# Gadersd/stable-diffusion-burn

Measured on AMD Instinct MI355X. Metric: images/sec @512x512, 20-step DDIM CFG=7.5, SD v1.4, higher is better.
Workload: dtype f32

## Files before the change

include/sdmi.h:

```cpp
#ifndef SDMI_H
#define SDMI_H

#include <stddef.h>
#include <stdint.h>

#ifdef __cplusplus
extern "C" {
#endif

typedef struct sdmi_ctx sdmi_ctx;

typedef enum sdmi_status {
    SDMI_OK = 0,
    SDMI_ERR_INVALID = -1,
    SDMI_ERR_HIP = -2,
    SDMI_ERR_WEIGHTS = -3,
    SDMI_ERR_IO = -4,
    SDMI_ERR_UNSUPPORTED = -5,
    SDMI_ERR_STATE = -6
} sdmi_status;

typedef struct sdmi_config {
    int32_t device;
    int32_t model_channels;
// ... 87 lines not shown
} sdmi_hires;
int sdmi_hires_latent(sdmi_ctx* ctx, const float* context, int32_t n, int32_t T, const float* uncond, int32_t Tu, double scale, size_t n_steps,
                      const float* init_latent, uint64_t seed, const sdmi_hires* hires, const float* hires_noise, float* latent_out);
int sdmi_hires_image(sdmi_ctx* ctx, const float* context, int32_t n, int32_t T, const float* uncond, int32_t Tu, double scale, size_t n_steps,
                     const float* init_latent, uint64_t seed, const sdmi_hires* hires, const float* hires_noise, uint8_t* rgb_out);

typedef struct sdmi_lora sdmi_lora;
int sdmi_lora_create(sdmi_ctx* ctx, sdmi_lora** out);
int sdmi_lora_add(sdmi_lora* a, const char* target, const float* down, const float* up, int32_t rank, float alpha);
int sdmi_lora_set_scale(sdmi_lora* a, double scale);
int sdmi_lora_get_scale(sdmi_lora* a, double* scale, int32_t* n_targets);
int sdmi_lora_destroy(sdmi_lora* a);
int sdmi_lora_effective_weight(sdmi_ctx* ctx, const char* name, float* out, size_t n);

int sdmi_qkv_attention(sdmi_ctx* ctx, const float* q, const float* k, const float* v,
                       const float* mask, int32_t mask_ld, int32_t n, int32_t nq, int32_t nk,
                       int32_t n_state, int32_t n_head, float* out);

typedef struct sdmi_tokenizer sdmi_tokenizer;

int sdmi_tokenizer_create(sdmi_tokenizer** out, const char* merges_path);
void sdmi_tokenizer_destroy(sdmi_tokenizer* tok);
int sdmi_tokenizer_vocab_size(const sdmi_tokenizer* tok);
int sdmi_tokenizer_encode(const sdmi_tokenizer* tok, const char* text, int32_t* ids, int32_t capacity, int32_t* n_ids);
int sdmi_tokenizer_decode(const sdmi_tokenizer* tok, const int32_t* ids, int32_t n, char* out, int32_t capacity, int32_t* n_bytes);

int sdmi_clip_forward(sdmi_ctx* ctx, const int32_t* tokens, int32_t n, int32_t seq_len, float* out);

int sdmi_context(sdmi_ctx* ctx, const sdmi_tokenizer* tok, const char* text, float* out, int32_t capacity_tokens, int32_t* T);

int sdmi_write_png(const char* path, const uint8_t* rgb, int32_t width, int32_t height);

int sdmi_sample_latent_dev(sdmi_ctx* ctx, const float* context, int32_t n, int32_t T,
                           const float* uncond, int32_t Tu, double scale, size_t n_steps,
                           const float* init_latent, float* latent_out);
int sdmi_latent_to_image_dev(sdmi_ctx* ctx, const float* latent, int32_t n, uint8_t* rgb_out);
int sdmi_sample_image_dev(sdmi_ctx* ctx, const float* context, int32_t n, int32_t T,
                          const float* uncond, int32_t Tu, double scale, size_t n_steps,
                          const float* init_latent, uint8_t* rgb_out);
int sdmi_img2img_latent_dev(sdmi_ctx* ctx, const float* context, int32_t n, int32_t T, const float* uncond, int32_t Tu,
                            double scale, size_t n_steps, double strength, const float* z0, const float* mask,
                            const float* noise, uint64_t seed, float* latent_out);
int sdmi_img2img_image_dev(sdmi_ctx* ctx, const float* context, int32_t n, int32_t T, const float* uncond, int32_t Tu,
                           double scale, size_t n_steps, double strength, const uint8_t* init_rgb, const float* mask,
                           const float* noise, uint64_t seed, uint8_t* rgb_out);
int sdmi_hires_latent_dev(sdmi_ctx* ctx, const float* context, int32_t n, int32_t T, const float* uncond, int32_t Tu, double scale, size_t n_steps,
                          const float* init_latent, const sdmi_hires* hires, const float* hires_noise, float* latent_out);
int sdmi_hires_image_dev(sdmi_ctx* ctx, const float* context, int32_t n, int32_t T, const float* uncond, int32_t Tu, double scale, size_t n_steps,
                         const float* init_latent, const sdmi_hires* hires, const float* hires_noise, uint8_t* rgb_out);

typedef struct sdmi_multi sdmi_multi;
int sdmi_create_multi(sdmi_multi** out, const sdmi_config* cfg , const int32_t* devices, int32_t n_devices);
void sdmi_destroy_multi(sdmi_multi* m);
int32_t sdmi_multi_size(sdmi_multi* m);
sdmi_ctx* sdmi_multi_ctx(sdmi_multi* m, int32_t index);
int sdmi_multi_load_weights(sdmi_multi* m, const char* kind, const char* path);
int sdmi_sample_image_sharded(sdmi_multi* m, const float* context, int32_t T, const float* uncond, int32_t Tu,
                              double scale, size_t n_steps, int32_t n_images, const float* init_latents, uint64_t seed,
                              uint8_t* rgb_out);
int sdmi_multi_set_sampler(sdmi_multi* m, const sdmi_sampler* sampler);
int sdmi_shard_range(int32_t n_images, int32_t rank, int32_t n_ranks, int32_t* begin, int32_t* end);
int64_t sdmi_multi_broadcast_count(sdmi_multi* m);
int sdmi_selftest_rank_errors(int32_t n_ranks, int32_t failing_rank);


int sdmi_op_group_norm(sdmi_ctx* ctx, const float* x, const float* gamma, const float* beta,
                       int32_t n, int32_t c, int32_t h, int32_t w, int32_t n_group, float eps,
                       int32_t fuse_silu, float* out);
int sdmi_op_group_norm_fp8(sdmi_ctx* ctx, const float* x, const float* gamma, const float* beta,
                           int32_t n, int32_t c, int32_t h, int32_t w, int32_t n_group, float eps,
                           int32_t fuse_silu, float* out);
int sdmi_op_layer_norm(sdmi_ctx* ctx, const float* x, const float* gamma, const float* beta,
                       int32_t rows, int32_t c, float eps, float* out);
int sdmi_op_conv2d(sdmi_ctx* ctx, const float* x, const float* weight, const float* bias,
                   int32_t n, int32_t cin, int32_t h, int32_t w, int32_t cout, int32_t k,
                   int32_t stride, int32_t pad, int32_t upsample2x, float* out);
int sdmi_op_linear(sdmi_ctx* ctx, const float* x, const float* weight, const float* bias,
                   int32_t rows, int32_t cin, int32_t cout, float* out);
int sdmi_op_conv2d_epilogue(sdmi_ctx* ctx, const float* x, const float* weight, const float* bias, const float* temb,
                            int32_t temb_stride, const float* resid, int32_t resid_ld, int32_t n, int32_t cin, int32_t h,
                            int32_t w, int32_t cout, int32_t k, int32_t stride, int32_t pad, int32_t upsample2x, float* out);
int sdmi_op_linear_epilogue(sdmi_ctx* ctx, const float* x, const float* weight, const float* bias, const float* resid,
                            int32_t resid_ld, int32_t rows, int32_t cin, int32_t cout, float* out);
typedef struct sdmi_op_view {
    int32_t in_ld, in_off;
    int32_t out_ld, out_off;
    float in_fill;
    int32_t in_planes, out_planes;
} sdmi_op_view;
int sdmi_op_conv2d_view(sdmi_ctx* ctx, const float* x, const float* weight, const float* bias, const float* temb, int32_t temb_stride,
                        const float* resid, int32_t resid_ld, int32_t n, int32_t cin, int32_t h, int32_t w, int32_t cout, int32_t k,
                        int32_t stride, int32_t pad, int32_t upsample2x, const sdmi_op_view* view, float* parent, float* parent_planes);
int sdmi_op_linear_view(sdmi_ctx* ctx, const float* x, const float* weight, const float* bias, const float* resid, int32_t resid_ld,
                        int32_t rows, int32_t cin, int32_t cout, const sdmi_op_view* view, float* parent);
int sdmi_op_group_norm_view(sdmi_ctx* ctx, const float* x, const float* gamma, const float* beta, int32_t n, int32_t c, int32_t h, int32_t w,
                            int32_t n_group, float eps, int32_t fuse_silu, const sdmi_op_view* view, int32_t form, float* out);
int sdmi_op_cat_chain(sdmi_ctx* ctx, const float* x, const float* w_x, const float* b_x, const float* w_skip, const float* b_skip,
                      const float* gamma, const float* beta, int32_t n, int32_t cin, int32_t h, int32_t w, int32_t cx, int32_t cskip,
                      float eps, int32_t fuse_silu, int32_t dense, float* out);
int sdmi_op_geglu(sdmi_ctx* ctx, const float* proj, int32_t rows, int32_t hidden, float* out);
int sdmi_op_qkv_attention_ragged(sdmi_ctx* ctx, const float* q, const float* k, const float* v, const int32_t* kv_len,
                                 int32_t n, int32_t nq, int32_t nk, int32_t n_state, int32_t n_head, float* out);
int sdmi_op_resize(sdmi_ctx* ctx, const float* x, int32_t n, int32_t h, int32_t w, int32_t out_h, int32_t out_w, int32_t mode, int32_t antialias,
                   float* out);
int sdmi_op_geglu_forward(sdmi_ctx* ctx, const float* x, const float* weight, const float* bias, int32_t rows, int32_t cin,
                          int32_t hidden, float* out);
int sdmi_op_timestep_embedding(sdmi_ctx* ctx, int32_t t, int32_t dim, float* out);

int sdmi_set_option(sdmi_ctx* ctx, const char* key, const char* value);
int sdmi_last_call_stats(sdmi_ctx* ctx, double* gpu_ms, int64_t* n_kernels, double* flops);
int sdmi_profile_stats(sdmi_ctx* ctx, int32_t cls, double* ms, int64_t* launches, double* flops, double* bytes);
int sdmi_profile_overhead(sdmi_ctx* ctx, double* ms);
int sdmi_bench_conv(sdmi_ctx* ctx, int32_t n, int32_t cin, int32_t h, int32_t w, int32_t cout,
                    int32_t k, int32_t stride, int32_t upsample2x, int32_t tile_cfg, int32_t splitk,
                    int32_t iters, double* ms_out);

int sdmi_bench_attention(sdmi_ctx* ctx, int32_t n, int32_t nq, int32_t nk, int32_t n_state, int32_t n_head,
                         int32_t iters, double* ms_out);

#ifdef __cplusplus
}
#endif
#endif
```

stable_diffusion_burn_amd/_capi.py:

```python
from __future__ import annotations

import ctypes as C
import os
import sys
from pathlib import Path

_PKG = Path(__file__).resolve().parent
LIB_PATH = _PKG / "lib" / "libsdmi.so"


class SdmiError(RuntimeError):
    def __init__(self, status: int, message: str):
        super().__init__(f"sdmi status {status}: {message}")
        self.status = status


class SdmiConfig(C.Structure):
    _fields_ = [
        ("device", C.c_int32), ("model_channels", C.c_int32), ("n_head", C.c_int32), ("ctx_dim", C.c_int32),
        ("latent_h", C.c_int32), ("latent_w", C.c_int32), ("vae_ch", C.c_int32), ("max_batch", C.c_int32),
        ("precision", C.c_int32), ("clip_layers", C.c_int32), ("clip_heads", C.c_int32), ("clip_vocab", C.c_int32),
        ("clip_ctx", C.c_int32), ("reserved", C.c_int32 * 3),
    ]

# ... 16 lines not shown
_F = C.POINTER(C.c_float)
_HIRES = C.POINTER(SdmiHires)
_SAMPLER = C.POINTER(SdmiSampler)
_VIEW = C.POINTER(SdmiOpView)
_U8 = C.POINTER(C.c_uint8)
_CTX = C.c_void_p
_TOK = C.c_void_p
_I32 = C.POINTER(C.c_int32)

SIGNATURES = {
    "sdmi_default_config": (C.c_int, [C.POINTER(SdmiConfig)]),
    "sdmi_create": (C.c_int, [C.POINTER(_CTX), C.POINTER(SdmiConfig)]),
    "sdmi_destroy": (None, [_CTX]),
    "sdmi_last_error": (C.c_char_p, []),
    "sdmi_synchronize": (C.c_int, [_CTX]),
    "sdmi_version": (C.c_char_p, []),
    "sdmi_set_stream": (C.c_int, [_CTX, C.c_void_p, C.c_int32]),
    "sdmi_set_weight": (C.c_int, [_CTX, C.c_char_p, _F, C.c_int32, C.POINTER(C.c_int64)]),
    "sdmi_weight_count": (C.c_int, [_CTX]),
    "sdmi_weight_info": (C.c_int, [_CTX, C.c_int32, C.POINTER(C.c_char_p), C.POINTER(C.c_int32), C.POINTER(C.c_int64)]),
    "sdmi_load_weights_dir": (C.c_int, [_CTX, C.c_char_p]),
    "sdmi_load_weights_mpk": (C.c_int, [_CTX, C.c_char_p]),
    "sdmi_mpk_list": (C.c_int, [C.c_char_p, C.c_char_p, C.c_size_t, C.POINTER(C.c_size_t)]),
    "sdmi_load_weights_packed": (C.c_int, [_CTX, _F, C.c_size_t, C.c_int32]),
    "sdmi_packed_size": (C.c_int64, [_CTX, C.c_int32]),
    "sdmi_finalize_weights": (C.c_int, [_CTX]),
    "sdmi_unet_forward": (C.c_int, [_CTX, _F, C.c_int32, _F, C.c_int32, C.c_int32, _F]),
    "sdmi_sample_latent": (C.c_int, [_CTX, _F, C.c_int32, C.c_int32, _F, C.c_int32, C.c_double, C.c_size_t, _F, C.c_uint64, _F]),
    "sdmi_decode_latent": (C.c_int, [_CTX, _F, C.c_int32, _F]),
    "sdmi_latent_to_image": (C.c_int, [_CTX, _F, C.c_int32, _U8]),
    "sdmi_sample_image": (C.c_int, [_CTX, _F, C.c_int32, C.c_int32, _F, C.c_int32, C.c_double, C.c_size_t, _F, C.c_uint64, _U8]),
    "sdmi_img2img_timesteps": (C.c_int, [C.c_int32, C.c_size_t, C.c_double, _I32, C.c_int32, _I32]),
    "sdmi_img2img_latent": (C.c_int, [_CTX, _F, C.c_int32, C.c_int32, _F, C.c_int32, C.c_double, C.c_size_t, C.c_double, _F, _F, _F, C.c_uint64, _F]),
    "sdmi_img2img_image": (C.c_int, [_CTX, _F, C.c_int32, C.c_int32, _F, C.c_int32, C.c_double, C.c_size_t, C.c_double, _U8, _F, _F, C.c_uint64, _U8]),
    "sdmi_set_sampler": (C.c_int, [_CTX, _SAMPLER]),
    "sdmi_get_sampler": (C.c_int, [_CTX, _SAMPLER]),
    "sdmi_sampler_coefs": (C.c_int, [_SAMPLER, _F, C.c_int32, _I32, C.c_int32, C.c_int64, C.POINTER(C.c_double)]),
    "sdmi_set_latent_size": (C.c_int, [_CTX, C.c_int32, C.c_int32]),
    "sdmi_get_latent_size": (C.c_int, [_CTX, _I32, _I32]),
    "sdmi_resize_weights": (C.c_int, [C.c_int32, C.c_int32, C.c_int32, C.c_int32, _I32, _I32, C.POINTER(C.c_double), C.c_int32, _I32, _I32]),
    "sdmi_hires_latent": (C.c_int, [_CTX, _F, C.c_int32, C.c_int32, _F, C.c_int32, C.c_double, C.c_size_t, _F, C.c_uint64, _HIRES, _F, _F]),
    "sdmi_hires_image": (C.c_int, [_CTX, _F, C.c_int32, C.c_int32, _F, C.c_int32, C.c_double, C.c_size_t, _F, C.c_uint64, _HIRES, _F, _U8]),
    "sdmi_hires_latent_dev": (C.c_int, [_CTX, C.c_void_p, C.c_int32, C.c_int32, C.c_void_p, C.c_int32, C.c_double, C.c_size_t, C.c_void_p, _HIRES, C.c_void_p, C.c_void_p]),
    "sdmi_hires_image_dev": (C.c_int, [_CTX, C.c_void_p, C.c_int32, C.c_int32, C.c_void_p, C.c_int32, C.c_double, C.c_size_t, C.c_void_p, _HIRES, C.c_void_p, C.c_void_p]),
    "sdmi_op_resize": (C.c_int, [_CTX, _F, C.c_int32, C.c_int32, C.c_int32, C.c_int32, C.c_int32, C.c_int32, C.c_int32, _F]),
    "sdmi_multi_set_sampler": (C.c_int, [C.c_void_p, _SAMPLER]),
    "sdmi_lora_create": (C.c_int, [_CTX, C.POINTER(C.c_void_p)]),
    "sdmi_lora_add": (C.c_int, [C.c_void_p, C.c_char_p, _F, _F, C.c_int32, C.c_float]),
    "sdmi_lora_set_scale": (C.c_int, [C.c_void_p, C.c_double]),
    "sdmi_lora_get_scale": (C.c_int, [C.c_void_p, C.POINTER(C.c_double), _I32]),
    "sdmi_lora_destroy": (C.c_int, [C.c_void_p]),
    "sdmi_lora_effective_weight": (C.c_int, [_CTX, C.c_char_p, _F, C.c_size_t]),
    "sdmi_qkv_attention": (C.c_int, [_CTX, _F, _F, _F, _F, C.c_int32, C.c_int32, C.c_int32, C.c_int32, C.c_int32, C.c_int32, _F]),
    "sdmi_tokenizer_create": (C.c_int, [C.POINTER(_TOK), C.c_char_p]),
    "sdmi_tokenizer_destroy": (None, [_TOK]),
    "sdmi_tokenizer_vocab_size": (C.c_int, [_TOK]),
    "sdmi_tokenizer_encode": (C.c_int, [_TOK, C.c_char_p, _I32, C.c_int32, _I32]),
    "sdmi_tokenizer_decode": (C.c_int, [_TOK, _I32, C.c_int32, C.c_char_p, C.c_int32, _I32]),
    "sdmi_clip_forward": (C.c_int, [_CTX, _I32, C.c_int32, C.c_int32, _F]),
    "sdmi_context": (C.c_int, [_CTX, _TOK, C.c_char_p, _F, C.c_int32, _I32]),
    "sdmi_encode_image": (C.c_int, [_CTX, _F, C.c_int32, _F]),
    "sdmi_write_png": (C.c_int, [C.c_char_p, _U8, C.c_int32, C.c_int32]),
    "sdmi_sample_latent_dev": (C.c_int, [_CTX, C.c_void_p, C.c_int32, C.c_int32, C.c_void_p, C.c_int32, C.c_double, C.c_size_t, C.c_void_p, C.c_void_p]),
    "sdmi_latent_to_image_dev": (C.c_int, [_CTX, C.c_void_p, C.c_int32, C.c_void_p]),
    "sdmi_sample_image_dev": (C.c_int, [_CTX, C.c_void_p, C.c_int32, C.c_int32, C.c_void_p, C.c_int32, C.c_double, C.c_size_t, C.c_void_p, C.c_void_p]),
    "sdmi_img2img_latent_dev": (C.c_int, [_CTX, C.c_void_p, C.c_int32, C.c_int32, C.c_void_p, C.c_int32, C.c_double, C.c_size_t, C.c_double, C.c_void_p, C.c_void_p, C.c_void_p, C.c_uint64, C.c_void_p]),
    "sdmi_img2img_image_dev": (C.c_int, [_CTX, C.c_void_p, C.c_int32, C.c_int32, C.c_void_p, C.c_int32, C.c_double, C.c_size_t, C.c_double, C.c_void_p, C.c_void_p, C.c_void_p, C.c_uint64, C.c_void_p]),
    "sdmi_create_multi": (C.c_int, [C.POINTER(C.c_void_p), C.POINTER(SdmiConfig), _I32, C.c_int32]),
    "sdmi_destroy_multi": (None, [C.c_void_p]),
    "sdmi_multi_size": (C.c_int32, [C.c_void_p]),
    "sdmi_multi_ctx": (C.c_void_p, [C.c_void_p, C.c_int32]),
    "sdmi_multi_load_weights": (C.c_int, [C.c_void_p, C.c_char_p, C.c_char_p]),
    "sdmi_sample_image_sharded": (C.c_int, [C.c_void_p, _F, C.c_int32, _F, C.c_int32, C.c_double, C.c_size_t, C.c_int32, _F, C.c_uint64, _U8]),
    "sdmi_shard_range": (C.c_int, [C.c_int32, C.c_int32, C.c_int32, _I32, _I32]),
    "sdmi_multi_broadcast_count": (C.c_int64, [C.c_void_p]),
    "sdmi_selftest_rank_errors": (C.c_int, [C.c_int32, C.c_int32]),
    "sdmi_op_group_norm": (C.c_int, [_CTX, _F, _F, _F, C.c_int32, C.c_int32, C.c_int32, C.c_int32, C.c_int32, C.c_float, C.c_int32, _F]),
    "sdmi_op_group_norm_fp8": (C.c_int, [_CTX, _F, _F, _F, C.c_int32, C.c_int32, C.c_int32, C.c_int32, C.c_int32, C.c_float, C.c_int32, _F]),
    "sdmi_op_layer_norm": (C.c_int, [_CTX, _F, _F, _F, C.c_int32, C.c_int32, C.c_float, _F]),
    "sdmi_op_conv2d": (C.c_int, [_CTX, _F, _F, _F, C.c_int32, C.c_int32, C.c_int32, C.c_int32, C.c_int32, C.c_int32, C.c_int32, C.c_int32, C.c_int32, _F]),
    "sdmi_op_linear": (C.c_int, [_CTX, _F, _F, _F, C.c_int32, C.c_int32, C.c_int32, _F]),
    "sdmi_op_conv2d_epilogue": (C.c_int, [_CTX, _F, _F, _F, _F, C.c_int32, _F, C.c_int32, C.c_int32, C.c_int32, C.c_int32, C.c_int32, C.c_int32, C.c_int32, C.c_int32,
                                          C.c_int32, C.c_int32, _F]),
    "sdmi_op_linear_epilogue": (C.c_int, [_CTX, _F, _F, _F, _F, C.c_int32, C.c_int32, C.c_int32, C.c_int32, _F]),
    "sdmi_op_conv2d_view": (C.c_int, [_CTX, _F, _F, _F, _F, C.c_int32, _F, C.c_int32, C.c_int32, C.c_int32, C.c_int32, C.c_int32, C.c_int32, C.c_int32, C.c_int32,
                                      C.c_int32, C.c_int32, _VIEW, _F, _F]),
    "sdmi_op_linear_view": (C.c_int, [_CTX, _F, _F, _F, _F, C.c_int32, C.c_int32, C.c_int32, C.c_int32, _VIEW, _F]),
    "sdmi_op_group_norm_view": (C.c_int, [_CTX, _F, _F, _F, C.c_int32, C.c_int32, C.c_int32, C.c_int32, C.c_int32, C.c_float, C.c_int32, _VIEW, C.c_int32, _F]),
    "sdmi_op_cat_chain": (C.c_int, [_CTX, _F, _F, _F, _F, _F, _F, _F, C.c_int32, C.c_int32, C.c_int32, C.c_int32, C.c_int32, C.c_int32, C.c_float, C.c_int32,
                                    C.c_int32, _F]),
    "sdmi_op_geglu_forward": (C.c_int, [_CTX, _F, _F, _F, C.c_int32, C.c_int32, C.c_int32, _F]),
    "sdmi_op_geglu": (C.c_int, [_CTX, _F, C.c_int32, C.c_int32, _F]),
    "sdmi_op_qkv_attention_ragged": (C.c_int, [_CTX, _F, _F, _F, _I32, C.c_int32, C.c_int32, C.c_int32, C.c_int32, C.c_int32, _F]),
    "sdmi_op_timestep_embedding": (C.c_int, [_CTX, C.c_int32, C.c_int32, _F]),
    "sdmi_set_option": (C.c_int, [_CTX, C.c_char_p, C.c_char_p]),
    "sdmi_last_call_stats": (C.c_int, [_CTX, C.POINTER(C.c_double), C.POINTER(C.c_int64), C.POINTER(C.c_double)]),
    "sdmi_profile_stats": (C.c_int, [_CTX, C.c_int32, C.POINTER(C.c_double), C.POINTER(C.c_int64), C.POINTER(C.c_double), C.POINTER(C.c_double)]),
    "sdmi_profile_overhead": (C.c_int, [_CTX, C.POINTER(C.c_double)]),
    "sdmi_bench_conv": (C.c_int, [_CTX, C.c_int32, C.c_int32, C.c_int32, C.c_int32, C.c_int32, C.c_int32, C.c_int32, C.c_int32, C.c_int32, C.c_int32, C.c_int32, C.POINTER(C.c_double)]),
    "sdmi_bench_attention": (C.c_int, [_CTX, C.c_int32, C.c_int32, C.c_int32, C.c_int32, C.c_int32, C.c_int32, C.POINTER(C.c_double)]),
}

_lib = None


def load_library() -> C.CDLL:
    global _lib
    if _lib is not None:
        return _lib
    if not LIB_PATH.exists():
        raise ImportError(
            f"{LIB_PATH} is missing: build it with `python -m stable_diffusion_burn_amd.build` "
            "(libsdmi has no CPU or PyTorch fallback)")
    lib = C.CDLL(str(LIB_PATH), mode=C.RTLD_GLOBAL if "torch" in sys.modules else C.RTLD_LOCAL)
    for name, (res, args) in SIGNATURES.items():
        fn = getattr(lib, name)
        fn.restype = res
        fn.argtypes = args
    _lib = lib
    return lib


def check(status: int) -> None:
    if status != 0:
        msg = load_library().sdmi_last_error()
        raise SdmiError(status, msg.decode("utf-8", "replace") if msg else "")
```

stable_diffusion_burn_amd/csrc/engine.cpp:

```cpp
#include "engine.hpp"
#include "mpk_reader.hpp"

#include <dlfcn.h>

#include <algorithm>
#include <cmath>
#include <cstdarg>
#include <cstdio>
#include <cstring>
#include <fstream>
#include <sstream>

namespace sdmi {

static constexpr size_t kAlign = 256;
static constexpr size_t kSlabMin = (size_t)1 << 30;

DevPool::~DevPool() {
    for (auto& s : slabs_) (void)hipFree(s.base);
}

void* DevPool::alloc(size_t bytes) {
    if (bytes == 0) bytes = kAlign;
    bytes = (bytes + kAlign - 1) / kAlign * kAlign;
// ... 532 lines not shown
            SDMI_HIP(hipEventCreateWithFlags(&stager_->done[i], hipEventDisableTiming));
        }
    }
    Stager& st = *stager_;
    const size_t need = (bytes + 255) / 256 * 256;
    if (st.used + need > kStageBytes) {
        SDMI_HIP(hipEventRecord(st.done[st.cur], stream_));
        st.busy[st.cur] = true;
        st.cur ^= 1;
        st.used = 0;
        if (st.busy[st.cur]) { SDMI_HIP(hipEventSynchronize(st.done[st.cur])); st.busy[st.cur] = false; }
    }
    *offset = st.used;
    *half = st.cur;
    st.used += need;
    return st.pinned[st.cur] + *offset;
}

void* Engine::persistent_alloc(size_t bytes, bool weight_buffer) {
    void* p = nullptr;
    SDMI_HIP(hipMalloc(&p, bytes));
    if (pool_.fill() >= 0) {
        hipError_t e = hipMemsetAsync(p, pool_.fill(), bytes, stream_);
        if (e == hipSuccess && !weight_buffer) e = hipStreamSynchronize(stream_);
        if (e != hipSuccess) { (void)hipFree(p); SDMI_HIP(e); }
        pool_.note_fill(bytes);
    }
    if (weight_buffer) persistent_blocks_.push_back({p, bytes});
    return p;
}

void Engine::ensure_arena(int group) {
    if (arena_done_[group]) return;
    size_t total = 0;
    for (auto& e : entries_) {
        if (e.group != group || e.kind == 3 || *e.dst) continue;
        size_t count = 1;
        for (int i = 0; i < e.ndim; ++i) count *= (size_t)e.dims[i];
        if (e.kind == 0 && e.dims[1] == 3) count = count / 3 * 4;
        total += (count * (e.wdt ? 2 : 4) + 255) / 256 * 256;
    }
    if (total) {
        char* base = static_cast<char*>(persistent_alloc(total));
        weight_allocs_.push_back(base);
        arena_base_[group] = base;
        arena_bytes_[group] = total;
        if (!bf16_) {
            split_base_[group] = static_cast<char*>(persistent_alloc(total / 2 * 3));
            weight_allocs_.push_back(split_base_[group]);
        }
        size_t off = 0;
        for (auto& e : entries_) {
            if (e.group != group || e.kind == 3 || *e.dst) continue;
            size_t count = 1;
            for (int i = 0; i < e.ndim; ++i) count *= (size_t)e.dims[i];
            if (e.kind == 0 && e.dims[1] == 3) count = count / 3 * 4;
            *e.dst = reinterpret_cast<float*>(base + off);
            off += (count * (e.wdt ? 2 : 4) + 255) / 256 * 256;
        }
    }
    if (opt_keep_masters_) {
        size_t mtotal = 0;
        for (auto& e : entries_)
            if (e.group == group && e.kind <= 1) mtotal += (stage_elems(e) * sizeof(float) + 255) / 256 * 256;
        if (mtotal) {
            char* mbase = static_cast<char*>(persistent_alloc(mtotal));
            weight_allocs_.push_back(mbase);
            size_t off = 0;
            for (auto& e : entries_) {
                if (e.group != group || e.kind > 1) continue;
                e.master = reinterpret_cast<float*>(mbase + off);
                off += (stage_elems(e) * sizeof(float) + 255) / 256 * 256;
            }
        }
    }
    arena_done_[group] = true;
}

Engine::TempSplit::TempSplit(Engine* e_, const float* bt_, long long rows, long long K) : e(e_), bt(bt_) {
    if (e->bf16_ || K % 32 || rows <= 0) return;
    planes = e->pool_.alloc((size_t)rows * K * 6);
    hipError_t err = launch_pack_split3(bt, planes, rows, (int)K, e->stream_, e->b3_grouped(rows));
    if (err != hipSuccess) { e->pool_.free(planes); planes = nullptr; SDMI_HIP(err); }
    e->temp_split_bt_ = bt;
    e->temp_split_planes_ = planes;
}
Engine::TempSplit::~TempSplit() {
    if (!planes) return;
    e->temp_split_bt_ = nullptr;
    e->temp_split_planes_ = nullptr;
    e->pool_.free(planes);
}

const void* Engine::split_planes(const float* bt) const {
    if (bt && bt == temp_split_bt_) return temp_split_planes_;
    const char* b = reinterpret_cast<const char*>(bt);
    for (int g = 0; g < 3; ++g)
        if (split_base_[g] && b >= arena_base_[g] && b < arena_base_[g] + arena_bytes_[g]) return split_base_[g] + (size_t)(b - arena_base_[g]) / 2 * 3;
    for (const SplitRegion& r : split_regions_)
        if (b >= r.base && b < r.base + r.bytes) return r.planes + (size_t)(b - r.base) / 2 * 3;
    return nullptr;
}

static size_t entry_count(const WeightEntry& e) {
    size_t count = 1;
    for (int i = 0; i < e.ndim; ++i) count *= (size_t)e.dims[i];
    return count;
}

size_t Engine::stage_elems(const WeightEntry& e) {
    const size_t count = entry_count(e);
    return (e.kind == 0 && e.dims[1] == 3) ? count / 3 * 4 : count;
}

void Engine::pack_entry(WeightEntry& e, float* stage) {
    const size_t n_stage = stage_elems(e);
    if (e.pre_scale != 1.f) SDMI_HIP(launch_scale_f32(stage, (long long)n_stage, e.pre_scale, stream_));
    hipError_t err;
    if (e.kind == 0) {
        const int cout = (int)e.dims[0], cin = e.dims[1] == 3 ? 4 : (int)e.dims[1], k = (int)e.dims[2];
        if (!(cin % 32 == 0 || (cin < 32 && cin % 4 == 0))) throw Error(SDMI_ERR_UNSUPPORTED, "conv Cin must be a multiple of 32, or < 32 and a multiple of 4");
        err = e.wdt ? launch_pack_conv_weight_bf16(stage, *e.dst, cout, cin, k, k, stream_)
                    : launch_pack_conv_weight(stage, *e.dst, cout, cin, k, k, stream_);
        if (err == hipSuccess && e.dst8) {
            const size_t kp = (size_t)((cin + 127) / 128 * 128) * k * k;
            if (!*e.dst8) {
                void* q = persistent_alloc((size_t)cout * kp);
                weight_allocs_.push_back(q);
                void* sc = persistent_alloc((size_t)cout * kp / 32);
                weight_allocs_.push_back(sc);
                *e.dst8 = reinterpret_cast<float*>(q);
                *e.dsts = reinterpret_cast<float*>(sc);
            }
            err = launch_pack_conv_weight_fp8(stage, *e.dst8, *e.dsts, cout, cin, k, k, stream_);
        }
    } else {
        err = e.wdt ? launch_pack_linear_weight_bf16(stage, *e.dst, (int)e.dims[0], (int)e.dims[1], stream_)
                    : launch_pack_linear_weight(stage, *e.dst, (int)e.dims[0], (int)e.dims[1], stream_);
        if (err == hipSuccess && e.dst8) {
            const int cin = (int)e.dims[0], cout = (int)e.dims[1];
            const size_t kp = (size_t)(cin + 127) / 128 * 128;
            if (!*e.dst8) {
                void* q = persistent_alloc((size_t)cout * kp);
                weight_allocs_.push_back(q);
                void* sc = persistent_alloc((size_t)cout * kp / 32);
                weight_allocs_.push_back(sc);
                *e.dst8 = reinterpret_cast<float*>(q);
                *e.dsts = reinterpret_cast<float*>(sc);
            }
            err = launch_pack_linear_weight_fp8(stage, *e.dst8, *e.dsts, cin, cout, stream_);
        }
    }
    SDMI_HIP(err);
    if (!e.wdt) {
        const long long rows = e.kind == 0 ? e.dims[0] : e.dims[1];
        const long long K = e.kind == 0 ? (e.dims[1] == 3 ? 4 : e.dims[1]) * e.dims[2] * e.dims[3] : e.dims[0];
        void* planes = const_cast<void*>(split_planes(*e.dst));
        if (planes && K % 32 == 0) SDMI_HIP(launch_pack_split3(*e.dst, planes, rows, (int)K, stream_, b3_grouped(rows)));
    }
}

void Engine::stage_commit(WeightEntry& e, size_t offset, int half) {
    Stager& st = *stager_;
    const size_t count = entry_count(e);
    const float* host = reinterpret_cast<const float*>(st.pinned[half] + offset);
    if (e.kind == 3) {
        alphas_.assign(host, host + count);
        e.set = true;
        return;
    }
    ensure_arena(e.group);
    if (e.kind == 2) {
        SDMI_HIP(hipMemcpyAsync(*e.dst, host, count * sizeof(float), hipMemcpyHostToDevice, stream_));
    } else {
        float* stage = reinterpret_cast<float*>(st.dev[half] + offset);
        const size_t n_stage = stage_elems(e);
        SDMI_HIP(hipMemcpyAsync(stage, host, n_stage * sizeof(float), hipMemcpyHostToDevice, stream_));
        if (e.master) SDMI_HIP(hipMemcpyAsync(e.master, stage, n_stage * sizeof(float), hipMemcpyDeviceToDevice, stream_));
// ... 409 lines not shown
        }
    }
    SDMI_HIP(hipEventRecord(ev0_, stream_));
}
void Engine::end_call() {
    SDMI_HIP(hipEventRecord(ev1_, stream_));
    if (call_dev_ && has_user_stream_) SDMI_HIP(hipStreamWaitEvent(user_stream_, ev1_, 0));
    SDMI_HIP(hipEventSynchronize(ev1_));
    float ms = 0;
    SDMI_HIP(hipEventElapsedTime(&ms, ev0_, ev1_));
    last_ms = ms; last_kernels = n_kernels_; last_flops = flops_;
}
void Engine::abort_call() noexcept {
    (void)hipStreamSynchronize(stream_);
    try {
        us_ = UNetState{};
        pool_.free_since(call_mark_);
    } catch (...) {}
}

void Engine::set_option(const std::string& key, const std::string& value) {
    if (key == "gemm_tile") gopt_.force_tile = (value == "auto") ? -1 : std::stoi(value);
    else if (key == "splitk") gopt_.force_splits = std::stoi(value);
    else if (key == "roctx") roctx_enable(std::stoi(value) != 0);
    else if (key == "fp8_convs") opt_fp8_convs_ = std::stoi(value);
    else if (key == "fp8_min_rows") opt_fp8_min_rows_ = std::stoi(value);
    else if (key == "fp8_linear") opt_fp8_linear_ = std::stoi(value);
    else if (key == "fp8_ops") opt_fp8_ops_ = std::stoi(value);
    else if (key == "op_resid") opt_op_resid_ = std::stoi(value);
    else if (key == "op_misalign") opt_op_misalign_ = std::stoi(value);
    else if (key == "pool_fill") {
        const int b = std::stoi(value);
        if (b < -1 || b > 255) throw Error(SDMI_ERR_INVALID, "pool_fill: -1 (off) or a byte 0 .. 255");
        pool_.set_fill(b);
        if (b >= 0 && std::none_of(entries_.begin(), entries_.end(), [](const WeightEntry& w) { return w.set; })) {
            SDMI_HIP(hipSetDevice(cfg_.device));
            for (const PersistentBlock& pb : persistent_blocks_) {
                SDMI_HIP(hipMemsetAsync(pb.p, b, pb.bytes, stream_));
                pool_.note_fill(pb.bytes);
            }
        }
    }
    else if (key == "dump_pool_fills") {
        std::ofstream f(value);
        if (!f) throw Error(SDMI_ERR_IO, "dump_pool_fills: cannot write " + value);
        unsigned long long blocks = 0, bytes = 0;
        pool_.take_fill_counts(&blocks, &bytes);
        f << blocks << " " << bytes << "\n";
    }
    else if (key == "cfg_share") opt_cfg_share_ = std::stoi(value);
    else if (key == "attn_kv_splits") opt_attn_kv_splits_ = std::stoi(value);
    else if (key == "attn_kv_prefer8") opt_attn_kv_prefer8_ = std::stoi(value);
    else if (key == "b3_grouped") {
        if (!entries_.empty() && std::any_of(entries_.begin(), entries_.end(), [](const WeightEntry& w) { return w.set; }))
            throw Error(SDMI_ERR_STATE, "b3_grouped selects the layout the weight planes are packed in: set it before the first weight is loaded");
        opt_b3_grouped_ = std::stoi(value);
    }
    else if (key == "keep_masters") {
        if (std::any_of(entries_.begin(), entries_.end(), [](const WeightEntry& w) { return w.set; }) || arena_done_[0] || arena_done_[1] || arena_done_[2])
            throw Error(SDMI_ERR_STATE, "keep_masters decides what the weight arenas hold: set it before the first weight is loaded");
        opt_keep_masters_ = std::stoi(value) != 0;
    }
    else if (key == "attn_pack_tail") opt_attn_pack_tail_ = (value == "default") ? 3 : std::stoi(value);
    else if (key == "gn32_min_wgs") opt_gn32_min_wgs_ = (opt_gn32_min_wgs_ & ~0xFFFF) | (std::stoi(value) & 0xFFFF);
    else if (key == "gn32_stats_min_wgs") opt_gn32_min_wgs_ = (opt_gn32_min_wgs_ & 0xFFFF) | ((std::stoi(value) + 1) << 16);
    else if (key == "gn_target_wgs") gn_tune_.target_wgs = std::stoi(value);
    else if (key == "gn_max_threads") gn_tune_.max_threads = std::stoi(value);
    else if (key == "gn_unroll") gn_tune_.unroll = std::stoi(value);
    else if (key == "fp8_tile") opt_fp8_tile_ = (value == "auto") ? -1 : std::stoi(value);
    else if (key == "resid_acc") opt_resid_acc_ = std::stoi(value);
    else if (key == "attn_bf16") opt_attn_bf16_ = std::stoi(value);
    else if (key == "attn_bf16_variant") opt_attn_bf16_variant_ = (value == "default") ? kAttnBf16VariantDefault : std::stoi(value, nullptr, 0);
    else if (key == "attn_split") opt_attn_split_ = std::stoi(value);
    else if (key == "gemm_bf16x") gopt_.gemm_bf16x = std::stoi(value);
    else if (key == "gemm_x32") gopt_.gemm_x32 = std::stoi(value);
    else if (key == "gemm_f32s") gopt_.gemm_f32s = std::stoi(value);
    else if (key == "bench_cold") opt_bench_cold_ = std::stoi(value);
    else if (key == "gemm_probe") opt_gemm_probe_ = std::stoi(value);
    else if (key == "conv3_reuse") gopt_.conv3_reuse = std::stoi(value);
    else if (key == "gemm_planes") gopt_.gemm_planes = (value == "default") ? GemmPlanOpts().gemm_planes : std::stoi(value);
    else if (key == "gemm3x_variant") opt_gemm3x_variant_ = (value == "default") ? kGemm3xVariantDefault : std::stoi(value);
    else if (key == "gemm_bf16x_variant") opt_gemm_bf16x_variant_ = (value == "default") ? kGemmBf16xVariantDefault : std::stoi(value);
    else if (key == "geglu_fuse") opt_geglu_fuse_ = std::stoi(value);
    else if (key == "record_shapes") { record_shapes_ = std::stoi(value) != 0; if (record_shapes_) { shape_counts_.clear(); choice_counts_.clear(); } }
    else if (key == "dump_shapes") {
        std::ofstream f(value);
        if (!f) throw Error(SDMI_ERR_IO, "dump_shapes: cannot write " + value);
        for (auto& kv : shape_counts_) f << kv.first << " " << kv.second << "\n";
    }
    else if (key == "dump_choices") {
        std::ofstream f(value);
        if (!f) throw Error(SDMI_ERR_IO, "dump_choices: cannot write " + value);
        for (auto& kv : choice_counts_) f << kv.first << " x" << kv.second << "\n";
    }
    else if (key == "profile") { prof_flush(); profiling_ = std::stoi(value) != 0; prof_tagging_ = std::stoi(value) >= 2; if (profiling_) prof_calibrate(); }
    else if (key == "dump_profile_tags") {
        prof_flush();
        std::ofstream f(value);
        if (!f) throw Error(SDMI_ERR_IO, "dump_profile_tags: cannot write " + value);
        for (auto& kv : prof_tags_) f << kv.second.ms << " " << kv.second.launches << " " << kv.second.flops << " " << kv.second.bytes << "\t" << kv.first << "\n";
    }
    else if (key == "profile_reset") prof_reset();
    else if (key == "tune" || key == "tune_bf16") tuning_.set(value, key == "tune_bf16");
    else if (key == "tune_clear") tuning_.clear();
    else throw Error(SDMI_ERR_INVALID, "unknown option '" + key + "'");
}

void Engine::set_resid_acc(ConvGemm& p, bool eligible, bool resid_ok) const {
    p.resid_acc = 0;
    if (!eligible || (p.N % 8) || (p.ldc % 8)) return;
    if ((opt_resid_acc_ & 1) && p.resid && resid_ok && (p.ldr % 4) == 0 && ((uintptr_t)p.resid & 7) == 0) p.resid_acc |= 1;
    if ((opt_resid_acc_ & 2) && (p.bias || p.rowvec) && (p.rowvec_stride % 4) == 0 && (((uintptr_t)p.bias | (uintptr_t)p.rowvec) & 15) == 0) p.resid_acc |= 2;
}

void Engine::record_choice(const ConvGemm& p, const char* kind, int cfg, const char* note) {
    if (!record_shapes_) return;
    char ck[128];
    std::snprintf(ck, sizeof ck, "%d,%d,%d k%d s%d u%d W%d%s cfg=%d splits=%d%s acc=%d", p.M, p.N, p.K, p.KH, p.stride, p.ups, p.Ws, kind, cfg, p.splits, note, p.resid_acc);
    ++choice_counts_[ck];
}

void Engine::run_gemm(ConvGemm& p, const GemmRun& r) {
    if (p.splits == 1) {
        p.slabs = nullptr; p.slab_stride = 0;
        ProfScope ps(this, r.pc, r.flops, r.bytes);
        ps.set_tag("%s %d,%d,%d k%d%s%s%s cfg=%d splits=1", r.what, p.M, p.N, p.K, p.KH, p.geglu ? " geglu" : "", p.resid ? " resid" : "", p.rowvec ? " rowvec" : "", r.cfg);
        SDMI_HIP(r.launch(p, r.index, stream_));
        count_kernel(r.flops);
        return;
    }
    p.slab_stride = (long long)p.M * p.N;
    Buf slab(this, (size_t)p.splits * p.slab_stride * sizeof(float));
    p.slabs = slab.f();
    {
        ProfScope ps(this, r.pc, r.flops, r.bytes);
        ps.set_tag("%s %d,%d,%d k%d%s cfg=%d splits=%d", r.what, p.M, p.N, p.K, p.KH, p.geglu ? " geglu" : "", r.cfg, p.splits);
        SDMI_HIP(r.launch(p, r.index, stream_));
    }
    count_kernel(r.flops);
    ProfScope ps(this, PC_SPLITK_REDUCE, 0, (double)(p.splits + 1) * p.slab_stride * 4.0);
    if (r.reduce_tag) ps.set_tag("reduce %d,%d,%d k%d cfg=%d splits=%d", p.M, p.N, p.K, p.KH, r.cfg, p.splits);
    SDMI_HIP(r.bf16_reduce ? launch_splitk_reduce_bf16(p, stream_) : launch_splitk_reduce(p, stream_));
    count_kernel();
}

void Engine::launch_gemm(ConvGemm& p, int in_dt, int force_cfg, int force_splits) {
    const int kt_elems = in_dt ? 64 : 32;
    p.kt_total = (p.K + kt_elems - 1) / kt_elems;
    if (in_dt && (p.Cin % 64)) throw Error(SDMI_ERR_UNSUPPORTED, "bf16 GEMM: K slices must be multiples of 64");
    if (record_shapes_) {
        char sk[96];
        std::snprintf(sk, sizeof sk, "%d,%d,%d,%d,%d,%d,%d,%d", p.NB, p.Cin, p.Hs, p.Ws, p.N, p.KH, p.stride, p.ups);
        ++shape_counts_[sk];
    }
    p.Bt3 = in_dt ? nullptr : split_planes(p.Bt);
    p.b3_grouped = b3_grouped((long long)p.N * (p.geglu ? 2 : 1)) ? 1 : 0;
    p.variant = in_dt ? opt_gemm_bf16x_variant_ : opt_gemm3x_variant_;
    p.zero_page = zero_page_;
    p.probe = probe_buf_;
    GemmPlanIn in{};
    in.M = p.M; in.N = p.N; in.K = p.K; in.kt_total = p.kt_total; in.bf16 = in_dt; in.geglu = p.geglu; in.out_mode = p.out_mode; in.force_cfg = force_cfg; in.force_splits = force_splits;
    in.KH = p.KH; in.KW = p.KW; in.stride = p.stride; in.pad = p.pad; in.ups = p.ups; in.Cin = p.Cin; in.Hs = p.Hs; in.Ws = p.Ws; in.Ho = p.Ho; in.Wo = p.Wo;
    in.zero_page = zero_page_ != nullptr;
    in.x32_ok = !in_dt && p.CS == 32 && p.Cin % 32 == 0 && p.out_mode == 0;
    in.s_ok = in.x32_ok && p.Bt3 && (unsigned long long)p.N * (p.geglu ? 2 : 1) * (unsigned long long)p.kt_total * 192ull < 0xFFFFFF00ull;
    in.p_ok = in.s_ok && (unsigned long long)p.NB * p.Hs * p.Ws * (unsigned long long)(p.A3 ? p.a3_ld : p.Cin * 6) < 0xFFFFFF00ull;
    in.from_planes = !in_dt && p.A3 != nullptr;
    if (!in.from_planes && !p.A) throw Error(SDMI_ERR_STATE, "gemm: no activations");
    const GemmPlan g = plan_gemm(in, gopt_, tuning_);
    p.kt_per_split = g.kt_per_split; p.splits = g.splits;
    const bool w_planes = g.tile.family >= kFamS, a_planes = g.tile.family == kFamP;
    const double flops = 2.0 * p.M * (double)p.N * p.K * (p.geglu ? 2.0 : 1.0);
    const unsigned long long es = in_dt ? 2ull : 4ull;
    const unsigned long long a_ext = ((unsigned long long)p.NB * p.Hs * p.Ws - 1) * (unsigned long long)p.a_ld * es + (unsigned long long)p.Cin * es;
    const unsigned long long b_ext = ((unsigned long long)p.N * (p.geglu ? 2 : 1) - 1) * (unsigned long long)p.b_ld * es + (unsigned long long)p.K * es;
    if (a_ext >= 0xFFFFFFE0ull || b_ext >= 0xFFFFFFE0ull) throw Error(SDMI_ERR_UNSUPPORTED, "GEMM: operand larger than 4 GiB (the buffer-load range check needs 32-bit extents)");
    p.a_bytes = (unsigned)a_ext;
    p.b_bytes = (unsigned)b_ext;
    void* const c3_want = in_dt ? nullptr : p.C3;
    const int ldc3_want = p.ldc3;
    const bool vec_out = (p.N % 4 == 0) && (!p.C || p.ldc % 4 == 0) && (!p.resid || p.ldr % 4 == 0);
    const bool c3_native = c3_want && w_planes && vec_out && (!p.geglu || (p.geglu == 2 && a_planes));
    std::unique_ptr<Buf> c_tmp;
    if (!c3_native) {
        p.C3 = nullptr;
        if (c3_want && !p.C) {
            c_tmp.reset(new Buf(this, (size_t)p.M * p.N * sizeof(float)));
            p.C = c_tmp->f(); p.ldc = p.N;
        }
    }
    if (!p.C) p.ldc = p.N;
    std::unique_ptr<Buf> a3_tmp;
    if (a_planes && !p.A3) {
        const long long rows = (long long)p.NB * p.Hs * p.Ws;
        p.a3_ld = (p.Cin / 32) * 192;
        a3_tmp.reset(new Buf(this, (size_t)rows * p.a3_ld));
        ProfScope ps(this, PC_SPLIT_ROWS, 0, (double)rows * p.Cin * 10.0);
        SDMI_HIP(launch_split3_rows(p.A, a3_tmp->p, rows, p.Cin, p.a_ld, p.a3_ld, stream_));
        count_kernel();
        p.A3 = a3_tmp->p;
    }
    set_resid_acc(p, in_dt && g.tile.family == kFamX && g.splits == 1, !p.geglu);
    record_choice(p, "", g.cfg, p.Bt3 || in_dt ? "" : " (no planes)");
    const double a_es = in_dt ? 2.0 : (a_planes ? 6.0 : 4.0), w_es = in_dt ? 2.0 : (w_planes ? 6.0 : 4.0);
    const double c_es = in_dt ? (p.out_mode == 1 ? 4.0 : 2.0) : (p.out_mode == 2 ? 2.0 : ((p.C ? 4.0 : 0.0) + (c3_native ? 6.0 : 0.0)));
    const double gemm_bytes = (double)p.NB * p.Hs * p.Ws * p.Cin * a_es + (double)p.N * (p.geglu ? 2.0 : 1.0) * p.K * w_es + (double)p.M * p.N * c_es;
    static const GemmLauncher kLaunchers[2][kNumGemmFamilies] = {{launch_conv_gemm2, launch_conv_gemm2x, launch_conv_gemm3x, launch_conv_gemm3p},
                                                                 {launch_conv_gemm_bf16, launch_conv_gemm_bf16_large, nullptr, nullptr}};
    run_gemm(p, GemmRun{kLaunchers[in_dt ? 1 : 0][g.tile.family], g.tile.index, "gemm", g.cfg, w_planes ? PC_CONV_SPLIT : PC_CONV_GEMM, in_dt != 0, true, flops, gemm_bytes});
    if (c3_want && !c3_native) {
        ProfScope ps(this, PC_SPLIT_ROWS, 0, (double)p.M * p.N * 10.0);
        SDMI_HIP(launch_split3_rows(p.C, c3_want, p.M, p.N, p.ldc, ldc3_want, stream_));
        count_kernel();
    }
}

void Engine::conv(const ConvW& w, const Act& x, Act& y, int stride, int ups, const float* rowvec, int rowvec_stride,
                  const Act* resid, bool pad_br) {
    if (x.c != w.cin) throw Error(SDMI_ERR_INVALID, "conv: input channels mismatch");
    const int pad = pad_br ? 0 : (w.k == 3 ? 1 : 0);
    const int hin = x.h << ups, win = x.w << ups;
    const int extra = pad_br ? 1 : 0;
    const int ho = (hin + 2 * pad + extra - w.k) / stride + 1, wo = (win + 2 * pad + extra - w.k) / stride + 1;
    if (y.n != x.n || y.h != ho || y.w != wo || y.c != w.cout) throw Error(SDMI_ERR_INVALID, "conv: output shape mismatch");
    ConvGemm p{};
    if (resid && (resid->rows() != y.rows() || resid->c != y.c || resid->dt != y.dt)) throw Error(SDMI_ERR_STATE, "conv: residual shape / type mismatch");
    p.A = x.p; p.Bt = w.bt; p.C = y.p; p.bias = w.bias; p.rowvec = rowvec; p.resid = resid ? resid->p : nullptr;
    if (resid && !resid->p) throw Error(SDMI_ERR_STATE, "conv: the residual must exist as fp32");
    if (!x.dt && plane_gemm(w.cin, w.cout) && split_planes(w.bt)) { p.A3 = x.p3; p.a3_ld = x.ld3; }
    if (!x.p && !p.A3) throw Error(SDMI_ERR_STATE, "conv: the input exists only as planes, which this layer cannot read");
    p.C3 = y.p3; p.ldc3 = y.ld3;
    p.M = x.n * ho * wo; p.N = w.cout; p.K = w.cin * w.k * w.k;
    p.NB = x.n; p.Hs = x.h; p.Ws = x.w; p.Cin = w.cin; p.Ho = ho; p.Wo = wo;
    p.KH = w.k; p.KW = w.k; p.stride = stride; p.pad = pad; p.ups = ups;
    p.ldc = y.stride(); p.ldr = resid ? resid->stride() : y.stride(); p.a_ld = x.stride(); p.b_ld = p.K; p.rowvec_stride = rowvec_stride;
    p.CS = std::min(32, w.cin);
    if (!y.p && !y.p3) throw Error(SDMI_ERR_STATE, "conv: no output buffer");
    if (x.dt != w.dt) throw Error(SDMI_ERR_STATE, "conv: activation / weight storage types disagree");
    p.out_mode = x.dt ? (y.dt ? 0 : 1) : (y.dt ? 2 : 0);
    if (resid && !x.dt && y.dt) throw Error(SDMI_ERR_STATE, "conv: residual not supported on the fp32->bf16 layers");
    launch_gemm(p, x.dt);
}

static ConvGemm linear_gemm(const float* A, int rows, const float* bt, const float* bias, int cin, int cout, float* C, int ldc, const float* resid, int ldr) {
    ConvGemm p{};
    p.A = A; p.Bt = bt; p.C = C; p.bias = bias; p.resid = resid;
    p.M = rows; p.N = cout; p.K = cin;
    p.NB = 1; p.Hs = 1; p.Ws = rows; p.Cin = cin; p.Ho = 1; p.Wo = rows;
    p.KH = 1; p.KW = 1; p.stride = 1; p.pad = 0; p.ups = 0;
    p.ldc = ldc; p.ldr = ldr; p.a_ld = cin; p.b_ld = cin; p.rowvec_stride = 0; p.CS = 32;
    return p;
}

void Engine::gemm(const float* A, int a_rows, const float* bt, const float* bias, int cin, int cout, float* C, int ldc,
                  const float* resid, int ldr, int dt, int out_mode, const void* A3, void* C3) {
    if (dt < 0) dt = edt();
    if (cin % 32) throw Error(SDMI_ERR_UNSUPPORTED, "linear: in_features must be a multiple of 32");
    ConvGemm p = linear_gemm(A, a_rows, bt, bias, cin, cout, C, ldc, resid, ldr);
    p.A3 = A3; p.a3_ld = (cin / 32) * 192;
    p.C3 = C3; p.ldc3 = (cout / 32) * 192;
    if (C3 && (cout % 32)) throw Error(SDMI_ERR_STATE, "linear: plane output needs out_features % 32 == 0");
    p.out_mode = out_mode;
    launch_gemm(p, dt);
}

void Engine::gemm_geglu(const float* x, long long rows, const float* bt, const float* bias, int cin, int hidden, float* out, int dt,
                        const void* x3, void* out3) {
    if (dt < 0) dt = edt();
    if (x3 && (out3 || out) && !dt && opt_geglu_fuse_ && hidden % 32 == 0 && cin % 32 == 0 && split_planes(bt)) {
        const int cfg = plan_geglu_plane_tile(rows, hidden, cin, gopt_, tuning_);
        if (cfg >= 0) {
            ConvGemm p = linear_gemm(x, (int)rows, bt, bias, cin, hidden, out, hidden, nullptr, hidden);
            p.A3 = x3; p.a3_ld = (cin / 32) * 192;
            p.C3 = out3; p.ldc3 = (hidden / 32) * 192;
            p.geglu = 2;
            launch_gemm(p, 0, cfg, 1);
            return;
        }
    }
    if (x3 || out3) {
        Buf proj(this, (size_t)rows * 2 * hidden * 4);
        gemm(x, (int)rows, bt, bias, cin, 2 * hidden, proj.f(), 2 * hidden, nullptr, 0, dt, 0, x3, nullptr);
        {
            ProfScope ps(this, PC_GEGLU, 0, (double)rows * hidden * (8.0 + (out3 ? 6.0 : 4.0)));
            if (out3) SDMI_HIP(launch_geglu_planes(proj.f(), out3, rows, hidden, stream_));
            else SDMI_HIP(launch_geglu(proj.f(), out, rows, hidden, stream_));
        }
        count_kernel();
        return;
    }
    const bool eligible = opt_geglu_fuse_ && hidden % 8 == 0 && cin % (dt ? 64 : 32) == 0 && (dt ? gopt_.gemm_bf16x : gopt_.gemm_x32);
    const int cfg = eligible ? plan_geglu_paired_tile(rows, hidden, opt_geglu_fuse_, !dt && gopt_.gemm_f32s && split_planes(bt)) : -1;
    if (cfg >= 0) {
        ConvGemm p = linear_gemm(x, (int)rows, bt, bias, cin, hidden, out, hidden, nullptr, hidden);
        p.geglu = 1;
        launch_gemm(p, dt, cfg, 1);
        return;
// ... 63 lines not shown
        int kv_splits = 1;
        if (!dt && !mask && opt_attn_kv_splits_ != 1) {
            const long long wgs = (long long)((nq + (on_split ? 127 : 63)) / (on_split ? 128 : 64)) * n * n_head;
            const int tiles = (nk + attn_f32_kv_tile(p) - 1) / attn_f32_kv_tile(p);
            long long s_auto = wgs > 0 && wgs <= 128 ? 256 / wgs : 1;
            s_auto = std::min<long long>(std::min<long long>(s_auto, tiles / 2), 8);
            if (on_split && opt_attn_kv_prefer8_) {
                const long long wgs8 = (long long)((nq + 255) / 256) * n * n_head;
                const long long s8 = std::min<long long>(std::min<long long>(wgs8 < 256 ? (256 + wgs8 - 1) / wgs8 : 1, tiles / 2), 8);
                if (s8 >= 2 && wgs8 * s8 >= 256) s_auto = s8;
            }
            kv_splits = opt_attn_kv_splits_ > 1 ? std::min(opt_attn_kv_splits_, std::max(1, tiles)) : (int)std::max<long long>(1, s_auto);
        }
        std::unique_ptr<Buf> part_o, part_ml;
        if (kv_splits > 1) {
            part_o.reset(new Buf(this, (size_t)kv_splits * n * nq * n_head * d_head * sizeof(float)));
            part_ml.reset(new Buf(this, (size_t)kv_splits * n * n_head * nq * 2 * sizeof(float)));
            p.kv_splits = kv_splits; p.part_o = part_o->f(); p.part_ml = part_ml->f();
        }
        ProfScope ps(this, PC_ATTENTION, fl, 0, kv_splits > 1 ? 2 : 1);
        ps.set_tag("attention n%d nq%d nk%d h%d d%d slices=%d", n, nq, nk, n_head, d_head, kv_splits);
        if (dt && opt_attn_bf16_ && (d_head == 40 || d_head == 80 || d_head == 160)) SDMI_HIP(launch_attention_bf16(p, stream_));
        else if (on_split) SDMI_HIP(launch_attention_split(p, stream_));
        else SDMI_HIP(launch_attention(p, stream_));
        count_kernel(fl);
        if (kv_splits > 1) {
            SDMI_HIP(launch_attention_combine(p, stream_));
            count_kernel();
        }
        return;
    }
    if (mask) throw Error(SDMI_ERR_UNSUPPORTED, "attention: additive mask is only supported for head dims 40/80/160");
    if (d_head % 32) throw Error(SDMI_ERR_UNSUPPORTED, "attention: head dim must be 40/80/160 or a multiple of 32");
    if (dt && (d_head % 64)) throw Error(SDMI_ERR_UNSUPPORTED, "bf16 attention (unfused path): head dim must be a multiple of 64");
    for (int b = 0; b < n; ++b)
        if ((kv_len_host ? kv_len_host[b] : nk) % (dt ? 64 : 32)) throw Error(SDMI_ERR_UNSUPPORTED, "attention (unfused path): key count must be a multiple of 32 (64 for bf16)");
    for (int b = 0; b < n; ++b) {
        const int nkb = kv_len_host ? kv_len_host[b] : nk;
        Buf s(this, (size_t)nq * nkb * sizeof(float));
        Buf pb(this, dt ? (size_t)nq * nkb * 2 : 256);
        Buf vt(this, (size_t)d_head * nkb * (dt ? 2 : 4));
        for (int h = 0; h < n_head; ++h) {
            const float* qb = adv(q, b * q_bs + h * d_head, dt);
            const float* kb = adv(k, b * k_bs + h * d_head, dt);
            const float* vb = adv(v, b * v_bs + h * d_head, dt);
            float* ob = adv(o, b * o_bs + h * d_head, dt);
            ConvGemm g{};
            g.A = qb; g.Bt = kb; g.C = s.f();
            g.M = nq; g.N = nkb; g.K = d_head; g.NB = 1; g.Hs = 1; g.Ws = nq; g.Cin = d_head; g.Ho = 1; g.Wo = nq;
            g.KH = g.KW = 1; g.stride = 1; g.ldc = nkb; g.ldr = nkb; g.a_ld = ldq; g.b_ld = ldk; g.CS = 32;
            g.out_mode = dt ? 1 : 0;
            launch_gemm(g, dt);
            if (dt) { ProfScope ps_o(this, PC_OTHER); SDMI_HIP(launch_softmax_rows_f32_to_bf16(s.f(), pb.p, nq, nkb, scale * scale, stream_)); }
            else { ProfScope ps_o(this, PC_OTHER); SDMI_HIP(launch_softmax_rows(s.f(), nq, nkb, scale * scale, stream_)); }
            count_kernel();
            if (dt) { ProfScope ps_o(this, PC_OTHER); SDMI_HIP(launch_transpose2d_bf16(vb, vt.p, nkb, d_head, ldv, stream_)); }
            else { ProfScope ps_o(this, PC_OTHER); SDMI_HIP(launch_transpose2d(vb, vt.f(), nkb, d_head, ldv, stream_)); }
            count_kernel();
            ConvGemm g2{};
            g2.A = dt ? pb.f() : s.f(); g2.Bt = vt.f(); g2.C = ob;
            g2.M = nq; g2.N = d_head; g2.K = nkb; g2.NB = 1; g2.Hs = 1; g2.Ws = nq; g2.Cin = nkb; g2.Ho = 1; g2.Wo = nq;
            g2.KH = g2.KW = 1; g2.stride = 1; g2.ldc = ldo; g2.ldr = ldo; g2.a_ld = nkb; g2.b_ld = nkb; g2.CS = 32;
            launch_gemm(g2, dt);
        }
    }
}

void Engine::res_block(const ResW& w, const Act& x, Act& y, int step) {
    Range rng(this, "ResBlock");
    Act h2 = new_act(x.n, x.h, x.w, w.cout);
    const float* rowvec = nullptr;
    if (w.has_embed) rowvec = us_.temb.at(w.temb_index) + (size_t)step * w.cout;
    if (use_fp8(w.conv_in, x)) {
        ActQ q1 = new_actq(x.n, x.h, x.w, x.c);
        group_norm_fp8(w.norm_in, x, q1, true);
        conv_fp8(w.conv_in, q1, h2, rowvec, nullptr);
        release(q1);
    } else {
        Act h1 = plane_gemm(x.c, w.cout) ? new_act3(x.n, x.h, x.w, x.c, 2) : new_act(x.n, x.h, x.w, x.c);
        group_norm(w.norm_in, x, h1, true);
        conv(w.conv_in, h1, h2, 1, 0, rowvec, 0, nullptr);
        release(h1);
    }
    Act sk{};
    if (w.has_skip) {
        if (y.p) { sk = y; sk.p3 = nullptr; sk.view = true; }
        else sk = new_act(y.n, y.h, y.w, y.c);
        if (use_fp8_wide(w.skip.bt8, x.rows()) && x.dt == 1 && x.c % 32 == 0) {
            ActQ xq = new_actq(x.n, x.h, x.w, x.c);
            quantize(x, xq);
            conv_fp8(w.skip, xq, sk, nullptr, nullptr);
            release(xq);
        } else {
            conv(w.skip, x, sk, 1, 0, nullptr, 0, nullptr);
        }
    }
    const Act* resid = w.has_skip ? &sk : &x;
    if (use_fp8(w.conv_out, h2)) {
        ActQ q3 = new_actq(x.n, x.h, x.w, w.cout);
        group_norm_fp8(w.norm_out, h2, q3, true);
        release(h2);
        conv_fp8(w.conv_out, q3, y, nullptr, resid);
        release(q3);
    } else {
        Act h3 = plane_gemm(w.cout, w.cout) ? new_act3(x.n, x.h, x.w, w.cout, 2) : new_act(x.n, x.h, x.w, w.cout);
        group_norm(w.norm_out, h2, h3, true);
        release(h2);
        conv(w.conv_out, h3, y, 1, 0, nullptr, 0, resid);
        release(h3);
    }
    if (w.has_skip) release(sk);
}

bool Engine::use_fp8(const ConvW& w, const Act& x) const {
    return fp8_ && opt_fp8_convs_ && w.bt8 && x.dt == 1 && x.rows() >= opt_fp8_min_rows_;
}

ActQ Engine::new_actq(int n, int h, int w, int c) {
    ActQ a; a.n = n; a.h = h; a.w = w; a.c = c; a.cp = (c + 127) / 128 * 128;
    a.q = pool_.alloc((size_t)a.rows() * a.cp);
    a.s = pool_.alloc((size_t)a.rows() * (a.cp / 32));
    return a;
}
void Engine::release(ActQ& a) {
    if (a.q) pool_.free(a.q);
    if (a.s) pool_.free(a.s);
    a.q = a.s = nullptr;
}

void Engine::group_norm_fp8(const NormW& w, const Act& x, ActQ& y, bool silu) {
    const int hw = x.h * x.w;
    if (x.dt != 1 || y.c != x.c) throw Error(SDMI_ERR_STATE, "group_norm_fp8: bf16 input of matching width expected");
    Buf part(this, gn_partials_bytes_bf16(x.n, hw, x.c, gn_tune_));
    ProfScope ps(this, PC_GROUP_NORM, 0, (double)x.bytes() + (double)x.rows() * (y.cp + y.cp / 32), 2);
    SDMI_HIP(launch_group_norm_fp8(x.p, y.q, y.s, w.gamma, w.beta, x.n, hw, x.c, x.stride(), 32, w.eps, silu, part.p, stream_, &gn_tune_));
    count_kernel(); count_kernel();
}

void Engine::conv_fp8(const ConvW& w, const ActQ& x, Act& y, const float* rowvec, const Act* resid, int stride, int ups, int rowvec_stride) {
    if (x.c != w.cin || (w.k != 3 && w.k != 1) || !w.bt8) throw Error(SDMI_ERR_STATE, "conv_fp8: not an MXFP8-packed convolution");
    const int pad = w.k == 3 ? 1 : 0;
    const int hin = x.h << ups, win = x.w << ups;
    const int ho = (hin + 2 * pad - w.k) / stride + 1, wo = (win + 2 * pad - w.k) / stride + 1;
    if (y.n != x.n || y.h != ho || y.w != wo || y.c != w.cout || y.dt != 1) throw Error(SDMI_ERR_INVALID, "conv_fp8: output shape / type mismatch");
    if (resid && (resid->rows() != y.rows() || resid->c != y.c || resid->dt != 1)) throw Error(SDMI_ERR_STATE, "conv_fp8: residual shape / type mismatch");
    ConvGemm p{};
    p.A = reinterpret_cast<const float*>(x.q); p.Bt = w.bt8; p.C = y.p; p.bias = w.bias; p.rowvec = rowvec; p.resid = resid ? resid->p : nullptr;
    p.a_scale = x.s; p.b_scale = w.bs8;
    p.M = x.n * ho * wo; p.N = w.cout; p.K = x.cp * w.k * w.k;
    p.NB = x.n; p.Hs = x.h; p.Ws = x.w; p.Cin = x.cp; p.Ho = ho; p.Wo = wo;
    p.KH = w.k; p.KW = w.k; p.stride = stride; p.pad = pad; p.ups = ups;
    p.ldc = y.stride(); p.ldr = resid ? resid->stride() : y.stride(); p.a_ld = x.cp; p.b_ld = p.K; p.rowvec_stride = rowvec_stride; p.CS = 128;
    launch_fp8(p, 2.0 * p.M * (double)p.N * w.cin * w.k * w.k);
}

void Engine::gemm_fp8(const ActQ& x, const LinW& w, int n_rows_w, void* C, int ldc, const float* resid, int ldr) {
    if (x.c != w.cin || !w.bt8) throw Error(SDMI_ERR_STATE, "gemm_fp8: not an MXFP8-packed Linear layer");
    ConvGemm p = linear_gemm(reinterpret_cast<const float*>(x.q), (int)x.rows(), w.bt8, w.bias, x.cp, n_rows_w, reinterpret_cast<float*>(C), ldc, resid, ldr);
    p.a_scale = x.s; p.b_scale = w.bs8; p.CS = 128;
    launch_fp8(p, 2.0 * p.M * (double)p.N * w.cin);
}

void Engine::launch_fp8(ConvGemm& p, double flops) {
    p.out_mode = 0;
    p.variant = opt_gemm_bf16x_variant_;
    p.zero_page = zero_page_;
    p.kt_total = p.K / 128;
    if ((unsigned long long)p.NB * p.Hs * p.Ws * (unsigned long long)p.a_ld >= 0xFFFFFFE0ull || (unsigned long long)p.N * p.K >= 0xFFFFFFE0ull) throw Error(SDMI_ERR_UNSUPPORTED, "fp8 GEMM: operand larger than 4 GiB");
    const TileChoice tc = plan_gemm_fp8(p.M, p.N, p.kt_total, opt_fp8_tile_, gopt_.force_splits, &p.kt_per_split);
    p.splits = tc.splits;
    set_resid_acc(p, tc.splits == 1, true);
    record_choice(p, " fp8", tc.cfg, "");
    const double fp8_bytes = ((double)p.NB * p.Hs * p.Ws * p.a_ld + (double)p.N * p.K) * (1.0 + 1.0 / 32.0) + (double)p.M * p.N * 2.0;
    run_gemm(p, GemmRun{launch_conv_gemm_fp8x, tc.cfg, "gemm_fp8", tc.cfg, PC_CONV_FP8, true, false, flops, fp8_bytes});
}

void Engine::conv_raw(const ConvW& w, const Act& x, Act& y, int stride, int ups) {
    if (use_fp8_wide(w.bt8, y.rows()) && x.dt == 1 && y.dt == 1 && x.p && x.c % 32 == 0) {
        ActQ xq = new_actq(x.n, x.h, x.w, x.c);
        quantize(x, xq);
        conv_fp8(w, xq, y, nullptr, nullptr, stride, ups);
        release(xq);
        return;
    }
    conv(w, x, y, stride, ups, nullptr, 0, nullptr);
}

void Engine::quantize(const Act& x, ActQ& y) {
    if (x.dt != 1 || !x.p || y.c != x.c || y.rows() != x.rows()) throw Error(SDMI_ERR_STATE, "quantize: bf16 input of matching shape expected");
    ProfScope ps(this, PC_OTHER, 0, (double)x.rows() * (x.c * 2.0 + y.cp * 1.03));
    SDMI_HIP(launch_quantize_bf16_fp8(x.p, y.q, y.s, x.rows(), x.c, x.stride(), stream_));
    count_kernel();
}

// ... 796 lines not shown
    }
    SDMI_HIP(launch_layer_norm(x, out, gamma, beta, rows, c, eps, stream_));
}

const float* Engine::stage_epi(std::unique_ptr<Buf>& b, const float* host, long long rows, int c, int ld, int dt, long long nchw_hw) {
    if (ld < c) throw Error(SDMI_ERR_INVALID, "epilogue operand: row stride below the channel count");
    const size_t es = dt ? 2 : 4, bytes = (size_t)rows * ld * es;
    std::vector<unsigned char> img(bytes);
    for (long long r = 0; r < rows; ++r)
        for (int j = 0; j < ld; ++j) {
            const float v = j >= c ? std::nanf("") : nchw_hw ? host[((r / nchw_hw) * c + j) * nchw_hw + r % nchw_hw] : host[r * c + j];
            unsigned char* d = img.data() + ((size_t)r * ld + j) * es;
            if (dt) {
                uint32_t u;
                std::memcpy(&u, &v, 4);
                const uint16_t hb = std::isnan(v) ? (uint16_t)0x7FC0 : (uint16_t)((u + 0x7FFFu + ((u >> 16) & 1u)) >> 16);
                std::memcpy(d, &hb, 2);
            } else std::memcpy(d, &v, 4);
        }
    b.reset(new Buf(this, bytes + 16));
    unsigned char* dst = static_cast<unsigned char*>(b->p) + (opt_op_misalign_ ? es : 0);
    SDMI_HIP(hipMemcpyAsync(dst, img.data(), bytes, hipMemcpyHostToDevice, stream_));
    SDMI_HIP(hipStreamSynchronize(stream_));
    return reinterpret_cast<const float*>(dst);
}

void Engine::op_conv2d(const float* x, const float* wt, const float* bias, int n, int cin, int h, int wd, int cout,
                       int k, int stride, int pad, int ups, float* out, const EpiOps* epi) {
    if (!(k == 1 || k == 3) || pad != (k == 3 ? 1 : 0) || !(stride == 1 || stride == 2))
        throw Error(SDMI_ERR_UNSUPPORTED, "conv2d: only 3x3 pad 1 / 1x1 pad 0, stride 1|2 are on the hot path");
    if (!(cin % 32 == 0 || (cin < 32 && cin % 4 == 0))) throw Error(SDMI_ERR_UNSUPPORTED, "conv2d: Cin must be a multiple of 32, or < 32 and a multiple of 4");
    if (epi && epi->temb_stride && epi->temb_stride < cout) throw Error(SDMI_ERR_INVALID, "conv2d: temb_stride below cout");
    std::unique_ptr<Buf> tb, rb;
    const float* temb = (epi && epi->temb) ? stage_epi(tb, epi->temb, epi->temb_stride ? n : 1, cout, epi->temb_stride ? epi->temb_stride : cout, 0) : nullptr;
    auto epi_resid = [&](const Act& y) {
        Act r = y;
        r.view = true; r.p3 = nullptr;
        r.ld = epi->resid_ld ? epi->resid_ld : y.c;
        r.p = const_cast<float*>(stage_epi(rb, epi->resid, y.rows(), y.c, r.ld, y.dt, (long long)y.h * y.w));
        return r;
    };
    if (fp8_ && opt_fp8_convs_ && k == 3 && stride == 1 && !ups && cin % 32 == 0 && cout % 8 == 0) {
        const int cp = (cin + 127) / 128 * 128;
        ConvW w; w.cin = cin; w.cout = cout; w.k = 3; w.dt = 1; w.bias = const_cast<float*>(bias);
        Buf bt8(this, (size_t)cout * cp * 9), bs8(this, (size_t)cout * cp * 9 / 32);
        SDMI_HIP(launch_pack_conv_weight_fp8(wt, bt8.p, bs8.p, cout, cin, 3, 3, stream_));
        w.bt8 = bt8.f(); w.bs8 = bs8.f();
        Act a32 = new_act(n, h, wd, cin, 0);
        SDMI_HIP(launch_nchw_to_nhwc(x, a32.p, n, cin, h, wd, 1.0f, stream_));
        ActQ q = new_actq(n, h, wd, cin);
        SDMI_HIP(launch_quantize_fp8(a32.p, q.q, q.s, a32.rows(), cin, stream_));
        release(a32);
        Act y = new_act(n, h, wd, cout, 1);
        Act r;
        if (epi && epi->resid) r = epi_resid(y);
        conv_fp8(w, q, y, temb, r.p ? &r : nullptr, 1, 0, epi ? epi->temb_stride : 0);
        SDMI_HIP(launch_nhwc_bf16_to_nchw_f32(y.p, out, n, cout, h, wd, stream_));
        release(q); release(y);
        return;
    }
    ConvW w; w.cin = cin; w.cout = cout; w.k = k;
    w.dt = (bf16_ && cin % 64 == 0) ? 1 : 0;
    if (bf16_ && !w.dt && cin >= 32) throw Error(SDMI_ERR_UNSUPPORTED, "bf16 conv2d: Cin must be a multiple of 64 (or < 32)");
    Buf bt(this, (size_t)cout * cin * k * k * 4);
    if (w.dt) SDMI_HIP(launch_pack_conv_weight_bf16(wt, bt.p, cout, cin, k, k, stream_));
    else SDMI_HIP(launch_pack_conv_weight(wt, bt.f(), cout, cin, k, k, stream_));
    TempSplit planes(this, bt.f(), w.dt ? 0 : cout, (long long)cin * k * k);
    w.bt = bt.f(); w.bias = const_cast<float*>(bias);
    Act a = new_act(n, h, wd, cin, w.dt);
    if (w.dt) SDMI_HIP(launch_nchw_f32_to_nhwc_bf16(x, a.p, n, cin, h, wd, 1.0f, stream_));
    else SDMI_HIP(launch_nchw_to_nhwc(x, a.p, n, cin, h, wd, 1.0f, stream_));
    const int hin = h << ups, win = wd << ups;
    const int ho = (hin + 2 * pad - k) / stride + 1, wo = (win + 2 * pad - k) / stride + 1;
    Act y = new_act(n, ho, wo, cout, (bf16_ && cout > 4) ? 1 : 0);
    const bool with_resid = opt_op_resid_ && cin == cout && stride == 1 && !ups && a.dt == y.dt;
    Act r;
    if (epi && epi->resid) r = epi_resid(y);
    conv(w, a, y, stride, ups, temb, epi ? epi->temb_stride : 0, r.p ? &r : with_resid ? &a : nullptr);
    if (y.dt) SDMI_HIP(launch_nhwc_bf16_to_nchw_f32(y.p, out, n, cout, ho, wo, stream_));
    else SDMI_HIP(launch_nhwc_to_nchw(y.p, out, n, cout, ho, wo, stream_));
    release(a); release(y);
}

void Engine::op_linear(const float* x, const float* wt, const float* bias, int rows, int cin, int cout, float* out, const EpiOps* epi) {
    const int rld = (epi && epi->resid) ? (epi->resid_ld ? epi->resid_ld : cout) : 0;
    std::unique_ptr<Buf> rb;
    auto epi_resid = [&](int dt) { return rld ? stage_epi(rb, epi->resid, rows, cout, rld, dt) : nullptr; };
    if (fp8_ && opt_fp8_ops_ && cin % 32 == 0 && cout % 8 == 0) {
        const size_t kp = (size_t)(cin + 127) / 128 * 128;
        Buf xh(this, (size_t)rows * cin * 2), yh(this, (size_t)rows * cout * 2), w8(this, (size_t)cout * kp), s8(this, (size_t)cout * kp / 32);
        SDMI_HIP(launch_f32_to_bf16(x, xh.p, (long long)rows * cin, stream_));
        SDMI_HIP(launch_pack_linear_weight_fp8(wt, w8.p, s8.p, cin, cout, stream_));
        Act xa; xa.p = xh.f(); xa.n = 1; xa.h = 1; xa.w = rows; xa.c = cin; xa.dt = 1;
        ActQ q = new_rowsq(rows, cin);
        quantize(xa, q);
        LinW lw; lw.cin = cin; lw.cout = cout; lw.dt = 1; lw.bias = const_cast<float*>(bias); lw.bt8 = w8.f(); lw.bs8 = s8.f();
        gemm_fp8(q, lw, cout, yh.p, cout, epi_resid(1), rld);
        SDMI_HIP(launch_nhwc_bf16_to_nchw_f32(yh.p, out, rows, cout, 1, 1, stream_));
        release(q);
        return;
    }
    Buf bt(this, (size_t)cin * cout * 4);
    if (bf16_ && cin % 64 == 0) {
        Buf xh(this, (size_t)rows * cin * 2), yh(this, (size_t)rows * cout * 2);
        SDMI_HIP(launch_pack_linear_weight_bf16(wt, bt.p, cin, cout, stream_));
        SDMI_HIP(launch_f32_to_bf16(x, xh.p, (long long)rows * cin, stream_));
        const bool with_resid = opt_op_resid_ && cin == cout;
        if (rld) gemm(xh.f(), rows, bt.f(), bias, cin, cout, yh.f(), cout, epi_resid(1), rld, 1);
        else gemm(xh.f(), rows, bt.f(), bias, cin, cout, yh.f(), cout, with_resid ? xh.f() : nullptr, with_resid ? cin : 0, 1);
        SDMI_HIP(launch_nhwc_bf16_to_nchw_f32(yh.p, out, rows, cout, 1, 1, stream_));
        return;
    }
    SDMI_HIP(launch_pack_linear_weight(wt, bt.f(), cin, cout, stream_));
    TempSplit planes(this, bt.f(), cout, cin);
    const bool with_resid = opt_op_resid_ && cin == cout;
    if (rld) gemm(x, rows, bt.f(), bias, cin, cout, out, cout, epi_resid(0), rld, 0);
    else gemm(x, rows, bt.f(), bias, cin, cout, out, cout, with_resid ? x : nullptr, with_resid ? cin : 0, 0);
}

void Engine::check_view(const sdmi_op_view& v, int cin, int cout) {
    if (v.in_ld < cin || v.in_off < 0 || v.in_off + cin > v.in_ld || v.out_ld < cout || v.out_off < 0 || v.out_off + cout > v.out_ld ||
        v.in_planes < 0 || v.in_planes > 3 || v.out_planes < 0 || v.out_planes > 3)
        throw Error(SDMI_ERR_INVALID, "view: need 0 <= off, off + c <= ld and planes in 0 .. 3");
}

void Engine::op_conv2d_view(const float* xp, const float* wt, const float* bias, int n, int cin, int h, int wd, int cout, int k, int stride, int pad, int ups,
                            const sdmi_op_view& v, const EpiOps* epi, float* yp, float* yp3) {
    check_view(v, cin, cout);
    if (!(k == 1 || k == 3) || pad != (k == 3 ? 1 : 0) || !(stride == 1 || stride == 2))
        throw Error(SDMI_ERR_UNSUPPORTED, "conv2d: only 3x3 pad 1 / 1x1 pad 0, stride 1|2 are on the hot path");
    if (!(cin % 32 == 0 || (cin < 32 && cin % 4 == 0))) throw Error(SDMI_ERR_UNSUPPORTED, "conv2d: Cin must be a multiple of 32, or < 32 and a multiple of 4");
    if (epi && epi->temb_stride && epi->temb_stride < cout) throw Error(SDMI_ERR_INVALID, "conv2d: temb_stride below cout");
    const bool q8 = fp8_ && opt_fp8_convs_ && k == 3 && stride == 1 && !ups && cin % 32 == 0 && cout % 8 == 0;
    const int wdt = (bf16_ && cin % 64 == 0) ? 1 : 0;
    if (!q8 && bf16_ && !wdt && cin >= 32) throw Error(SDMI_ERR_UNSUPPORTED, "bf16 conv2d: Cin must be a multiple of 64 (or < 32)");
    const int xdt = q8 ? 1 : wdt, ydt = q8 ? 1 : ((bf16_ && cout > 4) ? 1 : 0);
    const int hin = h << ups, win = wd << ups;
    const int ho = (hin + 2 * pad - k) / stride + 1, wo = (win + 2 * pad - k) / stride + 1;
    if ((xdt && v.in_planes > 1) || (ydt && v.out_planes > 1)) throw Error(SDMI_ERR_INVALID, "view: planes are an fp32 format");
    Act a = (!xdt && v.in_planes > 1) ? new_act3(n, h, wd, v.in_ld, v.in_planes) : new_act(n, h, wd, v.in_ld, xdt);
    if (xdt) SDMI_HIP(launch_f32_to_bf16(xp, a.p, a.rows() * v.in_ld, stream_));
    else {
        if (a.p) SDMI_HIP(hipMemcpyAsync(a.p, xp, a.bytes(), hipMemcpyDeviceToDevice, stream_));
        if (a.p3) SDMI_HIP(launch_split3_rows(xp, a.p3, a.rows(), v.in_ld, v.in_ld, a.ld3, stream_));
    }
    Act y = (!ydt && v.out_planes > 1) ? new_act3(n, ho, wo, v.out_ld, v.out_planes) : new_act(n, ho, wo, v.out_ld, ydt);
    if (ydt) SDMI_HIP(launch_f32_to_bf16(yp, y.p, y.rows() * v.out_ld, stream_));
    else {
        if (y.p) SDMI_HIP(hipMemcpyAsync(y.p, yp, y.bytes(), hipMemcpyDeviceToDevice, stream_));
        if (y.p3) SDMI_HIP(launch_split3_rows(yp, y.p3, y.rows(), v.out_ld, v.out_ld, y.ld3, stream_));
    }
    auto give_back = [&] {
        if (ydt) SDMI_HIP(launch_nhwc_bf16_to_nchw_f32(y.p, yp, (int)y.rows(), v.out_ld, 1, 1, stream_));
        else {
            if (y.p) SDMI_HIP(hipMemcpyAsync(yp, y.p, y.bytes(), hipMemcpyDeviceToDevice, stream_));
            if (y.p3) SDMI_HIP(launch_join3_rows(y.p3, y.p ? yp3 : yp, y.rows(), v.out_ld, y.ld3, v.out_ld, stream_));
        }
    };
    try {
        Act xs = slice(a, v.in_off, cin), ys = slice(y, v.out_off, cout);
        std::unique_ptr<Buf> tb, rb;
        const float* temb = (epi && epi->temb) ? stage_epi(tb, epi->temb, epi->temb_stride ? n : 1, cout, epi->temb_stride ? epi->temb_stride : cout, 0) : nullptr;
        Act r;
        if (epi && epi->resid) {
            if (!ys.p) throw Error(SDMI_ERR_INVALID, "view: a residual needs the output as fp32");
            r = ys;
// ... 383 lines not shown
```

stable_diffusion_burn_amd/csrc/engine.hpp:

```cpp
#pragma once
#include <hip/hip_runtime.h>

#include <functional>
#include <map>
#include <memory>
#include <stdexcept>
#include <string>
#include <vector>

#include "../../include/sdmi.h"
#include "error.hpp"
#include "gemm_plan.hpp"
#include "kernels.hpp"

namespace sdmi {

#define SDMI_HIP(expr)                                                                                   \
    do {                                                                                                 \
        hipError_t _e = (expr);                                                                          \
        if (_e != hipSuccess)                                                                            \
            throw ::sdmi::Error(SDMI_ERR_HIP, std::string(#expr) + ": " + hipGetErrorString(_e) + " (" + \
                                                  __FILE__ + ":" + std::to_string(__LINE__) + ")");      \
    } while (0)

// ... 55 lines not shown
};
struct MhaW { LinW q, k, v, out; };
struct SpatialW {
    NormW norm; ConvW proj_in, proj_out; NormW ln1, ln2, ln3; MhaW attn1, attn2; LinW geglu_proj, mlp_lin;
    int c = 0, ctx_index = -1;
};
enum BlockKind { BK_CONV, BK_DOWN, BK_RES, BK_RES_ST, BK_RES_UP, BK_RES_ST_UP };
struct UBlock { BlockKind kind; int cin, cout; ConvW conv; ResW res; SpatialW st; ConvW up; };
struct VaeAttnW { NormW norm; ConvW q, k, v, proj_out; int c = 0; };
struct DecBlockW { ResW res[3]; ConvW upsampler; bool has_up = false; int cin = 0, cout = 0; };

struct ClipBlockW { NormW attn_ln, mlp_ln; LinW q, k, v, out, fc1, fc2; };

struct WeightEntry {
    std::string name;
    int kind;
    int ndim;
    int64_t dims[4];
    float** dst;
    int wdt = 0;
    int group = 0;
    float** dst8 = nullptr;
    float** dsts = nullptr;
    float pre_scale = 1.f;
    bool set = false;
    float* master = nullptr;
};

struct LoraTarget { int entry; int rank; double alpha; float* down; float* up; };

struct MetaEntry { std::string name; int n; float expect[2]; float* store; };

class Engine {
public:
    explicit Engine(const sdmi_config& cfg);
    ~Engine();
    Engine(const Engine&) = delete;
    Engine& operator=(const Engine&) = delete;

    void set_weight(const char* name, const float* data, int ndim, const int64_t* dims);
    void load_weights_dir(const char* dir);
    void load_weights_mpk(const char* path);
    void load_weights_packed(const float* data, size_t n_floats, int groups);
    size_t packed_size(int groups) const;
    void finalize_weights();
    const std::vector<WeightEntry>& entries() const { return entries_; }
    sdmi_lora* lora_create();
    void lora_add(sdmi_lora* a, const char* target, const float* down, const float* up, int rank, float alpha);
    void lora_set_scale(sdmi_lora* a, double scale);
    void lora_destroy(sdmi_lora* a);
    void effective_weight(const char* name, float* out, size_t n);

    void unet_forward_dev(const float* x_nchw, int t, const float* context, int n, int T, float* out_nchw);
    void clip_forward_dev(const int32_t* tokens, int n, int T, float* out);
    bool clip_ready() const { return clip_ready_; }
    void encode_image_dev(const float* img_nchw, int n, float* latent_nchw);
    void sample_latent_dev(const float* context, int n, int T, const float* uncond, int Tu, double scale,
                           size_t n_steps, const float* init_latent, float* latent_out, bool out_nhwc = false);
    void img2img_latent_dev(const float* context, int n, int T, const float* uncond, int Tu, double scale, size_t n_steps,
                            double strength, const float* z0, const float* mask, const float* noise, uint64_t seed, float* latent_out);
    void img2img_image_dev(const float* context, int n, int T, const float* uncond, int Tu, double scale, size_t n_steps,
                           double strength, const uint8_t* init_rgb, const float* mask, const float* noise, uint64_t seed, float* latent_out);
    void hires_latent_dev(const float* context, int n, int T, const float* uncond, int Tu, double scale, size_t n_steps, const float* init_latent,
                          const sdmi_hires& hr, const float* hires_noise, float* latent_out);
    static void check_hires(const sdmi_hires* hr);
    void resize_nhwc4(const float* x, int n, int h, int w, int oh, int ow, int mode, int antialias, float* y);
    void op_resize(const float* x_nchw, int n, int h, int w, int oh, int ow, int mode, int antialias, float* out_nchw);
    static void check_sampler(const sdmi_sampler& s);
    void set_sampler(const sdmi_sampler* s);
    const sdmi_sampler& sampler() const { return sampler_; }
    void decode_latent_dev(const float* latent_nchw, int n, float in_scale, float* img_nchw, uint8_t* rgb_u8);
    void qkv_attention_dev(const float* q, const float* k, const float* v, const float* mask, int mask_ld, int n,
                           int nq, int nk, int n_state, int n_head, float* out, const int* kv_len_host = nullptr);

    void op_group_norm(const float* x, const float* gamma, const float* beta, int n, int c, int h, int w, int groups,
                       float eps, bool silu, float* out);
    void op_group_norm_fp8(const float* x, const float* gamma, const float* beta, int n, int c, int h, int w, int groups, float eps,
                           bool silu, float* out);
    void op_layer_norm(const float* x, const float* gamma, const float* beta, int rows, int c, float eps, float* out);
    struct EpiOps { const float* temb = nullptr; int temb_stride = 0; const float* resid = nullptr; int resid_ld = 0; };
    void op_conv2d(const float* x, const float* w, const float* bias, int n, int cin, int h, int wd, int cout, int k,
                   int stride, int pad, int ups, float* out, const EpiOps* epi = nullptr);
    void op_linear(const float* x, const float* w, const float* bias, int rows, int cin, int cout, float* out, const EpiOps* epi = nullptr);
    void op_geglu(const float* proj, int rows, int hidden, float* out);
    static void check_view(const sdmi_op_view& v, int cin, int cout);
    void op_conv2d_view(const float* xp, const float* w, const float* bias, int n, int cin, int h, int wd, int cout, int k, int stride, int pad, int ups,
                        const sdmi_op_view& v, const EpiOps* epi, float* yp, float* yp3);
    void op_linear_view(const float* x, const float* w, const float* bias, int rows, int cin, int cout, const sdmi_op_view& v, const EpiOps* epi, float* yp);
    void op_group_norm_view(const float* xp, const float* gamma, const float* beta, int n, int c, int h, int w, int groups, float eps, bool silu,
                            const sdmi_op_view& v, int form, float* out);
    void op_cat_chain(const float* x, const float* w_x, const float* b_x, const float* w_skip, const float* b_skip, const float* gamma, const float* beta,
                      int n, int cin, int h, int wd, int cx, int cskip, float eps, bool silu, bool dense, float* out);
    void op_geglu_forward(const float* x, const float* wt, const float* bias, int rows, int cin, int hidden, float* out);
    void op_timestep_embedding(int t, int dim, float* out);
    double bench_conv(int n, int cin, int h, int w, int cout, int k, int stride, int ups, int tile_cfg, int splitk,
                      int iters);

    double bench_attention(int n, int nq, int nk, int n_state, int n_head, int iters);
    void set_option(const std::string& key, const std::string& value);
    void sync();
    void begin_call(bool dev_inputs = false);
    void end_call();
    void abort_call() noexcept;
    struct Call {
        Engine& e; bool done = false;
        Call(Engine& e_, bool dev_inputs = false) : e(e_) { e.begin_call(dev_inputs); }
        void finish() { e.end_call(); done = true; }
        ~Call() { if (!done) e.abort_call(); }
        Call(const Call&) = delete;
        Call& operator=(const Call&) = delete;
    };
    void set_user_stream(hipStream_t s, bool enable) { user_stream_ = s; has_user_stream_ = enable; }
    double last_ms = 0;
    long long last_kernels = 0;
    double last_flops = 0;

    hipStream_t stream() const { return stream_; }
    DevPool& pool() { return pool_; }
    const sdmi_config& config() const { return cfg_; }
    int latent_h() const { return lat_h_; }
    int latent_w() const { return lat_w_; }
    static void check_latent_size(int h, int w);
    void set_latent_size(int h, int w) { check_latent_size(h, w); lat_h_ = h; lat_w_ = w; }

    struct Buf {
        Engine* e; void* p;
        Buf(Engine* e_, size_t bytes) : e(e_), p(e_->pool_.alloc(bytes)) {}
        ~Buf() { if (p) e->pool_.free(p); }
        Buf(const Buf&) = delete;
        Buf& operator=(const Buf&) = delete;
        float* f() const { return reinterpret_cast<float*>(p); }
    };
    const float* stage_epi(std::unique_ptr<Buf>& b, const float* host, long long rows, int c, int ld, int dt, long long nchw_hw = 0);

private:
    void destroy() noexcept;
    struct Stager;
    std::unique_ptr<Stager> stager_;
    bool arena_done_[3] = {false, false, false};
    char* arena_base_[3] = {nullptr, nullptr, nullptr};
    size_t arena_bytes_[3] = {0, 0, 0};
    char* split_base_[3] = {nullptr, nullptr, nullptr};
    struct SplitRegion { char* base; size_t bytes; char* planes; };
    std::vector<SplitRegion> split_regions_;
    const void* split_planes(const float* bt) const;
    bool b3_grouped(long long rows) const { return opt_b3_grouped_ != 0 && rows % 16 == 0; }
    struct TempSplit {
        Engine* e; const float* bt; void* planes = nullptr;
        TempSplit(Engine* e_, const float* bt_, long long rows, long long K);
        ~TempSplit();
        TempSplit(const TempSplit&) = delete;
        TempSplit& operator=(const TempSplit&) = delete;
    };
    const float* temp_split_bt_ = nullptr;
    const void* temp_split_planes_ = nullptr;
    char* stage_reserve(size_t bytes, size_t* offset, int* half);
    void stage_commit(WeightEntry& e, size_t offset, int half);
    void pack_entry(WeightEntry& e, float* stage);
    static size_t stage_elems(const WeightEntry& e);
    int opt_keep_masters_ = 0;
    std::vector<sdmi_lora*> loras_;
    bool lora_owned(const sdmi_lora* a) const;
    void lora_refuse_bulk_load(const char* what) const;
    bool lora_active_on(int entry) const;
    void lora_compose(int entry, float* dst);
    void lora_repack(int entry);
    void upload_weight(WeightEntry& e, const float* data);
    void stager_release();
    void ensure_arena(int group);
    bool set_meta(const std::string& name, const float* values, size_t n);
    void add_meta(const std::string& name, int n, float e0, float e1, float* store);
    std::vector<MetaEntry> meta_;
    std::map<std::string, int> meta_index_;
    void add_entry(const std::string& name, int kind, std::initializer_list<int64_t> dims, float** dst, int wdt = 0);
    int cur_group_ = 0;
    void build_model();

    Act new_act(int n, int h, int w, int c, int dt = -1);
    Act new_act3(int n, int h, int w, int c, int what);
    void release(Act& a);
    void probe_report(void* pb_dev, size_t max_blocks, int n, int cin, int h, int w, int cout, int k, int tile_cfg, int splitk);
    void conv(const ConvW& w, const Act& x, Act& y, int stride, int ups, const float* rowvec, int rowvec_stride,
              const Act* resid, bool pad_br = false);
    static Act slice(const Act& parent, int c_off, int c);
    void gemm(const float* A, int a_rows, const float* bt, const float* bias, int cin, int cout, float* C, int ldc,
              const float* resid, int ldr, int dt = -1, int out_mode = 0, const void* A3 = nullptr, void* C3 = nullptr);
    bool plane_gemm(int cin, int cout) const { return !bf16_ && gopt_.gemm_planes != 0 && gopt_.gemm_f32s != 0 && cin % 32 == 0 && cout >= 32; }
    void launch_gemm(ConvGemm& p, int in_dt, int force_cfg = -1, int force_splits = 0);
    using GemmLauncher = hipError_t (*)(const ConvGemm&, int, hipStream_t);
    struct GemmRun { GemmLauncher launch; int index; const char* what; int cfg; int pc; bool bf16_reduce, reduce_tag; double flops, bytes; };
    void record_choice(const ConvGemm& p, const char* kind, int cfg, const char* note);
    void run_gemm(ConvGemm& p, const GemmRun& r);
    int edt() const { return bf16_ ? 1 : 0; }
    size_t esz() const { return bf16_ ? 2 : 4; }
    static float* adv(const float* p, long long elems, int dt) { return (float*)((char*)const_cast<float*>(p) + elems * (dt ? 2 : 4)); }
    void group_norm(const NormW& w, const Act& x, Act& y, bool silu);
    ActQ new_actq(int n, int h, int w, int c);
    void release(ActQ& a);
    void group_norm_fp8(const NormW& w, const Act& x, ActQ& y, bool silu);
    void conv_fp8(const ConvW& w, const ActQ& x, Act& y, const float* rowvec, const Act* resid, int stride = 1, int ups = 0, int rowvec_stride = 0);
    bool use_fp8(const ConvW& w, const Act& x) const;
    bool use_fp8_wide(const float* bt8, long long rows) const { return fp8_ && opt_fp8_convs_ && opt_fp8_linear_ && bt8 && rows >= opt_fp8_min_rows_; }
    void set_resid_acc(ConvGemm& p, bool eligible, bool resid_ok) const;
    void launch_fp8(ConvGemm& p, double flops);
    void gemm_fp8(const ActQ& x, const LinW& w, int n_rows_w, void* C, int ldc, const float* resid, int ldr);
    void conv_raw(const ConvW& w, const Act& x, Act& y, int stride, int ups);
    void quantize(const Act& x, ActQ& y);
    void layer_norm_fp8(const NormW& w, const float* x, long long rows, ActQ& y);
    ActQ new_rowsq(long long rows, int c) { return new_actq(1, 1, (int)rows, c); }
    void layer_norm(const NormW& w, const float* x, long long rows, float* y, int dt = -1, void* y3 = nullptr);
    void gemm_geglu(const float* x, long long rows, const float* bt, const float* bias, int cin, int hidden, float* out, int dt,
                    const void* x3 = nullptr, void* out3 = nullptr);
    void attention(const float* q, int ldq, long long q_bs, const float* k, int ldk, long long k_bs, const float* v,
                   int ldv, long long v_bs, float* o, int ldo, long long o_bs, int n, int nq, int nk, int n_head,
                   int d_head, const int* kv_len_dev, const int* kv_len_host, const float* mask, int mask_ld, int dt = -1, void* o3 = nullptr, bool q_log2 = false);
    static bool q_prescaled(int dt, int d_head) { return dt != 0 && attn_bf16_q_is_log2(d_head); }

    void res_block(const ResW& w, const Act& x, Act& y, int step);
    void spatial_transformer(const SpatialW& w, const Act& x, Act& y);
    void vae_attn(const VaeAttnW& w, const Act& x, Act& y);

    void unet_prepare(const float* ctx_packed, int nb, int t_max, const int* kv_len_host, const std::vector<int>& ts);
    void unet_release();
    void unet_run(const float* x_nhwc, int nb, int step, float* out_nhwc, bool cfg_pair = false);
    void decode_one(const float* z_nhwc, int n, Act& img);
    Act encode_one(Act& rgb);
    struct Blend { const float* mask; const float* z0; const float* eps; };
    void sample_loop(const float* context, int n, int T, const float* uncond, int Tu, double scale, const std::vector<int>& ts,
                     size_t step_size, const std::function<void(float* latent, float* unet_in, long long per_half)>& start,
                     const Blend* blend, float* latent_out, bool out_nhwc = false);
    std::vector<int> img2img_schedule(int n, int T, int Tu, size_t n_steps, double strength, size_t* step_size);

    void count_kernel(double flops = 0) { ++n_kernels_; flops_ += flops; }
    struct Range {
        Engine* e;
        Range(Engine* e_, const char* name) : e(e_->roctx_on_ ? e_ : nullptr) { if (e) e->roctx_push(name); }
        Range(Engine* e_, const std::string& name) : Range(e_, name.c_str()) {}
        ~Range() { if (e) e->roctx_pop(); }
        Range(const Range&) = delete;
        Range& operator=(const Range&) = delete;
    };
    bool roctx_on_ = false;
    void roctx_enable(bool on);
    void roctx_push(const char* name);
    void roctx_pop();
    void check_batch(int n) const {
        if (cfg_.max_batch > 0 && n > cfg_.max_batch)
            throw Error(SDMI_ERR_INVALID, "batch of " + std::to_string(n) + " exceeds sdmi_config.max_batch = " + std::to_string(cfg_.max_batch));
    }

public:
    enum ProfClass { PC_CONV_GEMM, PC_SPLITK_REDUCE, PC_ATTENTION, PC_GROUP_NORM, PC_LAYER_NORM, PC_CONV_FP8, PC_CONV_SPLIT, PC_SPLIT_ROWS, PC_OTHER, PC_GEGLU, PC_COUNT };
    struct ProfStat { double ms = 0; long long launches = 0; double flops = 0; double bytes = 0; };
    ProfStat prof_[PC_COUNT];
    void prof_flush();
    void prof_calibrate();
    double prof_overhead_ms_ = 0;
    void prof_reset() { prof_flush(); for (auto& p : prof_) p = ProfStat{}; prof_tags_.clear(); }
    std::map<std::string, ProfStat> prof_tags_;

private:
    struct ProfScope {
        Engine* e; int cls; double flops, bytes; int n_launch; hipEvent_t a = nullptr, b = nullptr; int tag = -1;
        ProfScope(Engine* e_, int cls_, double flops_ = 0, double bytes_ = 0, int n_launch_ = 1);
        ~ProfScope();
        void set_tag(const char* fmt, ...) __attribute__((format(printf, 2, 3)));
    };
    struct ProfPending { int cls; hipEvent_t a, b; double flops, bytes; int n_launch; int tag; };
    bool prof_tagging_ = false;
    std::vector<std::string> prof_tag_names_;
    std::map<std::string, int> prof_tag_ids_;
    hipEvent_t prof_event();
    bool profiling_ = false;
    std::vector<hipEvent_t> prof_free_;
    std::vector<ProfPending> prof_pending_;

    sdmi_config cfg_;
    int lat_h_ = 0, lat_w_ = 0;
    bool bf16_ = false;
    bool fp8_ = false;
    int opt_fp8_convs_ = 1;
    int opt_fp8_min_rows_ = 1024;
    int opt_fp8_tile_ = -1;
    int opt_gn32_min_wgs_ = 256 | ((64 + 1) << 16);
    GnTune gn_tune_;
    int opt_b3_grouped_ = 1;
    int opt_attn_pack_tail_ = 3;
    int opt_attn_kv_prefer8_ = 1;
    int opt_attn_kv_splits_ = 0;
    int opt_cfg_share_ = 1;
    int opt_op_resid_ = 0;
    int opt_op_misalign_ = 0;
    int opt_fp8_ops_ = 0;
    int opt_fp8_linear_ = 0;
    sdmi_sampler sampler_{};
    hipStream_t stream_ = nullptr;
    hipEvent_t ev0_ = nullptr, ev1_ = nullptr, ev_user_ = nullptr;
    hipStream_t user_stream_ = nullptr;
    bool has_user_stream_ = false;
    bool call_dev_ = false;
    unsigned long long call_mark_ = 0;
    DevPool pool_;
    std::vector<WeightEntry> entries_;
    std::map<std::string, int> entry_index_;
    std::vector<void*> weight_allocs_;
    void* persistent_alloc(size_t bytes, bool weight_buffer = true);
    struct PersistentBlock { void* p; size_t bytes; };
    std::vector<PersistentBlock> persistent_blocks_;
    bool finalized_ = false;
    std::vector<float> alphas_;

    LinW lin1_time_, lin2_time_;
    std::vector<UBlock> in_blocks_, out_blocks_;
    ResW mid_res1_, mid_res2_;
    SpatialW mid_st_;
    NormW unet_norm_out_;
    ConvW unet_conv_out_;
    std::vector<ResW*> res_list_;
    std::vector<SpatialW*> st_list_;
    ConvW post_quant_, dec_conv_in_, dec_conv_out_;
    ResW dec_mid1_, dec_mid2_;
    VaeAttnW dec_attn_;
    DecBlockW dec_blocks_[4];
    NormW dec_norm_out_;
    float* clip_tok_ = nullptr;
    float* clip_pos_ = nullptr;
    std::vector<ClipBlockW> clip_blocks_;
    NormW clip_ln_;
    bool clip_ready_ = false;
    struct EncBlockW { ResW res[2]; ConvW down; bool has_down = false; int cin = 0, cout = 0; };
    ConvW enc_conv_in_, enc_conv_out_, quant_conv_;
    EncBlockW enc_blocks_[4];
    ResW enc_mid1_, enc_mid2_;
    VaeAttnW enc_attn_;
    NormW enc_norm_out_;
    bool enc_ready_ = false;

    struct UNetState {
        int nb = 0, t_max = 0, steps = 0;
        std::vector<float*> temb;
        std::vector<float*> kc, vc;
        int* kv_len_dev = nullptr;
        std::vector<int> kv_len_host;
        std::vector<void*> owned;
    } us_;

    int opt_resid_acc_ = 3;
    int opt_attn_bf16_ = 1;
    static constexpr int kAttnBf16VariantDefault = 7;
    int opt_attn_bf16_variant_ = kAttnBf16VariantDefault;
    int opt_geglu_fuse_ = 1;
    int opt_attn_split_ = 1;
    static constexpr int kGemm3xVariantDefault = 2;
    int opt_gemm3x_variant_ = kGemm3xVariantDefault;
    int opt_gemm_probe_ = 0;
    unsigned long long* probe_buf_ = nullptr;
    int opt_bench_cold_ = 0;
    static constexpr int kGemmBf16xVariantDefault = 5;
    int opt_gemm_bf16x_variant_ = kGemmBf16xVariantDefault;
    void* zero_page_ = nullptr;
    GemmPlanOpts gopt_;
    GemmTuning tuning_;
    bool record_shapes_ = false;
    std::map<std::string, long long> shape_counts_;
    std::map<std::string, long long> choice_counts_;

    long long n_kernels_ = 0;
    double flops_ = 0;
};

struct ResizeRow { int first = 0; std::vector<double> w; };
std::vector<ResizeRow> resize_rows(int in_size, int out_size, int mode, bool antialias);

void set_last_error(const std::string& msg);

}

struct sdmi_ctx {
    sdmi::Engine* engine;
};
struct sdmi_lora {
    sdmi::Engine* engine;
    double scale = 0;
    std::vector<sdmi::LoraTarget> targets;
    std::vector<void*> allocs;
};
```

stable_diffusion_burn_amd/csrc/k_gemm3p.hip:

```cpp
#include "kernels.hpp"
#include "k_common.hpp"
#include "k_gemm_epi.hpp"
#include "k_split3.hpp"

namespace sdmi {

typedef float f32x4 __attribute__((ext_vector_type(4)));
typedef unsigned int u32x4 __attribute__((ext_vector_type(4)));
typedef unsigned int u32x2 __attribute__((ext_vector_type(2)));
typedef __bf16 bf16x8 __attribute__((ext_vector_type(8)));
typedef __attribute__((address_space(3))) void lds_void;
typedef __attribute__((address_space(1))) const void global_cvoid;

template <int MI, int NI, int NAG, int NBW, int A_BYTES, int NWV>
struct P3Wave {
    static constexpr int NA = 3 * NAG;
    static constexpr int NP = NA + NBW;
    static constexpr int NMF = 6 * NI;
    static constexpr int NAF = MI > 2 ? 3 : MI;
    static_assert(MI == 2 || MI == 4, "fragment rows per wave");
    static_assert(NI >= 2, "plane reads of a fragment take three instruction slots (behind())");

    f32x4 acc[MI][NI];
    u32x4 wf[3][NI];
    u32x4 af[NAF][3];
    int a_iy0[NAG], a_ix0[NAG];
    unsigned a_off[NAG];
    unsigned w_off[NBW];
    unsigned w_kstep;
    const char *Abase, *Wbase, *zero, *a_src;
    unsigned pix_bytes;
    int Hin, Win, ups, Ws, KH, KW, wave;
    int cs, ky, kx, kt_next, kt_end;
    const unsigned char* a_tile;
    const unsigned char* w_tile;
    unsigned char* next_stage;

    template <int J>
    __device__ __forceinline__ void piece() {
        if constexpr (J < NA) {
            constexpr int jg = J / 3, pl = J - 3 * jg;
            if constexpr (pl == 0) {
                const int iy = a_iy0[jg] + ky;
                const int ix = a_ix0[jg] + kx;
                const bool ok = ((unsigned)iy < (unsigned)Hin) & ((unsigned)ix < (unsigned)Win);
                const unsigned off = a_off[jg] + (unsigned)((iy >> ups) * Ws + (ix >> ups)) * pix_bytes + (unsigned)cs * 192u;
                a_src = (ok ? Abase : zero) + (ok ? off : 0u);
            }
            __builtin_amdgcn_global_load_lds((global_cvoid*)(a_src + pl * 64), (lds_void*)(next_stage + ((wave + NWV * jg) * 3 + pl) * 1024), 16, 0, 0);
        } else {
            constexpr int j = J - NA;
            const char* src = Wbase + (w_off[j] + (unsigned)kt_next * w_kstep);
            __builtin_amdgcn_global_load_lds((global_cvoid*)src, (lds_void*)(next_stage + A_BYTES + (wave + NWV * j) * 1024), 16, 0, 0);
        }
        if constexpr (J == NP - 1) {
            const bool adv = kt_next + 1 < kt_end;
            const bool wrap_x = (kx + 1 == KW);
            const bool wrap_y = wrap_x && (ky + 1 == KH);
            const int kx1 = wrap_x ? 0 : kx + 1;
            const int ky1 = wrap_x ? (wrap_y ? 0 : ky + 1) : ky;
            const int cs1 = wrap_y ? cs + 1 : cs;
            kx = adv ? kx1 : kx;
            ky = adv ? ky1 : ky;
            cs = adv ? cs1 : cs;
            kt_next = adv ? kt_next + 1 : kt_next;
        }
    }
    template <int J0, int J1>
    __device__ __forceinline__ void pieces() {
        if constexpr (J0 < J1) { piece<J0>(); pieces<J0 + 1, J1>(); }
    }

    template <int F, int PL>
    __device__ __forceinline__ void read_a() { af[F % NAF][PL] = *reinterpret_cast<const u32x4*>(a_tile + (F * 3 + PL) * 1024); }
    template <int PL, int N>
    __device__ __forceinline__ void read_w() { wf[PL][N] = *reinterpret_cast<const u32x4*>(w_tile + (N * 3 + PL) * 1024); }

    static constexpr int DMA_SLOTS = 3 * NI + NMF;
    template <int MIDX, int K>
    __device__ __forceinline__ void behind() {
        constexpr int pr = K / NI, ni = K % NI;
        if constexpr (MIDX == 0) {
            if constexpr (pr == 0) { read_w<0, ni>(); if constexpr (ni == NI - 1) read_a<0, 2>(); }
            if constexpr (pr == 1) { read_w<1, ni>(); if constexpr (ni == NI - 1) read_a<0, 1>(); }
            if constexpr (K >= 2 * NI && K < 2 * NI + 3) read_a<1, K - 2 * NI>();
            if constexpr (MI > 2 && K >= 2 * NI + 3 && K < 2 * NI + 6) read_a<2, K - 2 * NI - 3>();
        } else if constexpr (MIDX + 2 < MI) {
            if constexpr (K < 3) read_a<MIDX + 2, K>();
        }
        if constexpr (MIDX == 0 && pr >= 3) {
            constexpr int slot = K - 3 * NI;
            pieces<slot * NP / DMA_SLOTS, (slot + 1) * NP / DMA_SLOTS>();
        } else if constexpr (MIDX == 1) {
            constexpr int slot = 3 * NI + K;
            pieces<slot * NP / DMA_SLOTS, (slot + 1) * NP / DMA_SLOTS>();
        }
    }
    template <int MIDX, int K>
    __device__ __forceinline__ void mfmas() {
        if constexpr (K < NMF) {
            constexpr int WP[6] = {2, 0, 1, 1, 0, 0};
            constexpr int AP[6] = {0, 2, 1, 0, 1, 0};
            constexpr int pr = K / NI, ni = K % NI;
            acc[MIDX][ni] = __builtin_amdgcn_mfma_f32_16x16x32_bf16(__builtin_bit_cast(bf16x8, wf[WP[pr]][ni]), __builtin_bit_cast(bf16x8, af[MIDX % NAF][AP[pr]]),
                                                                    acc[MIDX][ni], 0, 0, 0);
            behind<MIDX, K>();
            __builtin_amdgcn_sched_barrier(0);
            mfmas<MIDX, K + 1>();
        }
    }
    template <int MIDX>
    __device__ __forceinline__ void rows() {
        if constexpr (MIDX < MI) { mfmas<MIDX, 0>(); rows<MIDX + 1>(); }
    }
    template <int N>
    __device__ __forceinline__ void head_w() {
        if constexpr (N < NI) { read_w<2, N>(); head_w<N + 1>(); }
    }
    __device__ __forceinline__ void tile() {
        read_a<0, 0>();
        head_w<0>();
        __builtin_amdgcn_sched_barrier(0);
        rows<0>();
    }
};

template <int MI, int NI, int WM, int WN, int NSTG, bool PROBE = false>
__global__ __launch_bounds__(WM * WN * 64, 2) void conv_gemm3p_kernel(const ConvGemm p) {
    static_assert(NSTG == 2 || NSTG == 3, "LDS stages");
    constexpr int BM = 16 * MI * WM;
    constexpr int BN = 16 * NI * WN;
    constexpr int NWV = WM * WN;
    static_assert(NWV == 8 || NWV == 4, "8 or 4 waves per workgroup");
    static_assert(BM % (16 * NWV) == 0, "every wave owns whole 16-row fragment groups of the activation tile");
    constexpr int NAG = BM / (16 * NWV);
    constexpr int PW = (BN / 16) * 3;
    constexpr int NBW = (PW + NWV - 1) / NWV;
    constexpr int A_BYTES = (BM / 16) * 3 * 1024;
    constexpr int STAGE = A_BYTES + NBW * NWV * 1024;

    extern __shared__ __attribute__((aligned(16))) unsigned char smem_p3[];

    const int tid = threadIdx.x;
    const int lane = tid & 63;
    const int wave = __builtin_amdgcn_readfirstlane(tid >> 6);
    const int wm = wave / WN;
    const int wn = wave - wm * WN;

    constexpr int WNC = 16 * NI;
    const bool geglu = p.geglu != 0;
    const int BNO = geglu ? BN / 2 : BN;
    const int MT = (p.M + BM - 1) / BM;
    const int NT = (p.N + BNO - 1) / BNO;
    const GemmWork gw = gemm_work_of_block(p, MT, NT);
    if (!gw.live) return;
    const int lid = gw.lid;
    const int m0 = gw.tm * BM;
    const int n0 = gw.tn * BNO;
    const int z = gw.z;
    const int kt_begin = z * p.kt_per_split;
    const int kt_end = min(kt_begin + p.kt_per_split, p.kt_total);
    const int n_t = kt_end - kt_begin;
    const int T = p.KH * p.KW;
    const int HoWo = p.Ho * p.Wo;

    P3Wave<MI, NI, NAG, NBW, A_BYTES, NWV> w;
    w.Hin = p.Hs << p.ups;
    w.Win = p.Ws << p.ups;
    w.ups = p.ups;
    w.Ws = p.Ws;
    w.KH = p.KH;
    w.KW = p.KW;
    w.wave = wave;
    w.pix_bytes = (unsigned)p.a3_ld;
    w.Abase = reinterpret_cast<const char*>(p.A3);
    w.Wbase = reinterpret_cast<const char*>(p.Bt3);
    w.zero = reinterpret_cast<const char*>(p.zero_page);
    w.a_src = w.zero;

    const int r16 = lane >> 2;
    const int ch = (lane & 3) ^ ((-(r16 >> 2)) & 3);
#pragma unroll
    for (int j = 0; j < NAG; ++j) {
        const int m = m0 + (wave + NWV * j) * 16 + r16;
        const bool ok = m < p.M;
        const int mm = ok ? m : 0;
        const int nb = mm / HoWo;
        const int rem = mm - nb * HoWo;
        const int oy = rem / p.Wo;
        const int ox = rem - oy * p.Wo;
        w.a_off[j] = (unsigned)nb * (unsigned)(p.Hs * p.Ws) * w.pix_bytes + ch * 16;
        w.a_iy0[j] = ok ? oy * p.stride - p.pad : -(1 << 28);
        w.a_ix0[j] = ox * p.stride - p.pad;
    }
    const unsigned w_row_bytes = (unsigned)p.kt_total * 192u;
#pragma unroll
    for (int j = 0; j < NBW; ++j) {
        const int q = wave + NWV * j;
        const int f = q / 3, pl = q - 3 * f;
        int n = n0 + f * 16 + r16;
        long long wrow = n;
        if (p.geglu == 2) {
            const int fw = f / NI, ni = f - fw * NI;
            const int vg = fw / (WN / 2 > 0 ? WN / 2 : 1), col = fw - vg * (WN / 2);
            n = n0 + col * WNC + ni * 16 + r16;
            wrow = (long long)n + (vg ? p.N : 0);
        } else if (geglu) {
            const int fw = f / NI, ni = f - fw * NI;
            n = n0 + fw * (WNC / 2) + (ni >> 1) * 16 + r16;
            wrow = (long long)n + ((ni & 1) ? p.N : 0);
        }
        if (n >= p.N) wrow -= (n - (p.N - 1));
        w.w_off[j] = p.b3_grouped ? (unsigned)(wrow >> 4) * (w_row_bytes * 16u) + pl * 1024 + (unsigned)(wrow & 15) * 64 + ch * 16
                                  : (unsigned)wrow * w_row_bytes + pl * 64 + ch * 16;
    }
    w.w_kstep = p.b3_grouped ? 3072u : 192u;

    w.cs = kt_begin / T;
    const int tap0 = kt_begin - w.cs * T;
    w.ky = tap0 / p.KW;
    w.kx = tap0 - w.ky * p.KW;
    w.kt_next = kt_begin;
    w.kt_end = kt_end;

    const int c15 = lane & 15, g4 = lane >> 4;
    const int fr = c15 * 64 + ((g4 ^ ((-(c15 >> 2)) & 3)) << 4);
    const int a_fr = wm * MI * 3 * 1024 + fr;
    const int w_fr = A_BYTES + wn * NI * 3 * 1024 + fr;

#pragma unroll
    for (int mi = 0; mi < MI; ++mi)
#pragma unroll
        for (int ni = 0; ni < NI; ++ni) w.acc[mi][ni] = f32x4{0.f, 0.f, 0.f, 0.f};

    unsigned long long pt0 = 0, pt1 = 0, pc0 = 0, pwait = 0;
    if constexpr (PROBE) pt0 = __builtin_amdgcn_s_memrealtime();
    w.next_stage = smem_p3;
    w.template pieces<0, NAG * 3 + NBW>();
    if constexpr (PROBE) {
        __syncthreads();
        pt1 = __builtin_amdgcn_s_memrealtime();
        pc0 = __builtin_amdgcn_s_memtime();
    }
    if constexpr (NSTG == 2) {
        for (int t = 0; t < n_t; ++t) {
            const int cur = t & 1;
            unsigned long long pa = 0;
            if constexpr (PROBE) pa = __builtin_amdgcn_s_memtime();
            sdmi_dma_landed();
            __syncthreads();
            if constexpr (PROBE) pwait += __builtin_amdgcn_s_memtime() - pa;
            w.next_stage = smem_p3 + (cur ^ 1) * STAGE;
            w.a_tile = smem_p3 + cur * STAGE + a_fr;
            w.w_tile = smem_p3 + cur * STAGE + w_fr;
            w.tile();
        }
    } else {
        w.next_stage = smem_p3 + STAGE;
        w.template pieces<0, NAG * 3 + NBW>();
        int cur = 0;
        for (int t = 0; t < n_t; ++t) {
            unsigned long long pa = 0;
            if constexpr (PROBE) pa = __builtin_amdgcn_s_memtime();
            asm volatile("s_waitcnt vmcnt(%0)" ::"n"(NAG * 3 + NBW) : "memory");
            __builtin_amdgcn_s_barrier();
            asm volatile("" ::: "memory");
            if constexpr (PROBE) pwait += __builtin_amdgcn_s_memtime() - pa;
            const int nxt = cur == 0 ? 2 : cur - 1;
            w.next_stage = smem_p3 + nxt * STAGE;
            w.a_tile = smem_p3 + cur * STAGE + a_fr;
            w.w_tile = smem_p3 + cur * STAGE + w_fr;
            w.tile();
            cur = cur == 2 ? 0 : cur + 1;
        }
    }
    asm volatile("s_waitcnt vmcnt(0)" ::: "memory");
    unsigned long long pt2 = 0, pc2 = 0;
    if constexpr (PROBE) { pt2 = __builtin_amdgcn_s_memrealtime(); pc2 = __builtin_amdgcn_s_memtime(); }

    gemm_epilogue_f32<MI, NI, WM, WN>(p, w.acc, smem_p3, m0, n0, z, lid, wave, lane, HoWo);
    if constexpr (PROBE) {
        asm volatile("s_waitcnt vmcnt(0)" ::: "memory");
        __syncthreads();
        unsigned long long* d = p.probe + 24ull * (blockIdx.x + (unsigned long long)gridDim.x * blockIdx.z);
        if (lane == 0) { d[4 + 2 * wave] = pc2 - pc0; d[5 + 2 * wave] = pwait; }
        if (tid == 0) { d[0] = pt0; d[1] = pt1; d[2] = pt2; d[3] = __builtin_amdgcn_s_memrealtime(); }
    }
}

template <int MI, int NI, int WM, int WN, int NSTG, bool PROBE = false>
static hipError_t launch_cfg_3p(const ConvGemm& p, dim3 grid, hipStream_t stream) {
    auto k = conv_gemm3p_kernel<MI, NI, WM, WN, NSTG, PROBE>;
    constexpr int NWV = WM * WN;
    constexpr size_t stage = (size_t)(MI * WM) * 3 * 1024 + (size_t)((NI * WN * 3 + NWV - 1) / NWV) * NWV * 1024;
    constexpr size_t lds = NSTG * stage > (size_t)NWV * 16 * (16 * NI + 4) * 4 ? NSTG * stage : (size_t)NWV * 16 * (16 * NI + 4) * 4;
    static_assert(lds <= 160 * 1024, "the stages must fit the CU's LDS");
    hipError_t e = set_max_dynamic_lds(reinterpret_cast<const void*>(k), (int)lds);
    if (e != hipSuccess) return e;
    hipLaunchKernelGGL(k, grid, dim3(NWV * 64), lds, stream, p);
    return hipGetLastError();
}

hipError_t launch_conv_gemm3p(const ConvGemm& p, int cfg, hipStream_t stream) {
    if (cfg < 0 || cfg >= kNumGemmTilesP) return hipErrorInvalidValue;
    if ((p.Cin % 32) || p.CS != 32 || !p.zero_page || !p.Bt3 || !p.A3 || p.a3_ld <= 0 || (p.a3_ld % 192) || p.out_mode != 0) return hipErrorInvalidValue;
    const bool odd_ni = (cfg == 0 || cfg == 3 || cfg == 7);
    if (p.geglu == 1 && (odd_ni || p.splits != 1 || (p.N & 7) || (p.ldc & 7) || p.rowvec || p.resid)) return hipErrorInvalidValue;
    if (p.geglu == 2 && (cfg == 8 || p.splits != 1 || (p.N & 3) || (p.C && (p.ldc & 3)) || (p.C3 && (p.N & 31)) || p.rowvec || p.resid || (!p.C && !p.C3))) return hipErrorInvalidValue;
    if (p.geglu != 0 && p.geglu != 1 && p.geglu != 2) return hipErrorInvalidValue;
    if ((unsigned long long)p.N * (p.geglu ? 2 : 1) * (unsigned long long)p.kt_total * 192ull >= 0xFFFFFF00ull) return hipErrorInvalidValue;
    if ((unsigned long long)p.NB * p.Hs * p.Ws * (unsigned long long)p.a3_ld >= 0xFFFFFF00ull) return hipErrorInvalidValue;
    const int bm = kTilesP[cfg].bm, bn = kTilesP[cfg].bn;
    const int bno = p.geglu ? bn / 2 : bn;
    const int MT = (p.M + bm - 1) / bm, NT = (p.N + bno - 1) / bno;
    const dim3 grid = gemm_grid(p, MT * NT);
    if (p.probe) {
        if ((unsigned long long)grid.x * grid.z > (unsigned long long)kGemmProbeBlocks) return hipErrorInvalidValue;
        switch (cfg) {
            case 0: return launch_cfg_3p<4, 5, 4, 2, 2, true>(p, grid, stream);
            case 3: return launch_cfg_3p<2, 5, 4, 2, 2, true>(p, grid, stream);
            case 4: return launch_cfg_3p<2, 4, 4, 2, 3, true>(p, grid, stream);
        }
        return hipErrorInvalidValue;
    }
    switch (cfg) {
        case 0: return launch_cfg_3p<4, 5, 4, 2, 2>(p, grid, stream);
        case 1: return launch_cfg_3p<4, 4, 4, 2, 2>(p, grid, stream);
        case 2: return launch_cfg_3p<4, 4, 2, 4, 2>(p, grid, stream);
        case 3: return launch_cfg_3p<2, 5, 4, 2, 2>(p, grid, stream);
        case 4: return launch_cfg_3p<2, 4, 4, 2, 3>(p, grid, stream);
        case 5: return launch_cfg_3p<2, 2, 2, 2, 3>(p, grid, stream);
        case 6: return launch_cfg_3p<2, 4, 2, 2, 2>(p, grid, stream);
        case 7: return launch_cfg_3p<4, 5, 1, 4, 2>(p, grid, stream);
        case 8: return launch_cfg_3p<2, 4, 4, 1, 2>(p, grid, stream);
    }
    return hipErrorInvalidValue;
}

__global__ void split3_rows_kernel(const float* __restrict__ x, unsigned short* __restrict__ y3, long long rows, int kt, long long ld, long long ld3_elems) {
    const long long total = rows * kt * 4;
    for (long long i = (long long)blockIdx.x * blockDim.x + threadIdx.x; i < total; i += (long long)gridDim.x * blockDim.x) {
        const int g = (int)(i & 3);
        const long long rk = i >> 2;
        const long long row = rk / kt;
        const int k = (int)(rk - row * kt);
        const float* src = x + row * ld + k * 32;
        const f32x4 lo = *reinterpret_cast<const f32x4*>(src + 4 * g);
        const f32x4 hi = *reinterpret_cast<const f32x4*>(src + 16 + 4 * g);
        u32x4 ph, pm, plo;
        s3_split8(lo, hi, ph, pm, plo);
        unsigned short* dst = y3 + row * ld3_elems + k * 96 + g * 8;
        *reinterpret_cast<u32x4*>(dst) = ph;
        *reinterpret_cast<u32x4*>(dst + 32) = pm;
        *reinterpret_cast<u32x4*>(dst + 64) = plo;
    }
}

hipError_t launch_split3_rows(const float* x, void* y3, long long rows, int c, long long ld, long long ld3_bytes, hipStream_t s) {
    if ((c % 32) || (ld % 4) || (ld3_bytes % 192) || ld3_bytes < (long long)(c / 32) * 192) return hipErrorInvalidValue;
    const long long total = rows * (c / 32) * 4;
    long long blocks = (total + 255) / 256;
    if (blocks > 8192) blocks = 8192;
    if (blocks < 1) blocks = 1;
    hipLaunchKernelGGL(split3_rows_kernel, dim3((unsigned)blocks), dim3(256), 0, s, x, reinterpret_cast<unsigned short*>(y3), rows, c / 32, ld, ld3_bytes / 2);
    return hipGetLastError();
}

__global__ void join3_rows_kernel(const unsigned short* __restrict__ x3, float* __restrict__ y, long long rows, int kt, long long ld3_elems, long long ld) {
    const long long total = rows * kt * 32;
    for (long long i = (long long)blockIdx.x * blockDim.x + threadIdx.x; i < total; i += (long long)gridDim.x * blockDim.x) {
        const int j = (int)(i & 31);
        const long long rk = i >> 5;
        const long long row = rk / kt;
        const int k = (int)(rk - row * kt);
        const unsigned short* src = x3 + row * ld3_elems + k * 96 + s3_plane_pos(j);
        const float h = __builtin_bit_cast(float, (unsigned)src[0] << 16);
        const float m = __builtin_bit_cast(float, (unsigned)src[32] << 16);
        const float l = __builtin_bit_cast(float, (unsigned)src[64] << 16);
        y[row * ld + k * 32 + j] = (h + m) + l;
    }
}

hipError_t launch_join3_rows(const void* x3, float* y, long long rows, int c, long long ld3_bytes, long long ld, hipStream_t s) {
    if ((c % 32) || (ld3_bytes % 192)) return hipErrorInvalidValue;
    const long long total = rows * c;
    long long blocks = (total + 255) / 256;
    if (blocks > 8192) blocks = 8192;
    if (blocks < 1) blocks = 1;
    hipLaunchKernelGGL(join3_rows_kernel, dim3((unsigned)blocks), dim3(256), 0, s, reinterpret_cast<const unsigned short*>(x3), y, rows, c / 32, ld3_bytes / 2, ld);
    return hipGetLastError();
}

}
```

stable_diffusion_burn_amd/csrc/kernels.hpp:

```cpp
#pragma once
#include <hip/hip_runtime.h>
#include <stdint.h>
#include "gemm_tiles.hpp"

namespace sdmi {

struct ConvGemm {
    const float* A;
    const float* Bt;
    const void* Bt3;
    int b3_grouped;
    const void* A3;
    int a3_ld;
    float* C;
    void* C3;
    int ldc3;
    float* slabs;
    const float* bias;
    const float* rowvec;
    const float* resid;
    int M, N, K;
    int NB, Hs, Ws, Cin;
    int Ho, Wo;
    int KH, KW, stride, pad, ups;
    int ldc, ldr;
    int a_ld;
    int b_ld;
    int rowvec_stride;
    int CS;
    int kt_total;
    int kt_per_split;
    int splits;
    long long slab_stride;
    unsigned a_bytes, b_bytes;
    int out_mode;
    const void* zero_page;
    const void* a_scale;
    const void* b_scale;
    int variant;
    int resid_acc;
    int geglu;
    unsigned long long* probe;
};

constexpr int kGemmProbeBlocks = 1 << 13;

inline dim3 gemm_grid(const ConvGemm& p, int tiles) {
    return dim3((unsigned)(((tiles + 7) / 8) * 8), 1, (unsigned)p.splits);
}

hipError_t launch_conv_gemm2(const ConvGemm& p, int tile_cfg, hipStream_t stream);
size_t gemm2_tile_lds_bytes(int cfg);
hipError_t launch_conv_gemm_bf16(const ConvGemm& p, int tile_cfg, hipStream_t stream);
hipError_t launch_splitk_reduce_bf16(const ConvGemm& p, hipStream_t stream);
hipError_t launch_conv_gemm_bf16x(const ConvGemm& p, int tile_cfg, hipStream_t stream);
hipError_t launch_conv_gemm_bf16t(const ConvGemm& p, int tile_cfg, hipStream_t stream);
inline hipError_t launch_conv_gemm_bf16_large(const ConvGemm& p, int c, hipStream_t stream) {
    return c < kNumGemmTilesX ? launch_conv_gemm_bf16x(p, c, stream) : launch_conv_gemm_bf16t(p, c - kNumGemmTilesX, stream);
}
hipError_t launch_conv_gemm2x(const ConvGemm& p, int tile_cfg, hipStream_t stream);
hipError_t launch_conv_gemm3x(const ConvGemm& p, int tile_cfg, hipStream_t stream);
hipError_t launch_pack_split3(const float* bt, void* w3, long long rows, int K, hipStream_t s, bool grouped = false);
hipError_t launch_conv_gemm3p(const ConvGemm& p, int tile_cfg, hipStream_t stream);
hipError_t launch_split3_rows(const float* x, void* y3, long long rows, int c, long long ld, long long ld3_bytes, hipStream_t s);
hipError_t launch_join3_rows(const void* x3, float* y, long long rows, int c, long long ld3_bytes, long long ld, hipStream_t s);
hipError_t set_max_dynamic_lds(const void* kernel, int bytes);
hipError_t launch_conv_gemm_fp8x(const ConvGemm& p, int tile_cfg, hipStream_t stream);
hipError_t launch_pack_conv_weight_fp8(const float* w_oihw, void* bt8, void* bs, int cout, int cin, int kh, int kw, hipStream_t s);
struct GnTune;
hipError_t launch_group_norm_fp8(const void* x, void* y8, void* y_scale, const float* gamma, const float* beta, int n, int hw, int c,
                                 int ldx, int n_group, float eps, bool silu, void* partials, hipStream_t stream, const GnTune* t = nullptr);
hipError_t launch_quantize_fp8(const float* x, void* q, void* s, long long rows, int c, hipStream_t stream);
hipError_t launch_quantize_bf16_fp8(const void* x, void* q, void* s, long long rows, int c, int ldx, hipStream_t stream);
hipError_t launch_layer_norm_fp8(const void* x, void* y8, void* y_scale, const float* gamma, const float* beta, int rows, int c, float eps, hipStream_t stream);
hipError_t launch_geglu_fp8(const void* proj, void* y8, void* y_scale, long long rows, int hidden, hipStream_t stream);
hipError_t launch_pack_linear_weight_fp8(const float* w_in_out, void* bt8, void* bs, int cin, int cout, hipStream_t s);
hipError_t launch_dequant_fp8(const void* q, const void* s, float* out, long long rows, int c, hipStream_t stream);
hipError_t launch_pack_conv_weight_bf16(const float* w_oihw, void* bt, int cout, int cin, int kh, int kw, hipStream_t s);
hipError_t launch_pack_linear_weight_bf16(const float* w_in_out, void* bt, int cin, int cout, hipStream_t s);
hipError_t launch_splitk_reduce(const ConvGemm& p, hipStream_t stream);
__host__ __device__ inline bool splitk_reduce_vec(const ConvGemm& p, bool bf16) {
    const uintptr_t ra = bf16 ? 7 : 15, ca = (bf16 && p.out_mode != 1) ? 7 : 15;
    return ((p.N | p.ldc | p.rowvec_stride) & 3) == 0 && (!p.resid || (p.ldr & 3) == 0) && (((uintptr_t)p.bias | (uintptr_t)p.rowvec) & 15) == 0 &&
           ((uintptr_t)p.resid & ra) == 0 && ((uintptr_t)p.C & ca) == 0;
}
hipError_t launch_pack_conv_weight(const float* w_oihw, float* bt, int cout, int cin, int kh, int kw, hipStream_t s);
hipError_t launch_pack_linear_weight(const float* w_in_out, float* bt, int cin, int cout, hipStream_t s);

struct AttnParams {
    const float* q; const float* k; const float* v; float* o;
    const int* kv_len;
    const float* mask;
    int mask_ld;
    int n, n_head, nq, nk, d_head;
    int ldq, ldk, ldv, ldo;
    long long q_bs, k_bs, v_bs, o_bs;
    float scale;
    int bf16;
    int q_log2;
    void* o3;
    int ldo3;
    int kv_splits;
    float* part_o;
    float* part_ml;
    int variant;
    int pack_tail;
};
bool attn_supported_head_dim(int d);
hipError_t launch_attention(const AttnParams& p, hipStream_t stream);
bool attn_split_supported(const AttnParams& p);
hipError_t launch_attention_split(const AttnParams& p, hipStream_t stream);
hipError_t launch_attention_combine(const AttnParams& p, hipStream_t stream);
int attn_f32_kv_tile(const AttnParams& p);
inline float attn_bf16_q_scale(int d_head) { return (float)(1.4426950408889634 / __builtin_sqrt((double)d_head)); }
inline bool attn_bf16_q_is_log2(int d_head) { return d_head == 40 || d_head == 80 || d_head == 160; }
hipError_t launch_attention_bf16(const AttnParams& p, hipStream_t stream);
hipError_t launch_softmax_rows(float* x, int rows, int cols, float scale, hipStream_t stream);

size_t gn_partials_bytes(int n, int hw, int c, int min_wgs = 0);
hipError_t launch_group_norm(const float* x, float* y, const float* gamma, const float* beta,
                             int n, int hw, int c, int ldx, int n_group, float eps, bool silu,
                             void* partials, hipStream_t stream, int min_wgs = 0);
hipError_t launch_layer_norm(const float* x, float* y, const float* gamma, const float* beta,
                             int rows, int c, float eps, hipStream_t stream);
hipError_t launch_group_norm_planes(const float* x, void* y3, const float* gamma, const float* beta, int n, int hw, int c, int ldx,
// ... 65 lines not shown
```

stable_diffusion_burn_amd/csrc/sdmi_capi.cpp:

```cpp
#include <algorithm>
#include <climits>
#include <cmath>
#include <cstdint>
#include <cstring>
#include <memory>
#include <string>
#include <vector>

#include "engine.hpp"
#include "mpk_reader.hpp"
#include "tokenizer.hpp"

using sdmi::Engine;
using sdmi::Error;

namespace sdmi {
void write_png_rgb8(const std::string& path, const uint8_t* rgb, int width, int height);
}

struct sdmi_tokenizer {
    sdmi::Tokenizer tok;
};

static thread_local std::string g_last_error;
// ... 824 lines not shown
        dout.fetch();
    });
}

int sdmi_op_conv2d(sdmi_ctx* ctx, const float* x, const float* weight, const float* bias, int32_t n, int32_t cin,
                   int32_t h, int32_t w, int32_t cout, int32_t k, int32_t stride, int32_t pad, int32_t upsample2x,
                   float* out) {
    return guarded([&] {
        Engine& e = eng(ctx);
        if (n <= 0 || cin <= 0 || h <= 0 || w <= 0 || cout <= 0 || stride <= 0) throw Error(SDMI_ERR_INVALID, "conv2d: bad shape");
        const int ups = upsample2x ? 1 : 0;
        const int hin = h << ups, win = w << ups;
        const int ho = (hin + 2 * pad - k) / stride + 1, wo = (win + 2 * pad - k) / stride + 1;
        Engine::Call call(e);
        DevIn dx(e, x, (size_t)n * cin * h * w * sizeof(float)), dw(e, weight, (size_t)cout * cin * k * k * sizeof(float));
        Engine::Buf db(&e, (size_t)cout * sizeof(float));
        if (bias) SDMI_HIP(hipMemcpyAsync(db.p, bias, (size_t)cout * sizeof(float), hipMemcpyHostToDevice, e.stream()));
        DevOut dout(e, out, (size_t)n * cout * ho * wo * sizeof(float));
        e.op_conv2d(dx.f(), dw.f(), bias ? db.f() : nullptr, n, cin, h, w, cout, k, stride, pad, ups, dout.f());
        call.finish();
        dout.fetch();
    });
}

int sdmi_op_conv2d_epilogue(sdmi_ctx* ctx, const float* x, const float* weight, const float* bias, const float* temb, int32_t temb_stride,
                            const float* resid, int32_t resid_ld, int32_t n, int32_t cin, int32_t h, int32_t w, int32_t cout, int32_t k, int32_t stride,
                            int32_t pad, int32_t upsample2x, float* out) {
    return guarded([&] {
        Engine& e = eng(ctx);
        if (n <= 0 || cin <= 0 || h <= 0 || w <= 0 || cout <= 0 || stride <= 0 || temb_stride < 0 || resid_ld < 0) throw Error(SDMI_ERR_INVALID, "conv2d_epilogue: bad shape");
        const int ups = upsample2x ? 1 : 0;
        const int hin = h << ups, win = w << ups;
        const int ho = (hin + 2 * pad - k) / stride + 1, wo = (win + 2 * pad - k) / stride + 1;
        Engine::Call call(e);
        DevIn dx(e, x, (size_t)n * cin * h * w * sizeof(float)), dw(e, weight, (size_t)cout * cin * k * k * sizeof(float));
        std::unique_ptr<Engine::Buf> db;
        const float* bias_d = bias ? e.stage_epi(db, bias, 1, cout, cout, 0) : nullptr;
        Engine::EpiOps epi;
        epi.temb = temb; epi.temb_stride = temb_stride; epi.resid = resid; epi.resid_ld = resid_ld;
        DevOut dout(e, out, (size_t)n * cout * ho * wo * sizeof(float));
        e.op_conv2d(dx.f(), dw.f(), bias_d, n, cin, h, w, cout, k, stride, pad, ups, dout.f(), &epi);
        call.finish();
        dout.fetch();
    });
}

int sdmi_op_linear_epilogue(sdmi_ctx* ctx, const float* x, const float* weight, const float* bias, const float* resid, int32_t resid_ld, int32_t rows,
                            int32_t cin, int32_t cout, float* out) {
    return guarded([&] {
        Engine& e = eng(ctx);
        if (rows <= 0 || cin <= 0 || cout <= 0 || resid_ld < 0) throw Error(SDMI_ERR_INVALID, "linear_epilogue: bad shape");
        Engine::Call call(e);
        DevIn dx(e, x, (size_t)rows * cin * sizeof(float)), dw(e, weight, (size_t)cin * cout * sizeof(float));
        std::unique_ptr<Engine::Buf> db;
        const float* bias_d = bias ? e.stage_epi(db, bias, 1, cout, cout, 0) : nullptr;
        Engine::EpiOps epi;
        epi.resid = resid; epi.resid_ld = resid_ld;
        DevOut dout(e, out, (size_t)rows * cout * sizeof(float));
        e.op_linear(dx.f(), dw.f(), bias_d, rows, cin, cout, dout.f(), &epi);
        call.finish();
        dout.fetch();
    });
}

namespace {
std::vector<float> view_parent(const float* x, int n, int c, int h, int w, int ld, int off, float fill) {
    if (!x) throw Error(SDMI_ERR_INVALID, "null input pointer");
    const size_t hw = (size_t)h * w;
    std::vector<float> img((size_t)n * hw * ld, fill);
    for (int b = 0; b < n; ++b)
        for (int j = 0; j < c; ++j) {
            const float* src = x + ((size_t)b * c + j) * hw;
            float* dst = img.data() + (size_t)b * hw * ld + off + j;
            for (size_t i = 0; i < hw; ++i) dst[i * ld] = src[i];
        }
    return img;
}
void need_view(const sdmi_op_view* v, int cin, int cout) {
    if (!v) throw Error(SDMI_ERR_INVALID, "null view");
    Engine::check_view(*v, cin, cout);
}
}

int sdmi_op_conv2d_view(sdmi_ctx* ctx, const float* x, const float* weight, const float* bias, const float* temb, int32_t temb_stride,
                        const float* resid, int32_t resid_ld, int32_t n, int32_t cin, int32_t h, int32_t w, int32_t cout, int32_t k, int32_t stride,
                        int32_t pad, int32_t upsample2x, const sdmi_op_view* view, float* parent, float* parent_planes) {
    return guarded([&] {
        Engine& e = eng(ctx);
        if (n <= 0 || cin <= 0 || h <= 0 || w <= 0 || cout <= 0 || stride <= 0 || k <= 0 || pad < 0 || temb_stride < 0 || resid_ld < 0) throw Error(SDMI_ERR_INVALID, "conv2d_view: bad shape");
        need_view(view, cin, cout);
        const int ups = upsample2x ? 1 : 0;
        const int hin = h << ups, win = w << ups;
        const int ho = (hin + 2 * pad - k) / stride + 1, wo = (win + 2 * pad - k) / stride + 1;
        if (ho <= 0 || wo <= 0) throw Error(SDMI_ERR_INVALID, "conv2d_view: empty output");
        const bool both = view->out_planes == 3 && e.config().precision == 0;
        if (both && !parent_planes) throw Error(SDMI_ERR_INVALID, "conv2d_view: out_planes = 3 returns two copies of the parent");
        const std::vector<float> xp = view_parent(x, n, cin, h, w, view->in_ld, view->in_off, view->in_fill);
        const size_t pbytes = (size_t)n * ho * wo * view->out_ld * sizeof(float);
        Engine::Call call(e);
        DevIn dx(e, xp.data(), xp.size() * sizeof(float)), dw(e, weight, (size_t)cout * cin * k * k * sizeof(float));
        std::unique_ptr<Engine::Buf> db;
        const float* bias_d = bias ? e.stage_epi(db, bias, 1, cout, cout, 0) : nullptr;
        Engine::EpiOps epi;
        epi.temb = temb; epi.temb_stride = temb_stride; epi.resid = resid; epi.resid_ld = resid_ld;
        DevIn dpre(e, parent, pbytes);
        DevOut dout(e, parent, pbytes);
        SDMI_HIP(hipMemcpyAsync(dout.buf.p, dpre.buf.p, pbytes, hipMemcpyDeviceToDevice, e.stream()));
        std::unique_ptr<DevOut> dout3;
        if (both) dout3.reset(new DevOut(e, parent_planes, pbytes));
        try {
            e.op_conv2d_view(dx.f(), dw.f(), bias_d, n, cin, h, w, cout, k, stride, pad, ups, *view, &epi, dout.f(), both ? dout3->f() : nullptr);
        } catch (...) {
            try { dout.fetch(); } catch (...) {}
            throw;
        }
        call.finish();
        dout.fetch();
        if (both) dout3->fetch();
    });
}

int sdmi_op_linear_view(sdmi_ctx* ctx, const float* x, const float* weight, const float* bias, const float* resid, int32_t resid_ld, int32_t rows,
                        int32_t cin, int32_t cout, const sdmi_op_view* view, float* parent) {
    return guarded([&] {
        Engine& e = eng(ctx);
        if (rows <= 0 || cin <= 0 || cout <= 0 || resid_ld < 0) throw Error(SDMI_ERR_INVALID, "linear_view: bad shape");
        need_view(view, cin, cout);
        const size_t pbytes = (size_t)rows * view->out_ld * sizeof(float);
        Engine::Call call(e);
        DevIn dx(e, x, (size_t)rows * cin * sizeof(float)), dw(e, weight, (size_t)cin * cout * sizeof(float));
        std::unique_ptr<Engine::Buf> db;
        const float* bias_d = bias ? e.stage_epi(db, bias, 1, cout, cout, 0) : nullptr;
        Engine::EpiOps epi;
        epi.resid = resid; epi.resid_ld = resid_ld;
        DevIn dpre(e, parent, pbytes);
        DevOut dout(e, parent, pbytes);
        SDMI_HIP(hipMemcpyAsync(dout.buf.p, dpre.buf.p, pbytes, hipMemcpyDeviceToDevice, e.stream()));
        try {
            e.op_linear_view(dx.f(), dw.f(), bias_d, rows, cin, cout, *view, &epi, dout.f());
        } catch (...) {
            try { dout.fetch(); } catch (...) {}
            throw;
        }
        call.finish();
        dout.fetch();
    });
}

int sdmi_op_group_norm_view(sdmi_ctx* ctx, const float* x, const float* gamma, const float* beta, int32_t n, int32_t c, int32_t h, int32_t w,
                            int32_t n_group, float eps, int32_t fuse_silu, const sdmi_op_view* view, int32_t form, float* out) {
    return guarded([&] {
        Engine& e = eng(ctx);
        if (n <= 0 || c <= 0 || h <= 0 || w <= 0) throw Error(SDMI_ERR_INVALID, "group_norm_view: bad shape");
        need_view(view, c, c);
        const std::vector<float> xp = view_parent(x, n, c, h, w, view->in_ld, view->in_off, view->in_fill);
        Engine::Call call(e);
        DevIn dx(e, xp.data(), xp.size() * sizeof(float)), dg(e, gamma, c * sizeof(float)), db(e, beta, c * sizeof(float));
        DevOut dout(e, out, (size_t)n * c * h * w * sizeof(float));
        e.op_group_norm_view(dx.f(), dg.f(), db.f(), n, c, h, w, n_group, eps, fuse_silu != 0, *view, form, dout.f());
        call.finish();
        dout.fetch();
    });
}

int sdmi_op_cat_chain(sdmi_ctx* ctx, const float* x, const float* w_x, const float* b_x, const float* w_skip, const float* b_skip, const float* gamma,
                      const float* beta, int32_t n, int32_t cin, int32_t h, int32_t w, int32_t cx, int32_t cskip, float eps, int32_t fuse_silu,
// ... 125 lines not shown
```

stable_diffusion_burn_amd/pipeline.py:

```python
from __future__ import annotations

import ctypes as C
import os
from dataclasses import dataclass

import numpy as np

from . import _capi
from ._capi import SdmiConfig, SdmiError, SdmiHires, SdmiOpView, SdmiSampler, check, load_library

def mpk_list(path) -> list:
    lib = load_library()
    need = C.c_size_t()
    check(lib.sdmi_mpk_list(str(path).encode(), None, 0, C.byref(need)))
    buf = C.create_string_buffer(need.value)
    check(lib.sdmi_mpk_list(str(path).encode(), buf, need.value, C.byref(need)))
    out = []
    for line in buf.value.decode().splitlines():
        if line.startswith("#") or not line:
            continue
        name, shape, off = line.split("\t")
        out.append((name, tuple(int(v) for v in shape.split(",")) if shape else (), int(off)))
    return out

# ... 646 lines not shown
        return out

    def op_group_norm(self, x, gamma, beta, n_group=32, eps=1e-5, silu=False):
        x = _f32(x)
        n, c, h, w = x.shape
        out = np.empty_like(x)
        check(self._lib.sdmi_op_group_norm(self._ctx, _fp(x), _fp(_f32(gamma, (c,))), _fp(_f32(beta, (c,))), n, c, h, w,
                                           n_group, eps, int(silu), _fp(out)))
        return out

    def op_group_norm_fp8(self, x, gamma, beta, n_group=32, eps=1e-5, silu=False):
        x = _f32(x)
        n, c, h, w = x.shape
        out = np.empty_like(x)
        check(self._lib.sdmi_op_group_norm_fp8(self._ctx, _fp(x), _fp(_f32(gamma, (c,))), _fp(_f32(beta, (c,))), n, c, h, w,
                                               n_group, eps, int(silu), _fp(out)))
        return out

    def op_layer_norm(self, x, gamma, beta, eps=1e-5):
        x = _f32(x)
        c = x.shape[-1]
        rows = x.size // c
        out = np.empty_like(x)
        check(self._lib.sdmi_op_layer_norm(self._ctx, _fp(x), _fp(_f32(gamma, (c,))), _fp(_f32(beta, (c,))), rows, c,
                                           eps, _fp(out)))
        return out

    def op_conv2d(self, x, weight, bias=None, stride=1, pad=None, upsample2x=False):
        x = _f32(x)
        weight = _f32(weight)
        n, cin, h, w = x.shape
        cout, cin2, k, k2 = weight.shape
        if cin2 != cin or k != k2:
            raise ValueError("conv2d: weight shape does not match input")
        if pad is None:
            pad = 1 if k == 3 else 0
        ups = 1 if upsample2x else 0
        ho = ((h << ups) + 2 * pad - k) // stride + 1
        wo = ((w << ups) + 2 * pad - k) // stride + 1
        out = np.empty((n, cout, ho, wo), dtype=np.float32)
        b = None if bias is None else _f32(bias, (cout,))
        check(self._lib.sdmi_op_conv2d(self._ctx, _fp(x), _fp(weight), None if b is None else _fp(b), n, cin, h, w, cout,
                                       k, stride, pad, ups, _fp(out)))
        return out

    def op_linear(self, x, weight, bias=None):
        x = _f32(x)
        weight = _f32(weight)
        cin, cout = weight.shape
        rows = x.size // cin
        out = np.empty(x.shape[:-1] + (cout,), dtype=np.float32)
        b = None if bias is None else _f32(bias, (cout,))
        check(self._lib.sdmi_op_linear(self._ctx, _fp(x), _fp(weight), None if b is None else _fp(b), rows, cin, cout,
                                       _fp(out)))
        return out

    def op_conv2d_epilogue(self, x, weight, bias=None, temb=None, resid=None, stride=1, upsample2x=False, temb_stride=None, resid_ld=0):
        x = _f32(x)
        weight = _f32(weight)
        n, cin, h, w = x.shape
        cout, cin2, k, k2 = weight.shape
        if cin2 != cin or k != k2:
            raise ValueError("conv2d: weight shape does not match input")
        pad = 1 if k == 3 else 0
        ups = 1 if upsample2x else 0
        ho = ((h << ups) + 2 * pad - k) // stride + 1
        wo = ((w << ups) + 2 * pad - k) // stride + 1
        out = np.empty((n, cout, ho, wo), dtype=np.float32)
        b = None if bias is None else _f32(bias, (cout,))
        t = None if temb is None else _f32(temb)
        if t is not None:
            if t.shape not in ((cout,), (n, cout)):
                raise ValueError("conv2d_epilogue: temb must be [cout] or [n, cout]")
            if temb_stride is None:
                temb_stride = 0 if t.ndim == 1 else cout
            if (temb_stride == 0) != (t.ndim == 1):
                raise ValueError("conv2d_epilogue: temb_stride 0 means one row for the batch")
        r = None if resid is None else _f32(resid, (n, cout, ho, wo))
        check(self._lib.sdmi_op_conv2d_epilogue(self._ctx, _fp(x), _fp(weight), None if b is None else _fp(b), None if t is None else _fp(t),
                                                temb_stride or 0, None if r is None else _fp(r), resid_ld, n, cin, h, w, cout, k, stride, pad, ups,
                                                _fp(out)))
        return out

    def op_linear_epilogue(self, x, weight, bias=None, resid=None, resid_ld=0):
        x = _f32(x)
        weight = _f32(weight)
        cin, cout = weight.shape
        rows = x.size // cin
        out = np.empty(x.shape[:-1] + (cout,), dtype=np.float32)
        b = None if bias is None else _f32(bias, (cout,))
        r = None if resid is None else _f32(resid, out.shape)
        check(self._lib.sdmi_op_linear_epilogue(self._ctx, _fp(x), _fp(weight), None if b is None else _fp(b), None if r is None else _fp(r),
                                                resid_ld, rows, cin, cout, _fp(out)))
        return out

    def _view_call(self, parent, fn):
        try:
            fn()
        except SdmiError as e:
            e.parent = parent
            raise

    def op_conv2d_view(self, x, weight, bias=None, temb=None, resid=None, stride=1, upsample2x=False, temb_stride=None, resid_ld=0, *, parent, out_off,
                       in_ld=None, in_off=0, in_fill=float("nan"), in_planes=0, out_planes=0):
        x = _f32(x)
        weight = _f32(weight)
        n, cin, h, w = x.shape
        cout, cin2, k, k2 = weight.shape
        if cin2 != cin or k != k2:
            raise ValueError("conv2d: weight shape does not match input")
        pad = 1 if k == 3 else 0
        ups = 1 if upsample2x else 0
        ho = ((h << ups) + 2 * pad - k) // stride + 1
        wo = ((w << ups) + 2 * pad - k) // stride + 1
        out = np.array(parent, dtype=np.float32, order="C", copy=True)
        if out.ndim != 2 or out.shape[0] != n * ho * wo:
            raise ValueError(f"conv2d_view: parent must be [{n * ho * wo}, out_ld], got {out.shape}")
        b = None if bias is None else _f32(bias, (cout,))
        t = None if temb is None else _f32(temb)
        if t is not None:
            if t.shape not in ((cout,), (n, cout)):
                raise ValueError("conv2d_view: temb must be [cout] or [n, cout]")
            if temb_stride is None:
                temb_stride = 0 if t.ndim == 1 else cout
        r = None if resid is None else _f32(resid, (n, cout, ho, wo))
        v = SdmiOpView(cin if in_ld is None else in_ld, in_off, out.shape[1], out_off, in_fill, in_planes, out_planes)
        out3 = np.empty_like(out) if out_planes == 3 else None
        self._view_call(out, lambda: check(self._lib.sdmi_op_conv2d_view(
            self._ctx, _fp(x), _fp(weight), None if b is None else _fp(b), None if t is None else _fp(t), temb_stride or 0,
            None if r is None else _fp(r), resid_ld, n, cin, h, w, cout, k, stride, pad, ups, C.byref(v), _fp(out), None if out3 is None else _fp(out3))))
        return out if out3 is None else (out, out3)

    def op_linear_view(self, x, weight, bias=None, resid=None, resid_ld=0, *, parent, out_off):
        x = _f32(x)
        weight = _f32(weight)
        cin, cout = weight.shape
        rows = x.size // cin
        out = np.array(parent, dtype=np.float32, order="C", copy=True)
        if out.ndim != 2 or out.shape[0] != rows:
            raise ValueError(f"linear_view: parent must be [{rows}, out_ld], got {out.shape}")
        b = None if bias is None else _f32(bias, (cout,))
        r = None if resid is None else _f32(resid, (rows, cout))
        v = SdmiOpView(cin, 0, out.shape[1], out_off, float("nan"), 0, 0)
        self._view_call(out, lambda: check(self._lib.sdmi_op_linear_view(self._ctx, _fp(x), _fp(weight), None if b is None else _fp(b), None if r is None else _fp(r),
                                                                         resid_ld, rows, cin, cout, C.byref(v), _fp(out))))
        return out

    def op_group_norm_view(self, x, gamma, beta, eps=1e-5, silu=False, *, in_ld, in_off, in_fill=float("nan"), in_planes=0, form=0):
        x = _f32(x)
        n, c, h, w = x.shape
        out = np.empty_like(x)
        v = SdmiOpView(in_ld, in_off, c, 0, in_fill, in_planes, 0)
        check(self._lib.sdmi_op_group_norm_view(self._ctx, _fp(x), _fp(_f32(gamma, (c,))), _fp(_f32(beta, (c,))), n, c, h, w, 32, eps, int(silu), C.byref(v),
                                                form, _fp(out)))
        return out

    def op_cat_chain(self, x, w_x, b_x, w_skip, b_skip, gamma, beta, eps=1e-5, silu=True, dense=False):
        x = _f32(x)
        n, cin, h, w = x.shape
        w_x, w_skip = _f32(w_x), _f32(w_skip)
        cx, cskip = w_x.shape[0], w_skip.shape[0]
        if w_x.shape != (cx, cin, 3, 3) or w_skip.shape != (cskip, cin, 3, 3):
            raise ValueError("cat_chain: weights must be [cout, cin, 3, 3]")
        out = np.empty((n, cx + cskip, h, w), dtype=np.float32)
        check(self._lib.sdmi_op_cat_chain(self._ctx, _fp(x), _fp(w_x), _fp(_f32(b_x, (cx,))), _fp(w_skip), _fp(_f32(b_skip, (cskip,))),
                                          _fp(_f32(gamma, (cx + cskip,))), _fp(_f32(beta, (cx + cskip,))), n, cin, h, w, cx, cskip, eps, int(silu), int(dense),
# ... 270 lines not shown
```

Baseline: 4.155.

## Fuse resnet 1x1 skip conv into conv_out GEMM via extended K loop

Adds a fused path where the resnet block's 1x1 shortcut convolution is appended as extra K tiles to the 3x3 conv_out planar GEMM. The skip output no longer needs a separate GEMM launch and an intermediate buffer that is written and then read back as a residual. The kernel gains a second A/B plane source and a K-walk that switches to the shortcut operands after the main taps. It only applies to f32 plane GEMMs of the P family and falls back otherwise. It also adds a standalone op API and lets TempSplit hold two slots at once.

```diff
diff --git a/include/sdmi.h b/include/sdmi.h
--- a/include/sdmi.h
+++ b/include/sdmi.h
@@ -193,6 +193,9 @@
                             int32_t w, int32_t cout, int32_t k, int32_t stride, int32_t pad, int32_t upsample2x, float* out);
 int sdmi_op_linear_epilogue(sdmi_ctx* ctx, const float* x, const float* weight, const float* bias, const float* resid,
                             int32_t resid_ld, int32_t rows, int32_t cin, int32_t cout, float* out);
+int sdmi_op_conv2d_shortcut(sdmi_ctx* ctx, const float* h, const float* weight, const float* bias, const float* x, const float* weight_skip,
+                            const float* bias_skip, int32_t n, int32_t cout, int32_t cin, int32_t hh, int32_t ww, int32_t stride,
+                            int32_t in_ld, int32_t in_off, float in_fill, float* out);
 typedef struct sdmi_op_view {
     int32_t in_ld, in_off;
     int32_t out_ld, out_off;
diff --git a/stable_diffusion_burn_amd/_capi.py b/stable_diffusion_burn_amd/_capi.py
--- a/stable_diffusion_burn_amd/_capi.py
+++ b/stable_diffusion_burn_amd/_capi.py
@@ -122,6 +122,8 @@
     "sdmi_op_linear": (C.c_int, [_CTX, _F, _F, _F, C.c_int32, C.c_int32, C.c_int32, _F]),
     "sdmi_op_conv2d_epilogue": (C.c_int, [_CTX, _F, _F, _F, _F, C.c_int32, _F, C.c_int32, C.c_int32, C.c_int32, C.c_int32, C.c_int32, C.c_int32, C.c_int32, C.c_int32,
                                           C.c_int32, C.c_int32, _F]),
+    "sdmi_op_conv2d_shortcut": (C.c_int, [_CTX, _F, _F, _F, _F, _F, _F, C.c_int32, C.c_int32, C.c_int32, C.c_int32, C.c_int32, C.c_int32, C.c_int32, C.c_int32,
+                                          C.c_float, _F]),
     "sdmi_op_linear_epilogue": (C.c_int, [_CTX, _F, _F, _F, _F, C.c_int32, C.c_int32, C.c_int32, C.c_int32, _F]),
     "sdmi_op_conv2d_view": (C.c_int, [_CTX, _F, _F, _F, _F, C.c_int32, _F, C.c_int32, C.c_int32, C.c_int32, C.c_int32, C.c_int32, C.c_int32, C.c_int32, C.c_int32,
                                       C.c_int32, C.c_int32, _VIEW, _F, _F]),
diff --git a/stable_diffusion_burn_amd/csrc/engine.cpp b/stable_diffusion_burn_amd/csrc/engine.cpp
--- a/stable_diffusion_burn_amd/csrc/engine.cpp
+++ b/stable_diffusion_burn_amd/csrc/engine.cpp
@@ -638,18 +638,21 @@
     planes = e->pool_.alloc((size_t)rows * K * 6);
     hipError_t err = launch_pack_split3(bt, planes, rows, (int)K, e->stream_, e->b3_grouped(rows));
     if (err != hipSuccess) { e->pool_.free(planes); planes = nullptr; SDMI_HIP(err); }
-    e->temp_split_bt_ = bt;
-    e->temp_split_planes_ = planes;
+    slot = e->temp_split_bt_[0] ? 1 : 0;
+    if (e->temp_split_bt_[slot]) { e->pool_.free(planes); planes = nullptr; throw Error(SDMI_ERR_STATE, "TempSplit: both slots taken"); }
+    e->temp_split_bt_[slot] = bt;
+    e->temp_split_planes_[slot] = planes;
 }
 Engine::TempSplit::~TempSplit() {
     if (!planes) return;
-    e->temp_split_bt_ = nullptr;
-    e->temp_split_planes_ = nullptr;
+    e->temp_split_bt_[slot] = nullptr;
+    e->temp_split_planes_[slot] = nullptr;
     e->pool_.free(planes);
 }
 
 const void* Engine::split_planes(const float* bt) const {
-    if (bt && bt == temp_split_bt_) return temp_split_planes_;
+    for (int i = 0; i < 2; ++i)
+        if (bt && bt == temp_split_bt_[i]) return temp_split_planes_[i];
     const char* b = reinterpret_cast<const char*>(bt);
     for (int g = 0; g < 3; ++g)
         if (split_base_[g] && b >= arena_base_[g] && b < arena_base_[g] + arena_bytes_[g]) return split_base_[g] + (size_t)(b - arena_base_[g]) / 2 * 3;
@@ -1225,6 +1228,7 @@
     else if (key == "gemm3x_variant") opt_gemm3x_variant_ = (value == "default") ? kGemm3xVariantDefault : std::stoi(value);
     else if (key == "gemm_bf16x_variant") opt_gemm_bf16x_variant_ = (value == "default") ? kGemmBf16xVariantDefault : std::stoi(value);
     else if (key == "geglu_fuse") opt_geglu_fuse_ = std::stoi(value);
+    else if (key == "res_skip_fuse") opt_res_skip_fuse_ = (value == "default") ? kResSkipFuseDefault : std::stoi(value);
     else if (key == "record_shapes") { record_shapes_ = std::stoi(value) != 0; if (record_shapes_) { shape_counts_.clear(); choice_counts_.clear(); } }
     else if (key == "dump_shapes") {
         std::ofstream f(value);
@@ -1287,7 +1291,7 @@
     count_kernel();
 }
 
-void Engine::launch_gemm(ConvGemm& p, int in_dt, int force_cfg, int force_splits) {
+bool Engine::launch_gemm(ConvGemm& p, int in_dt, int force_cfg, int force_splits, int ext_cin) {
     const int kt_elems = in_dt ? 64 : 32;
     p.kt_total = (p.K + kt_elems - 1) / kt_elems;
     if (in_dt && (p.Cin % 64)) throw Error(SDMI_ERR_UNSUPPORTED, "bf16 GEMM: K slices must be multiples of 64");
@@ -1311,12 +1315,20 @@
     in.from_planes = !in_dt && p.A3 != nullptr;
     if (!in.from_planes && !p.A) throw Error(SDMI_ERR_STATE, "gemm: no activations");
     const GemmPlan g = plan_gemm(in, gopt_, tuning_);
+    if (ext_cin > 0 && (g.tile.family != kFamP || in_dt || !p.A3 || !p.A3b || !p.Bt3b || p.kt_main != p.kt_total)) return false;
     p.kt_per_split = g.kt_per_split; p.splits = g.splits;
+    const int k_main = p.K;
+    if (ext_cin > 0) {
+        p.kt_total = p.kt_main + ext_cin / 32;
+        p.kt_per_split = (p.kt_total + p.splits - 1) / p.splits;
+        p.splits = (p.kt_total + p.kt_per_split - 1) / p.kt_per_split;
+        p.K = k_main + ext_cin;
+    }
     const bool w_planes = g.tile.family >= kFamS, a_planes = g.tile.family == kFamP;
     const double flops = 2.0 * p.M * (double)p.N * p.K * (p.geglu ? 2.0 : 1.0);
     const unsigned long long es = in_dt ? 2ull : 4ull;
     const unsigned long long a_ext = ((unsigned long long)p.NB * p.Hs * p.Ws - 1) * (unsigned long long)p.a_ld * es + (unsigned long long)p.Cin * es;
-    const unsigned long long b_ext = ((unsigned long long)p.N * (p.geglu ? 2 : 1) - 1) * (unsigned long long)p.b_ld * es + (unsigned long long)p.K * es;
+    const unsigned long long b_ext = ((unsigned long long)p.N * (p.geglu ? 2 : 1) - 1) * (unsigned long long)p.b_ld * es + (unsigned long long)k_main * es;
     if (a_ext >= 0xFFFFFFE0ull || b_ext >= 0xFFFFFFE0ull) throw Error(SDMI_ERR_UNSUPPORTED, "GEMM: operand larger than 4 GiB (the buffer-load range check needs 32-bit extents)");
     p.a_bytes = (unsigned)a_ext;
     p.b_bytes = (unsigned)b_ext;
@@ -1347,7 +1359,7 @@
     record_choice(p, "", g.cfg, p.Bt3 || in_dt ? "" : " (no planes)");
     const double a_es = in_dt ? 2.0 : (a_planes ? 6.0 : 4.0), w_es = in_dt ? 2.0 : (w_planes ? 6.0 : 4.0);
     const double c_es = in_dt ? (p.out_mode == 1 ? 4.0 : 2.0) : (p.out_mode == 2 ? 2.0 : ((p.C ? 4.0 : 0.0) + (c3_native ? 6.0 : 0.0)));
-    const double gemm_bytes = (double)p.NB * p.Hs * p.Ws * p.Cin * a_es + (double)p.N * (p.geglu ? 2.0 : 1.0) * p.K * w_es + (double)p.M * p.N * c_es;
+    const double gemm_bytes = (double)p.NB * p.Hs * p.Ws * (p.Cin + ext_cin) * a_es + (double)p.N * (p.geglu ? 2.0 : 1.0) * p.K * w_es + (double)p.M * p.N * c_es;
     static const GemmLauncher kLaunchers[2][kNumGemmFamilies] = {{launch_conv_gemm2, launch_conv_gemm2x, launch_conv_gemm3x, launch_conv_gemm3p},
                                                                  {launch_conv_gemm_bf16, launch_conv_gemm_bf16_large, nullptr, nullptr}};
     run_gemm(p, GemmRun{kLaunchers[in_dt ? 1 : 0][g.tile.family], g.tile.index, "gemm", g.cfg, w_planes ? PC_CONV_SPLIT : PC_CONV_GEMM, in_dt != 0, true, flops, gemm_bytes});
@@ -1356,6 +1368,46 @@
         SDMI_HIP(launch_split3_rows(p.C, c3_want, p.M, p.N, p.ldc, ldc3_want, stream_));
         count_kernel();
     }
+    return true;
+}
+
+bool Engine::conv_shortcut(const ConvW& w, const Act& h, const ConvW& ws, const Act& x, Act& y) {
+    if (!opt_res_skip_fuse_ || bf16_ || fp8_ || h.dt || x.dt || y.dt || w.dt || ws.dt) return false;
+    if (w.k != 3 || ws.k != 1 || w.cin != h.c || ws.cin != x.c || w.cout != ws.cout || y.c != w.cout) return false;
+    if (x.n != h.n || x.h != h.h || x.w != h.w || y.n != h.n || y.h != h.h || y.w != h.w) return false;
+    if (!plane_gemm(w.cin, w.cout) || !h.p3 || !x.p3 || (x.c % 32) || x.ld3 <= 0 || (x.ld3 % 192)) return false;
+    if (!split_planes(w.bt) || !split_planes(ws.bt) || (!y.p && !y.p3)) return false;
+    if (opt_res_skip_fuse_ == 1 && !res_skip_gate(x.n * x.h * x.w, w.cout, x.c)) return false;
+    if ((unsigned long long)x.rows() * (unsigned long long)x.ld3 >= 0xFFFFFF00ull || (unsigned long long)w.cout * (unsigned long long)(x.c / 32) * 192ull >= 0xFFFFFF00ull) return false;
+    ConvGemm p{};
+    p.A = h.p; p.Bt = w.bt; p.C = y.p; p.bias = w.bias;
+    p.rowvec = ws.bias; p.rowvec_stride = 0;
+    p.A3 = h.p3; p.a3_ld = h.ld3;
+    p.A3b = x.p3; p.a3b_ld = x.ld3; p.Bt3b = split_planes(ws.bt);
+    p.C3 = y.p3; p.ldc3 = y.ld3;
+    p.M = (int)h.rows(); p.N = w.cout; p.K = w.cin * 9;
+    p.kt_main = p.K / 32;
+    p.NB = h.n; p.Hs = h.h; p.Ws = h.w; p.Cin = w.cin; p.Ho = h.h; p.Wo = h.w;
+    p.KH = 3; p.KW = 3; p.stride = 1; p.pad = 1; p.ups = 0;
+    p.ldc = y.stride(); p.ldr = y.stride(); p.a_ld = h.stride(); p.b_ld = p.K;
+    p.CS = 32;
+    p.out_mode = 0;
+    return launch_gemm(p, 0, -1, 0, x.c);
+}
+
+void Engine::conv_plus_shortcut(const ConvW& w, const Act& h, const ConvW& ws, const Act& x, Act& y, int stride) {
+    if (stride == 1 && conv_shortcut(w, h, ws, x, y)) return;
+    Act sk{};
+    if (y.p) { sk = y; sk.p3 = nullptr; sk.view = true; }
+    else sk = new_act(y.n, y.h, y.w, y.c);
+    conv(ws, x, sk, 1, 0, nullptr, 0, nullptr);
+    conv(w, h, y, stride, 0, nullptr, 0, &sk);
+    release(sk);
+}
+
+bool Engine::res_skip_gate(long long M, int cout, int cin) const {
+    (void)M; (void)cout; (void)cin;
+    return true;
 }
 
 void Engine::conv(const ConvW& w, const Act& x, Act& y, int stride, int ups, const float* rowvec, int rowvec_stride,
@@ -1585,8 +1637,9 @@
         conv(w.conv_in, h1, h2, 1, 0, rowvec, 0, nullptr);
         release(h1);
     }
+    const bool fuse_try = w.has_skip && opt_res_skip_fuse_ && !bf16_ && !fp8_ && !x.dt && x.p3 && plane_gemm(w.cout, w.cout);
     Act sk{};
-    if (w.has_skip) {
+    auto run_skip = [&] {
         if (y.p) { sk = y; sk.p3 = nullptr; sk.view = true; }
         else sk = new_act(y.n, y.h, y.w, y.c);
         if (use_fp8_wide(w.skip.bt8, x.rows()) && x.dt == 1 && x.c % 32 == 0) {
@@ -1597,7 +1650,8 @@
         } else {
             conv(w.skip, x, sk, 1, 0, nullptr, 0, nullptr);
         }
-    }
+    };
+    if (w.has_skip && !fuse_try) run_skip();
     const Act* resid = w.has_skip ? &sk : &x;
     if (use_fp8(w.conv_out, h2)) {
         ActQ q3 = new_actq(x.n, x.h, x.w, w.cout);
@@ -1609,10 +1663,11 @@
         Act h3 = plane_gemm(w.cout, w.cout) ? new_act3(x.n, x.h, x.w, w.cout, 2) : new_act(x.n, x.h, x.w, w.cout);
         group_norm(w.norm_out, h2, h3, true);
         release(h2);
-        conv(w.conv_out, h3, y, 1, 0, nullptr, 0, resid);
+        if (fuse_try) conv_plus_shortcut(w.conv_out, h3, w.skip, x, y, 1);
+        else conv(w.conv_out, h3, y, 1, 0, nullptr, 0, resid);
         release(h3);
     }
-    if (w.has_skip) release(sk);
+    if (sk.p) release(sk);
 }
 
 bool Engine::use_fp8(const ConvW& w, const Act& x) const {
@@ -2575,6 +2630,47 @@
     release(a); release(y);
 }
 
+void Engine::op_conv2d_shortcut(const float* h, const float* wt, const float* bias, const float* xp, const float* wskip, const float* bskip, int n, int cout, int cin,
+                                int hh, int ww, int stride, int in_ld, int in_off, float* out) {
+    if (fp8_) throw Error(SDMI_ERR_UNSUPPORTED, "conv2d_shortcut: precision 0 or 1");
+    if (!(stride == 1 || stride == 2)) throw Error(SDMI_ERR_UNSUPPORTED, "conv2d_shortcut: stride 1|2");
+    auto chan_ok = [](int c) { return c % 32 == 0 || (c < 32 && c % 4 == 0); };
+    if (!chan_ok(cin) || !chan_ok(cout)) throw Error(SDMI_ERR_UNSUPPORTED, "conv2d_shortcut: channel counts must be multiples of 32, or < 32 and multiples of 4");
+    if (bf16_ && (cin % 64 || cout % 64)) throw Error(SDMI_ERR_UNSUPPORTED, "bf16 conv2d_shortcut: channel counts must be multiples of 64");
+    if (in_ld < cin || in_off < 0 || in_off + cin > in_ld) throw Error(SDMI_ERR_INVALID, "conv2d_shortcut: need 0 <= in_off, in_off + cin <= in_ld");
+    const int dt = bf16_ ? 1 : 0;
+    const int ho = (hh + 2 - 3) / stride + 1, wo = (ww + 2 - 3) / stride + 1;
+    ConvW w; w.cin = cout; w.cout = cout; w.k = 3; w.dt = dt; w.bias = const_cast<float*>(bias);
+    ConvW ws; ws.cin = cin; ws.cout = cout; ws.k = 1; ws.dt = dt; ws.bias = const_cast<float*>(bskip);
+    Buf bt(this, (size_t)cout * cout * 9 * 4), bts(this, (size_t)cout * cin * 4);
+    if (dt) {
+        SDMI_HIP(launch_pack_conv_weight_bf16(wt, bt.p, cout, cout, 3, 3, stream_));
+        SDMI_HIP(launch_pack_conv_weight_bf16(wskip, bts.p, cout, cin, 1, 1, stream_));
+    } else {
+        SDMI_HIP(launch_pack_conv_weight(wt, bt.f(), cout, cout, 3, 3, stream_));
+        SDMI_HIP(launch_pack_conv_weight(wskip, bts.f(), cout, cin, 1, 1, stream_));
+    }
+    TempSplit planes(this, bt.f(), dt ? 0 : cout, (long long)cout * 9), planes_s(this, bts.f(), dt ? 0 : cout, cin);
+    w.bt = bt.f(); ws.bt = bts.f();
+    Act a = (!dt && plane_gemm(cout, cout)) ? new_act3(n, hh, ww, cout, 3) : new_act(n, hh, ww, cout, dt);
+    if (dt) SDMI_HIP(launch_nchw_f32_to_nhwc_bf16(h, a.p, n, cout, hh, ww, 1.0f, stream_));
+    else SDMI_HIP(launch_nchw_to_nhwc(h, a.p, n, cout, hh, ww, 1.0f, stream_));
+    if (a.p3) SDMI_HIP(launch_split3_rows(a.p, a.p3, a.rows(), cout, cout, a.ld3, stream_));
+    const bool xplanes = !dt && in_ld % 32 == 0 && in_off % 32 == 0 && cin % 32 == 0 && plane_gemm(cin, cout);
+    Act xa = xplanes ? new_act3(n, ho, wo, in_ld, 3) : new_act(n, ho, wo, in_ld, dt);
+    if (dt) SDMI_HIP(launch_f32_to_bf16(xp, xa.p, xa.rows() * in_ld, stream_));
+    else SDMI_HIP(hipMemcpyAsync(xa.p, xp, xa.bytes(), hipMemcpyDeviceToDevice, stream_));
+    if (xa.p3) SDMI_HIP(launch_split3_rows(xp, xa.p3, xa.rows(), in_ld, in_ld, xa.ld3, stream_));
+    Act y = new_act(n, ho, wo, cout, dt);
+    {
+        Act xs = slice(xa, in_off, cin);
+        conv_plus_shortcut(w, a, ws, xs, y, stride);
+    }
+    if (dt) SDMI_HIP(launch_nhwc_bf16_to_nchw_f32(y.p, out, n, cout, ho, wo, stream_));
+    else SDMI_HIP(launch_nhwc_to_nchw(y.p, out, n, cout, ho, wo, stream_));
+    release(a); release(xa); release(y);
+}
+
 void Engine::op_linear(const float* x, const float* wt, const float* bias, int rows, int cin, int cout, float* out, const EpiOps* epi) {
     const int rld = (epi && epi->resid) ? (epi->resid_ld ? epi->resid_ld : cout) : 0;
     std::unique_ptr<Buf> rb;
diff --git a/stable_diffusion_burn_amd/csrc/engine.hpp b/stable_diffusion_burn_amd/csrc/engine.hpp
--- a/stable_diffusion_burn_amd/csrc/engine.hpp
+++ b/stable_diffusion_burn_amd/csrc/engine.hpp
@@ -161,6 +161,8 @@
     void op_conv2d(const float* x, const float* w, const float* bias, int n, int cin, int h, int wd, int cout, int k,
                    int stride, int pad, int ups, float* out, const EpiOps* epi = nullptr);
     void op_linear(const float* x, const float* w, const float* bias, int rows, int cin, int cout, float* out, const EpiOps* epi = nullptr);
+    void op_conv2d_shortcut(const float* h, const float* w, const float* bias, const float* xp, const float* wskip, const float* bskip, int n, int cout, int cin,
+                            int hh, int ww, int stride, int in_ld, int in_off, float* out);
     void op_geglu(const float* proj, int rows, int hidden, float* out);
     static void check_view(const sdmi_op_view& v, int cin, int cout);
     void op_conv2d_view(const float* xp, const float* w, const float* bias, int n, int cin, int h, int wd, int cout, int k, int stride, int pad, int ups,
@@ -225,14 +227,14 @@
     const void* split_planes(const float* bt) const;
     bool b3_grouped(long long rows) const { return opt_b3_grouped_ != 0 && rows % 16 == 0; }
     struct TempSplit {
-        Engine* e; const float* bt; void* planes = nullptr;
+        Engine* e; const float* bt; void* planes = nullptr; int slot = 0;
         TempSplit(Engine* e_, const float* bt_, long long rows, long long K);
         ~TempSplit();
         TempSplit(const TempSplit&) = delete;
         TempSplit& operator=(const TempSplit&) = delete;
     };
-    const float* temp_split_bt_ = nullptr;
-    const void* temp_split_planes_ = nullptr;
+    const float* temp_split_bt_[2] = {nullptr, nullptr};
+    const void* temp_split_planes_[2] = {nullptr, nullptr};
     char* stage_reserve(size_t bytes, size_t* offset, int* half);
     void stage_commit(WeightEntry& e, size_t offset, int half);
     void pack_entry(WeightEntry& e, float* stage);
@@ -265,7 +267,10 @@
     void gemm(const float* A, int a_rows, const float* bt, const float* bias, int cin, int cout, float* C, int ldc,
               const float* resid, int ldr, int dt = -1, int out_mode = 0, const void* A3 = nullptr, void* C3 = nullptr);
     bool plane_gemm(int cin, int cout) const { return !bf16_ && gopt_.gemm_planes != 0 && gopt_.gemm_f32s != 0 && cin % 32 == 0 && cout >= 32; }
-    void launch_gemm(ConvGemm& p, int in_dt, int force_cfg = -1, int force_splits = 0);
+    bool launch_gemm(ConvGemm& p, int in_dt, int force_cfg = -1, int force_splits = 0, int ext_cin = 0);
+    bool conv_shortcut(const ConvW& w, const Act& h, const ConvW& ws, const Act& x, Act& y);
+    bool res_skip_gate(long long M, int cout, int cin) const;
+    void conv_plus_shortcut(const ConvW& w, const Act& h, const ConvW& ws, const Act& x, Act& y, int stride);
     using GemmLauncher = hipError_t (*)(const ConvGemm&, int, hipStream_t);
     struct GemmRun { GemmLauncher launch; int index; const char* what; int cfg; int pc; bool bf16_reduce, reduce_tag; double flops, bytes; };
     void record_choice(const ConvGemm& p, const char* kind, int cfg, const char* note);
@@ -428,6 +433,8 @@
     int opt_attn_bf16_ = 1;
     static constexpr int kAttnBf16VariantDefault = 7;
     int opt_attn_bf16_variant_ = kAttnBf16VariantDefault;
+    static constexpr int kResSkipFuseDefault = 0;
+    int opt_res_skip_fuse_ = kResSkipFuseDefault;
     int opt_geglu_fuse_ = 1;
     int opt_attn_split_ = 1;
     static constexpr int kGemm3xVariantDefault = 2;
diff --git a/stable_diffusion_burn_amd/csrc/k_gemm3p.hip b/stable_diffusion_burn_amd/csrc/k_gemm3p.hip
--- a/stable_diffusion_burn_amd/csrc/k_gemm3p.hip
+++ b/stable_diffusion_burn_amd/csrc/k_gemm3p.hip
@@ -2,6 +2,7 @@
 #include "k_common.hpp"
 #include "k_gemm_epi.hpp"
 #include "k_split3.hpp"
+#include "k_gemm3p_walk.hpp"
 
 namespace sdmi {
 
@@ -12,7 +13,7 @@
 typedef __attribute__((address_space(3))) void lds_void;
 typedef __attribute__((address_space(1))) const void global_cvoid;
 
-template <int MI, int NI, int NAG, int NBW, int A_BYTES, int NWV>
+template <int MI, int NI, int NAG, int NBW, int A_BYTES, int NWV, bool EXT = false>
 struct P3Wave {
     static constexpr int NA = 3 * NAG;
     static constexpr int NP = NA + NBW;
@@ -27,6 +28,10 @@
     int a_iy0[NAG], a_ix0[NAG];
     unsigned a_off[NAG];
     unsigned w_off[NBW];
+    unsigned w_offb[EXT ? NBW : 1];
+    const char *Abase2, *Wbase2;
+    unsigned pix_bytes2, ch16;
+    int kt_main;
     unsigned w_kstep;
     const char *Abase, *Wbase, *zero, *a_src;
     unsigned pix_bytes;
@@ -40,7 +45,18 @@
     __device__ __forceinline__ void piece() {
         if constexpr (J < NA) {
             constexpr int jg = J / 3, pl = J - 3 * jg;
-            if constexpr (pl == 0) {
+            if constexpr (pl == 0 && EXT) {
+                const P3Source s = p3_walk_source(kt_next, kt_main, 1, cs, ky, kx);
+                const bool ext = s.ext;
+                const unsigned pb_m = pix_bytes, pb_x = pix_bytes2;
+                const char *const ab_m = Abase, *const ab_x = Abase2, *const zp = zero;
+                const int iy = a_iy0[jg] + s.ky;
+                const int ix = a_ix0[jg] + s.kx;
+                const bool ok = ((unsigned)iy < (unsigned)Hin) & ((unsigned)ix < (unsigned)Win);
+                const unsigned off = (a_off[jg] + (unsigned)(iy * Ws + ix)) * (ext ? pb_x : pb_m) + (unsigned)s.slice * 192u + ch16;
+                const char* const ab = ext ? ab_x : ab_m;
+                a_src = (ok ? ab : zp) + (ok ? off : 0u);
+            } else if constexpr (pl == 0) {
                 const int iy = a_iy0[jg] + ky;
                 const int ix = a_ix0[jg] + kx;
                 const bool ok = ((unsigned)iy < (unsigned)Hin) & ((unsigned)ix < (unsigned)Win);
@@ -51,20 +67,16 @@
         } else {
             constexpr int j = J - NA;
             const char* src = Wbase + (w_off[j] + (unsigned)kt_next * w_kstep);
+            if constexpr (EXT) {
+                const bool ext = kt_next >= kt_main;
+                const char *const wb_m = Wbase, *const wb_x = Wbase2;
+                const unsigned o_m = w_off[j], o_x = w_offb[j];
+                const int kt_m = kt_next, kt_x = kt_next - kt_main;
+                src = (ext ? wb_x : wb_m) + ((ext ? o_x : o_m) + (unsigned)(ext ? kt_x : kt_m) * w_kstep);
+            }
             __builtin_amdgcn_global_load_lds((global_cvoid*)src, (lds_void*)(next_stage + A_BYTES + (wave + NWV * j) * 1024), 16, 0, 0);
         }
-        if constexpr (J == NP - 1) {
-            const bool adv = kt_next + 1 < kt_end;
-            const bool wrap_x = (kx + 1 == KW);
-            const bool wrap_y = wrap_x && (ky + 1 == KH);
-            const int kx1 = wrap_x ? 0 : kx + 1;
-            const int ky1 = wrap_x ? (wrap_y ? 0 : ky + 1) : ky;
-            const int cs1 = wrap_y ? cs + 1 : cs;
-            kx = adv ? kx1 : kx;
-            ky = adv ? ky1 : ky;
-            cs = adv ? cs1 : cs;
-            kt_next = adv ? kt_next + 1 : kt_next;
-        }
+        if constexpr (J == NP - 1) p3_walk_advance(kt_end, KH, KW, cs, ky, kx, kt_next);
     }
     template <int J0, int J1>
     __device__ __forceinline__ void pieces() {
@@ -125,7 +137,7 @@
     }
 };
 
-template <int MI, int NI, int WM, int WN, int NSTG, bool PROBE = false>
+template <int MI, int NI, int WM, int WN, int NSTG, bool PROBE = false, bool EXT = false>
 __global__ __launch_bounds__(WM * WN * 64, 2) void conv_gemm3p_kernel(const ConvGemm p) {
     static_assert(NSTG == 2 || NSTG == 3, "LDS stages");
     constexpr int BM = 16 * MI * WM;
@@ -161,10 +173,9 @@
     const int kt_begin = z * p.kt_per_split;
     const int kt_end = min(kt_begin + p.kt_per_split, p.kt_total);
     const int n_t = kt_end - kt_begin;
-    const int T = p.KH * p.KW;
     const int HoWo = p.Ho * p.Wo;
 
-    P3Wave<MI, NI, NAG, NBW, A_BYTES, NWV> w;
+    P3Wave<MI, NI, NAG, NBW, A_BYTES, NWV, EXT> w;
     w.Hin = p.Hs << p.ups;
     w.Win = p.Ws << p.ups;
     w.ups = p.ups;
@@ -177,6 +188,12 @@
     w.Wbase = reinterpret_cast<const char*>(p.Bt3);
     w.zero = reinterpret_cast<const char*>(p.zero_page);
     w.a_src = w.zero;
+    if constexpr (EXT) {
+        w.Abase2 = reinterpret_cast<const char*>(p.A3b);
+        w.Wbase2 = reinterpret_cast<const char*>(p.Bt3b);
+        w.pix_bytes2 = (unsigned)p.a3b_ld;
+        w.kt_main = p.kt_main;
+    }
 
     const int r16 = lane >> 2;
     const int ch = (lane & 3) ^ ((-(r16 >> 2)) & 3);
@@ -189,11 +206,13 @@
         const int rem = mm - nb * HoWo;
         const int oy = rem / p.Wo;
         const int ox = rem - oy * p.Wo;
-        w.a_off[j] = (unsigned)nb * (unsigned)(p.Hs * p.Ws) * w.pix_bytes + ch * 16;
+        if constexpr (EXT) w.a_off[j] = (unsigned)nb * (unsigned)(p.Hs * p.Ws);
+        else w.a_off[j] = (unsigned)nb * (unsigned)(p.Hs * p.Ws) * w.pix_bytes + ch * 16;
         w.a_iy0[j] = ok ? oy * p.stride - p.pad : -(1 << 28);
         w.a_ix0[j] = ox * p.stride - p.pad;
     }
-    const unsigned w_row_bytes = (unsigned)p.kt_total * 192u;
+    if constexpr (EXT) w.ch16 = ch * 16;
+    const unsigned w_row_bytes = (unsigned)(EXT ? p.kt_main : p.kt_total) * 192u;
 #pragma unroll
     for (int j = 0; j < NBW; ++j) {
         const int q = wave + NWV * j;
@@ -213,13 +232,15 @@
         if (n >= p.N) wrow -= (n - (p.N - 1));
         w.w_off[j] = p.b3_grouped ? (unsigned)(wrow >> 4) * (w_row_bytes * 16u) + pl * 1024 + (unsigned)(wrow & 15) * 64 + ch * 16
                                   : (unsigned)wrow * w_row_bytes + pl * 64 + ch * 16;
+        if constexpr (EXT) {
+            const unsigned rb2 = (unsigned)(p.kt_total - p.kt_main) * 192u;
+            w.w_offb[j] = p.b3_grouped ? (unsigned)(wrow >> 4) * (rb2 * 16u) + pl * 1024 + (unsigned)(wrow & 15) * 64 + ch * 16
+                                       : (unsigned)wrow * rb2 + pl * 64 + ch * 16;
+        }
     }
     w.w_kstep = p.b3_grouped ? 3072u : 192u;
 
-    w.cs = kt_begin / T;
-    const int tap0 = kt_begin - w.cs * T;
-    w.ky = tap0 / p.KW;
-    w.kx = tap0 - w.ky * p.KW;
+    p3_walk_begin(kt_begin, p.KH, p.KW, w.cs, w.ky, w.kx);
     w.kt_next = kt_begin;
     w.kt_end = kt_end;
 
@@ -288,9 +309,9 @@
     }
 }
 
-template <int MI, int NI, int WM, int WN, int NSTG, bool PROBE = false>
+template <int MI, int NI, int WM, int WN, int NSTG, bool PROBE = false, bool EXT = false>
 static hipError_t launch_cfg_3p(const ConvGemm& p, dim3 grid, hipStream_t stream) {
-    auto k = conv_gemm3p_kernel<MI, NI, WM, WN, NSTG, PROBE>;
+    auto k = conv_gemm3p_kernel<MI, NI, WM, WN, NSTG, PROBE, EXT>;
     constexpr int NWV = WM * WN;
     constexpr size_t stage = (size_t)(MI * WM) * 3 * 1024 + (size_t)((NI * WN * 3 + NWV - 1) / NWV) * NWV * 1024;
     constexpr size_t lds = NSTG * stage > (size_t)NWV * 16 * (16 * NI + 4) * 4 ? NSTG * stage : (size_t)NWV * 16 * (16 * NI + 4) * 4;
@@ -310,6 +331,16 @@
     if (p.geglu != 0 && p.geglu != 1 && p.geglu != 2) return hipErrorInvalidValue;
     if ((unsigned long long)p.N * (p.geglu ? 2 : 1) * (unsigned long long)p.kt_total * 192ull >= 0xFFFFFF00ull) return hipErrorInvalidValue;
     if ((unsigned long long)p.NB * p.Hs * p.Ws * (unsigned long long)p.a3_ld >= 0xFFFFFF00ull) return hipErrorInvalidValue;
+    if (p.kt_main < 0 || (p.kt_main == 0 && (p.A3b || p.Bt3b))) return hipErrorInvalidValue;
+    if (p.kt_main > 0) {
+        const int kt_ext = p.kt_total - p.kt_main;
+        if (p.KH != 3 || p.KW != 3 || p.stride != 1 || p.pad != 1 || p.ups != 0 || p.Ho != p.Hs || p.Wo != p.Ws || p.geglu || p.probe) return hipErrorInvalidValue;
+        if (!p.A3b || !p.Bt3b || kt_ext <= 0 || p.kt_main != p.Cin / 32 * 9 || p.a3b_ld <= 0 || (p.a3b_ld % 192) || p.a3b_ld / 192 < kt_ext) return hipErrorInvalidValue;
+        if ((unsigned long long)p.a3_ld / 192 < (unsigned long long)(p.Cin / 32)) return hipErrorInvalidValue;
+        if ((unsigned long long)p.NB * p.Hs * p.Ws * (unsigned long long)p.a3b_ld >= 0xFFFFFF00ull) return hipErrorInvalidValue;
+        if ((unsigned long long)p.N * (unsigned long long)kt_ext * 192ull >= 0xFFFFFF00ull) return hipErrorInvalidValue;
+        if (p.splits < 1 || (long long)(p.splits - 1) * p.kt_per_split >= p.kt_total) return hipErrorInvalidValue;
+    }
     const int bm = kTilesP[cfg].bm, bn = kTilesP[cfg].bn;
     const int bno = p.geglu ? bn / 2 : bn;
     const int MT = (p.M + bm - 1) / bm, NT = (p.N + bno - 1) / bno;
@@ -320,6 +351,20 @@
             case 0: return launch_cfg_3p<4, 5, 4, 2, 2, true>(p, grid, stream);
             case 3: return launch_cfg_3p<2, 5, 4, 2, 2, true>(p, grid, stream);
             case 4: return launch_cfg_3p<2, 4, 4, 2, 3, true>(p, grid, stream);
+        }
+        return hipErrorInvalidValue;
+    }
+    if (p.kt_main > 0) {
+        switch (cfg) {
+            case 0: return launch_cfg_3p<4, 5, 4, 2, 2, false, true>(p, grid, stream);
+            case 1: return launch_cfg_3p<4, 4, 4, 2, 2, false, true>(p, grid, stream);
+            case 2: return launch_cfg_3p<4, 4, 2, 4, 2, false, true>(p, grid, stream);
+            case 3: return launch_cfg_3p<2, 5, 4, 2, 2, false, true>(p, grid, stream);
+            case 4: return launch_cfg_3p<2, 4, 4, 2, 3, false, true>(p, grid, stream);
+            case 5: return launch_cfg_3p<2, 2, 2, 2, 3, false, true>(p, grid, stream);
+            case 6: return launch_cfg_3p<2, 4, 2, 2, 2, false, true>(p, grid, stream);
+            case 7: return launch_cfg_3p<4, 5, 1, 4, 2, false, true>(p, grid, stream);
+            case 8: return launch_cfg_3p<2, 4, 4, 1, 2, false, true>(p, grid, stream);
         }
         return hipErrorInvalidValue;
     }
diff --git a/stable_diffusion_burn_amd/csrc/k_gemm3p_walk.hpp b/stable_diffusion_burn_amd/csrc/k_gemm3p_walk.hpp
--- /dev/null
+++ b/stable_diffusion_burn_amd/csrc/k_gemm3p_walk.hpp
@@ -0,0 +1,38 @@
+#pragma once
+
+#if defined(__HIPCC__) || defined(__CUDACC__)
+#define SDMI_WALK_HD __host__ __device__ __forceinline__
+#else
+#define SDMI_WALK_HD inline
+#endif
+
+namespace sdmi {
+
+SDMI_WALK_HD void p3_walk_begin(int kt_begin, int KH, int KW, int& cs, int& ky, int& kx) {
+    const int T = KH * KW;
+    cs = kt_begin / T;
+    const int tap0 = kt_begin - cs * T;
+    ky = tap0 / KW;
+    kx = tap0 - ky * KW;
+}
+
+SDMI_WALK_HD void p3_walk_advance(int kt_end, int KH, int KW, int& cs, int& ky, int& kx, int& kt_next) {
+    const bool adv = kt_next + 1 < kt_end;
+    const bool wrap_x = (kx + 1 == KW);
+    const bool wrap_y = wrap_x && (ky + 1 == KH);
+    const int kx1 = wrap_x ? 0 : kx + 1;
+    const int ky1 = wrap_x ? (wrap_y ? 0 : ky + 1) : ky;
+    const int cs1 = wrap_y ? cs + 1 : cs;
+    kx = adv ? kx1 : kx;
+    ky = adv ? ky1 : ky;
+    cs = adv ? cs1 : cs;
+    kt_next = adv ? kt_next + 1 : kt_next;
+}
+
+struct P3Source { bool ext; int slice, ky, kx; };
+SDMI_WALK_HD P3Source p3_walk_source(int kt, int kt_main, int pad, int cs, int ky, int kx) {
+    const bool ext = kt >= kt_main;
+    return P3Source{ext, ext ? kt - kt_main : cs, ext ? pad : ky, ext ? pad : kx};
+}
+
+}
diff --git a/stable_diffusion_burn_amd/csrc/kernels.hpp b/stable_diffusion_burn_amd/csrc/kernels.hpp
--- a/stable_diffusion_burn_amd/csrc/kernels.hpp
+++ b/stable_diffusion_burn_amd/csrc/kernels.hpp
@@ -41,6 +41,10 @@
     int resid_acc;
     int geglu;
     unsigned long long* probe;
+    const void* A3b;
+    const void* Bt3b;
+    int a3b_ld;
+    int kt_main;
 };
 
 constexpr int kGemmProbeBlocks = 1 << 13;
diff --git a/stable_diffusion_burn_amd/csrc/sdmi_capi.cpp b/stable_diffusion_burn_amd/csrc/sdmi_capi.cpp
--- a/stable_diffusion_burn_amd/csrc/sdmi_capi.cpp
+++ b/stable_diffusion_burn_amd/csrc/sdmi_capi.cpp
@@ -930,6 +930,30 @@
 }
 }
 
+int sdmi_op_conv2d_shortcut(sdmi_ctx* ctx, const float* h, const float* weight, const float* bias, const float* x, const float* weight_skip,
+                            const float* bias_skip, int32_t n, int32_t cout, int32_t cin, int32_t hh, int32_t ww, int32_t stride, int32_t in_ld,
+                            int32_t in_off, float in_fill, float* out) {
+    return guarded([&] {
+        Engine& e = eng(ctx);
+        if (n <= 0 || cin <= 0 || cout <= 0 || hh <= 0 || ww <= 0 || !(stride == 1 || stride == 2) || in_ld < 0 || in_off < 0) throw Error(SDMI_ERR_INVALID, "conv2d_shortcut: bad shape");
+        if (!h || !weight || !weight_skip || !out) throw Error(SDMI_ERR_INVALID, "null pointer");
+        const int ld = in_ld ? in_ld : cin;
+        if (ld < cin || in_off + cin > ld) throw Error(SDMI_ERR_INVALID, "conv2d_shortcut: need in_off + cin <= in_ld");
+        const int ho = (hh + 2 - 3) / stride + 1, wo = (ww + 2 - 3) / stride + 1;
+        const std::vector<float> xp = view_parent(x, n, cin, ho, wo, ld, in_off, in_fill);
+        Engine::Call call(e);
+        DevIn dh(e, h, (size_t)n * cout * hh * ww * sizeof(float)), dw(e, weight, (size_t)cout * cout * 9 * sizeof(float));
+        DevIn dx(e, xp.data(), xp.size() * sizeof(float)), dws(e, weight_skip, (size_t)cout * cin * sizeof(float));
+        std::unique_ptr<Engine::Buf> db, dbs;
+        const float* bias_d = bias ? e.stage_epi(db, bias, 1, cout, cout, 0) : nullptr;
+        const float* bias_sd = bias_skip ? e.stage_epi(dbs, bias_skip, 1, cout, cout, 0) : nullptr;
+        DevOut dout(e, out, (size_t)n * cout * ho * wo * sizeof(float));
+        e.op_conv2d_shortcut(dh.f(), dw.f(), bias_d, dx.f(), dws.f(), bias_sd, n, cout, cin, hh, ww, stride, ld, in_off, dout.f());
+        call.finish();
+        dout.fetch();
+    });
+}
+
 int sdmi_op_conv2d_view(sdmi_ctx* ctx, const float* x, const float* weight, const float* bias, const float* temb, int32_t temb_stride,
                         const float* resid, int32_t resid_ld, int32_t n, int32_t cin, int32_t h, int32_t w, int32_t cout, int32_t k, int32_t stride,
                         int32_t pad, int32_t upsample2x, const sdmi_op_view* view, float* parent, float* parent_planes) {
diff --git a/stable_diffusion_burn_amd/pipeline.py b/stable_diffusion_burn_amd/pipeline.py
--- a/stable_diffusion_burn_amd/pipeline.py
+++ b/stable_diffusion_burn_amd/pipeline.py
@@ -752,6 +752,25 @@
                                                 _fp(out)))
         return out
 
+    def op_conv2d_shortcut(self, h, weight, bias, x, weight_skip, bias_skip=None, stride=1, in_ld=None, in_off=0, in_fill=float("nan")):
+        h = _f32(h)
+        weight = _f32(weight)
+        x = _f32(x)
+        weight_skip = _f32(weight_skip)
+        n, cout, hh, ww = h.shape
+        cin = x.shape[1]
+        ho = (hh + 2 - 3) // stride + 1
+        wo = (ww + 2 - 3) // stride + 1
+        if weight.shape != (cout, cout, 3, 3) or weight_skip.shape != (cout, cin, 1, 1) or x.shape != (n, cin, ho, wo):
+            raise ValueError("conv2d_shortcut: shapes do not match")
+        out = np.empty((n, cout, ho, wo), dtype=np.float32)
+        b = None if bias is None else _f32(bias, (cout,))
+        bs = None if bias_skip is None else _f32(bias_skip, (cout,))
+        check(self._lib.sdmi_op_conv2d_shortcut(self._ctx, _fp(h), _fp(weight), None if b is None else _fp(b), _fp(x), _fp(weight_skip),
+                                                None if bs is None else _fp(bs), n, cout, cin, hh, ww, stride, cin if in_ld is None else in_ld, in_off,
+                                                in_fill, _fp(out)))
+        return out
+
     def op_linear_epilogue(self, x, weight, bias=None, resid=None, resid_ld=0):
         x = _f32(x)
         weight = _f32(weight)
```

Result: no change. 4.156 (median of 3 runs) (+0.0%).
